# hanquansanren/DvD

Measured on AMD Instinct MI355X. Metric: documents/sec (50-step DDIM, 288x288 grid), higher is better.
Workload: dtype f16

## Files before the change

dvd_amd/csrc/attention.hip:

```cpp
#include "common.h"
#include "mfma.h"
#include <stdlib.h>

#ifndef DVD_ATTN64_OCC
#define DVD_ATTN64_OCC 2
#endif
#ifndef DVD_ATTN64_ROWSUM
#define DVD_ATTN64_ROWSUM 0
#endif
#ifndef DVD_ATTN_PF
#define DVD_ATTN_PF 4
#endif

namespace dvd {

struct AttnArgs {
  const _Float16* Q;
  const _Float16* K;
  const _Float16* Vt;
  _Float16* O;
  long sQ, sK, sVt, sO;
  int ldq, ldk, ldvt, ldo;
  int heads, batch, tq, tk;
  int kv_div;
  int nqb;
  float c;
  unsigned long long* stamps;
  int xcd_map;
};

__device__ __forceinline__ int kappa(int r) {
  return (r & ~12) | ((r & 4) << 1) | ((r & 8) >> 1);
}

__device__ __forceinline__ float half_swap_max(float x) {
  float a = x, b = x;
  asm volatile("s_nop 1\n\tv_permlane32_swap_b32 %0, %1\n\ts_nop 1" : "+v"(a), "+v"(b));
  return fmaxf(a, b);
}

template <int D>
__global__ void __launch_bounds__(256, (D == 256 ? 1 : 2)) flash_attn_kernel(AttnArgs p) {
  constexpr int KB = 64;
  constexpr int KP = 2 * D + 16;
  constexpr int VP = 2 * KB + 16;
  constexpr int KBYTES = KB * KP, VBYTES = D * VP;
  constexpr int KCH = D / 8;
  constexpr int NK = KB * KCH / 256;
  constexpr int NV = D * 8 / 256;
  constexpr int KS = D / 16;
  constexpr int DT = D / 32;
  constexpr float RESCALE_THR = 10.f;
  extern __shared__ __attribute__((aligned(16))) char smem[];

  const int nwg = gridDim.x;
  int id = blockIdx.x;
  {
    const int q = nwg / 8, rr = nwg % 8, xcd = id % 8, k = id / 8;
    id = (xcd < rr ? xcd * (q + 1) : rr * (q + 1) + (xcd - rr) * q) + k;
  }
  const int qb = id % p.nqb;
  const int bh = id / p.nqb;
  const int head = bh % p.heads, b = bh / p.heads;
  const int kvb = b / p.kv_div;

  const int tid = threadIdx.x, lane = tid & 63, wave = tid >> 6;
  const int r = lane & 31, h = lane >> 5;

  const _Float16* Qg = p.Q + b * p.sQ + (size_t)head * D;
  const _Float16* Kg = p.K + kvb * p.sK + (size_t)head * D;
  const _Float16* Vg = p.Vt + kvb * p.sVt + (size_t)head * D * p.ldvt;

  const int qrow = min(qb * 128 + wave * 32 + r, p.tq - 1);
  half8 qf[KS];
  {
    const _Float16* qp = Qg + (size_t)qrow * p.ldq + 8 * h;
#pragma unroll
    for (int ks = 0; ks < KS; ++ks) qf[ks] = *(const half8*)(qp + 16 * ks);
  }

  floatx16 o[DT];
#pragma unroll
  for (int dt = 0; dt < DT; ++dt)
#pragma unroll
    for (int i = 0; i < 16; ++i) o[dt][i] = 0.f;
  float m_run = -1e30f, l_run = 0.f;

  u32x4 kreg[NK], vreg[NV];
  int k_lofs[NK], v_lofs[NV];
  int k_row[NK], k_col[NK], v_row[NV], v_col[NV];
#pragma unroll
  for (int i = 0; i < NK; ++i) {
    const int cidx = tid + 256 * i;
    k_row[i] = cidx / KCH;
    k_col[i] = (cidx % KCH) * 8;
    k_lofs[i] = k_row[i] * KP + (cidx % KCH) * 16;
  }
#pragma unroll
  for (int i = 0; i < NV; ++i) {
    const int cidx = tid + 256 * i;
    v_row[i] = cidx / 8;
    v_col[i] = (cidx % 8) * 8;
    v_lofs[i] = KBYTES + v_row[i] * VP + (cidx % 8) * 16;
  }
  const int nt = (p.tk + KB - 1) / KB;

#define DVD_ATTN_GLOAD(t_)                                                                  \
  {                                                                                         \
    const int key0 = (t_) * KB;                                                             \
    _Pragma("unroll") for (int i = 0; i < NK; ++i) {                                        \
      const int kr = min(key0 + k_row[i], p.tk - 1);                                        \
// ... 1266 lines not shown
    if (j < 2) r64p::glds_piece(Vg + (size_t)min(j, nt - 1) * (KB * 2), voff, vdst + j * VBYTES);
  }
  asm volatile("s_waitcnt vmcnt(0)\n\ts_barrier" ::: "memory");

  float a0, a1;
  h64m_prologue_s0(kf, a0, a1);
  asm volatile("s_barrier" ::: "memory");
  {
    const float mloc[2] = {a0, a1};
#pragma unroll
    for (int rb = 0; rb < 2; ++rb) {
      const float m = half_swap_max(mloc[rb] * p.c);
      sm[rb].m = m;
      sm[rb].thr = m + RESCALE_THR;
    }
  }
  const char* kg = uniform_ptr(Kg + (size_t)min(3, nt - 1) * ktile);
  const char* vg = uniform_ptr(Vg + (size_t)min(2, nt - 1) * (KB * 2));
  const int klim = nt - 4, vlim = nt - 3;
  const unsigned kstep = (unsigned)ktile, vstep = KB * 2;
  float e0, e1;
  h64m_prologue_units(kf, p.c, sm[0].m, sm[1].m, e0, e1);
#define H64M_LOOP_ARGS sm[0].l, sm[1].l, sm[0].m, sm[1].m, sm[0].thr, sm[1].thr, e0, e1, kg, vg, nt, kf, vrel0, vrel1, koff, voff, p.c, \
                       kdst, vdst, kstep, vstep, klim, vlim
#ifdef DVD_LAB
  if constexpr (DBG == 1) h64m_loop_noeu(H64M_LOOP_ARGS);
  else if constexpr (DBG == 2) h64m_loop_m16(H64M_LOOP_ARGS);
  else if constexpr (DBG == 3) h64m_loop_mfmaonly(H64M_LOOP_ARGS);
  else
#endif
    h64m_loop(H64M_LOOP_ARGS);
#undef H64M_LOOP_ARGS

  const int lane_e = (int)__builtin_amdgcn_mbcnt_hi(~0u, __builtin_amdgcn_mbcnt_lo(~0u, 0u));
  const int re = lane_e & 31, he = lane_e >> 5;
#pragma unroll
  for (int rb = 0; rb < 2; ++rb) {
    const float l_tot = sm[rb].l + __shfl_xor(sm[rb].l, 32);
    const float inv = 1.f / l_tot;
    const int qglob = qb * 256 + wave * 64 + rb * 32 + re;
    if (qglob < p.tq) {
      _Float16* op = p.O + b * p.sO + (size_t)qglob * p.ldo + (size_t)head * D + 4 * he;
#pragma unroll
      for (int dt = 0; dt < 2; ++dt) {
        floatx16 x;
        if (rb == 0 && dt == 0) x = r64m_read_o<0>();
        else if (rb == 0) x = r64m_read_o<16>();
        else if (dt == 0) x = r64m_read_o<32>();
        else x = r64m_read_o<48>();
#pragma unroll
        for (int g4 = 0; g4 < 4; ++g4) {
          half4 v;
#pragma unroll
          for (int j = 0; j < 4; ++j) v[j] = (_Float16)(x[4 * g4 + j] * inv);
          *(half4*)(op + 32 * dt + 8 * g4) = v;
        }
      }
    }
  }
}


typedef unsigned uintx4 __attribute__((ext_vector_type(4)));
#include "attn_h64x_body.inc"
#include "attn_h64l_body.inc"
#ifdef DVD_LAB
#include "../../benchmarks/lab/csrc/attn_h64x_abl.inc"
#include "../../benchmarks/lab/csrc/attn_h64l_abl.inc"
#endif

template <int DBG, bool LM>
__global__ void __launch_bounds__(256, 2) __attribute__((amdgpu_num_vgpr(H64X_COMPILER_VGPRS))) flash_attn_h64x_kernel(AttnArgs p) {
  using namespace h64m;
  constexpr int D = 64, KB = 32;
  extern __shared__ __attribute__((aligned(16))) char smem[];
  typedef __attribute__((address_space(3))) void* lptr_t;

  const int nwg = gridDim.x;
  int id = blockIdx.x;
  {
    const int q = nwg / 8, rr = nwg % 8, xcd = id % 8, k = id / 8;
    id = (xcd < rr ? xcd * (q + 1) : rr * (q + 1) + (xcd - rr) * q) + k;
  }
  const int qb = id % p.nqb;
  const int bh = id / p.nqb;
  const int head = bh % p.heads, b = bh / p.heads;
  const int kvb = b / p.kv_div;
  const int tid = threadIdx.x, lane = tid & 63;
  const int wave = __builtin_amdgcn_readfirstlane(tid >> 6);
  const int c16 = lane & 15, g = lane >> 4;

  const _Float16* Qg = p.Q + b * p.sQ + (size_t)head * D;
  const char* Kg = (const char*)(p.K + kvb * p.sK + (size_t)head * D);
  const char* Vg = (const char*)(p.Vt + kvb * p.sVt + (size_t)head * D * p.ldvt);
  {
    const int qrow = qb * 256 + wave * 64 + c16;
    const unsigned rowb = (unsigned)(p.ldq * 2);
    const unsigned q0 = (unsigned)min(qrow, p.tq - 1) * rowb + 16 * g, q1 = (unsigned)min(qrow + 16, p.tq - 1) * rowb + 16 * g;
    const unsigned q2 = (unsigned)min(qrow + 32, p.tq - 1) * rowb + 16 * g, q3 = (unsigned)min(qrow + 48, p.tq - 1) * rowb + 16 * g;
    if constexpr (LM) h64l_load_q((const _Float16*)uniform_ptr((const char*)Qg), q0, q1, q2, q3, p.c);
    else h64x_load_q((const _Float16*)uniform_ptr((const char*)Qg), q0, q1, q2, q3, p.c);
  }
  unsigned koff, voff;
  {
    const int i = 8 * (wave & 1) + (lane >> 3), kb2 = wave >> 1;
    const int key = 8 * (i >> 2) + 4 * kb2 + (i & 3);
    koff = (unsigned)key * (unsigned)(p.ldk * 2) + (unsigned)(((lane & 7) ^ ((i >> 1) & 7)) * 16);
    voff = (unsigned)(16 * wave + (lane >> 2)) * (unsigned)(p.ldvt * 2) + (unsigned)(((lane & 3) ^ ((0u - (unsigned)(lane >> 4)) & 3)) * 16);
  }
  const unsigned lds0 = (unsigned)(uintptr_t)(lptr_t)smem;
  const unsigned kf0 = lds0 + c16 * 128 + (((0 + g) ^ ((c16 >> 1) & 7)) * 16);
  const unsigned kf1 = lds0 + c16 * 128 + (((4 + g) ^ ((c16 >> 1) & 7)) * 16);
  const unsigned vrel = lds0 + VBASE + c16 * 64 + ((g ^ ((0u - (unsigned)(c16 >> 2)) & 3)) * 16);

  if constexpr (LM) h64l_zero_o();
  else h64x_zero_o();
  const int nt = p.tk / KB;
  const size_t ktile = (size_t)KB * p.ldk * 2;
  const unsigned kdst = lds0 + wave * 1024, vdst = lds0 + VBASE + wave * 1024;
#pragma unroll
  for (int j = 0; j < 3; ++j) {
    r64p::glds_piece(Kg + (size_t)min(j, nt - 1) * ktile, koff, kdst + j * KBYTES);
    if (j < 2) r64p::glds_piece(Vg + (size_t)min(j, nt - 1) * (KB * 2), voff, vdst + j * VBYTES);
  }
  asm volatile("s_waitcnt vmcnt(0)\n\ts_barrier" ::: "memory");

  float a[4];
  if constexpr (LM) h64l_prologue_s0(kf0, kf1, a[0], a[1], a[2], a[3]);
  else h64x_prologue_s0(kf0, kf1, a[0], a[1], a[2], a[3]);
  asm volatile("s_barrier" ::: "memory");
  float m[4];
#pragma unroll
  for (int q = 0; q < 4; ++q) {
    float x = a[q];
    x = fmaxf(x, __shfl_xor(x, 16));
    x = fmaxf(x, __shfl_xor(x, 32));
    m[q] = x;
  }
  const char* kg = uniform_ptr(Kg + (size_t)min(3, nt - 1) * ktile);
  const char* vg = uniform_ptr(Vg + (size_t)min(2, nt - 1) * (KB * 2));
  const int klim = nt - 4, vlim = nt - 3;
  const unsigned kstep = (unsigned)ktile, vstep = KB * 2;
  if constexpr (LM) h64l_prologue_units(kf0, kf1, m[0], m[1], m[2], m[3]);
  else h64x_prologue_units(kf0, kf1, m[0], m[1], m[2], m[3]);
  float l[4] = {0.f, 0.f, 0.f, 0.f};
#define H64X_TAIL_ARGS kg, vg, nt, kf0, kf1, vrel, koff, voff, kdst, vdst, kstep, vstep, klim, vlim
  if constexpr (LM) {
    const uintx4 ones = {0x3c003c00u, 0x3c003c00u, 0x3c003c00u, 0x3c003c00u};
#ifdef DVD_LAB
    if constexpr (DBG == 1) h64l_loop_novalu(ones, H64X_TAIL_ARGS);
    else if constexpr (DBG == 2) h64l_loop_nobar(ones, H64X_TAIL_ARGS);
    else if constexpr (DBG == 3) h64l_loop_mfmaonly(ones, H64X_TAIL_ARGS);
    else
#endif
      h64l_loop(ones, H64X_TAIL_ARGS);
    l[0] = h64l_read_l<0>(); l[1] = h64l_read_l<1>(); l[2] = h64l_read_l<2>(); l[3] = h64l_read_l<3>();
  } else {
#ifdef DVD_LAB
    if constexpr (DBG == 1) h64x_loop_novalu(l[0], l[1], l[2], l[3], H64X_TAIL_ARGS);
    else if constexpr (DBG == 2) h64x_loop_nobar(l[0], l[1], l[2], l[3], H64X_TAIL_ARGS);
    else if constexpr (DBG == 3) h64x_loop_mfmaonly(l[0], l[1], l[2], l[3], H64X_TAIL_ARGS);
    else
#endif
      h64x_loop(l[0], l[1], l[2], l[3], H64X_TAIL_ARGS);
  }
#undef H64X_TAIL_ARGS

  const int lane_e = (int)__builtin_amdgcn_mbcnt_hi(~0u, __builtin_amdgcn_mbcnt_lo(~0u, 0u));
  const int c16e = lane_e & 15, ge = lane_e >> 4;
#pragma unroll
  for (int q = 0; q < 4; ++q) {
    float lt = l[q];
    if constexpr (!LM) {
      lt += __shfl_xor(lt, 16);
      lt += __shfl_xor(lt, 32);
    }
    const float inv = 1.f / lt;
    const int qglob = qb * 256 + wave * 64 + 16 * q + c16e;
    if (qglob < p.tq) {
      _Float16* op = p.O + b * p.sO + (size_t)qglob * p.ldo + (size_t)head * D + 4 * ge;
      floatx16 x;
      if (q == 0) x = r64m_read_o<0>();
      else if (q == 1) x = r64m_read_o<16>();
      else if (q == 2) x = r64m_read_o<32>();
      else x = r64m_read_o<48>();
#pragma unroll
      for (int db = 0; db < 4; ++db) {
        half4 v;
#pragma unroll
        for (int j = 0; j < 4; ++j) v[j] = (_Float16)(x[4 * db + j] * inv);
        *(half4*)(op + 16 * db) = v;
      }
    }
  }
}

#ifdef DVD_LAB
#include "../../benchmarks/lab/csrc/attention_lab.inc"
#endif

}

using namespace dvd;

#ifdef DVD_LAB
static unsigned long long* g_attn_stamps = nullptr;
extern "C" int dvd_attn_debug_stamps(void* dev_u64) { g_attn_stamps = (unsigned long long*)dev_u64; return DVD_OK; }
#endif

static constexpr int R64_MIN_TQ = 5376;

struct AttnKernel {
  const char* name;
  void (*fn)(AttnArgs);
  int rows, lds;
};
constexpr int GLDS256_LDS = 2 * (64 * 512 + 256 * 128), GLDS64_LDS = 2 * (64 * 128 + 64 * 128);

static AttnKernel attn_kernel(int head_dim, bool fast, bool r64) {
  const bool d256 = head_dim == 256;
  if (fast && d256 && !r64) return {"flash_attn_glds_kernel<256, 0>", flash_attn_glds_kernel<256, 0>, 128, GLDS256_LDS};
  if (fast && d256) return {"flash_attn_r64x_kernel<0>", flash_attn_r64x_kernel<0>, 256, r64p::LDS_BYTES};
  if (fast && r64) return {"flash_attn_h64x_kernel<0, true>", flash_attn_h64x_kernel<0, true>, 256, h64m::LDS_BYTES};
  if (d256) return {"flash_attn_kernel<256>", flash_attn_kernel<256>, 128, 2 * (64 * (2 * 256 + 16) + 256 * (2 * 64 + 16))};
  if (fast) return {"flash_attn_glds_kernel<64, 0>", flash_attn_glds_kernel<64, 0>, 128, GLDS64_LDS};
  return {"flash_attn_kernel<64>", flash_attn_kernel<64>, 128, 2 * (64 * (2 * 64 + 16) + 64 * (2 * 64 + 16))};
}
static bool attn_fast(int tk) { return tk % 64 == 0; }
static bool attn_r64(int tq) { return tq >= R64_MIN_TQ; }
static AttnKernel attn_select(int head_dim, int tq, int tk) { return attn_kernel(head_dim, attn_fast(tk), attn_r64(tq)); }

extern "C" const char* dvd_flash_attn_kernel_name(int head_dim, int tq, int tk) {
  if (head_dim == 32) return "flash_attn_f32_hd32_kernel";
  if (head_dim != 64 && head_dim != 256) return "";
  return attn_select(head_dim, tq, tk).name;
}

template <typename KernelT>
static void allow_lds(KernelT kernel, int bytes) {
  (void)hipFuncSetAttribute((const void*)kernel, hipFuncAttributeMaxDynamicSharedMemorySize, bytes);
}

extern "C" int dvd_flash_attn(const dvd_attn_desc* d, void* stream) {
  DVD_REQUIRE(d && d->Q && d->K && d->Vt && d->O, "flash_attn: null pointer");
  DVD_REQUIRE(d->head_dim == 64 || d->head_dim == 256, "flash_attn: head_dim %d not in {64,256}", d->head_dim);
  DVD_REQUIRE(d->heads > 0 && d->batch > 0 && d->tq > 0 && d->tk > 0 && d->kv_batch_div > 0, "flash_attn: bad shape");
  DVD_REQUIRE(d->tk % 8 == 0, "flash_attn: tk=%d must be a multiple of 8", d->tk);
  DVD_REQUIRE(d->ldq % 8 == 0 && d->ldk % 8 == 0 && d->ldvt % 8 == 0 && d->ldo % 4 == 0 &&
                  d->strideQ % 8 == 0 && d->strideK % 8 == 0 && d->strideVt % 8 == 0 && d->strideO % 4 == 0 &&
                  ((uintptr_t)d->Q % 16) == 0 && ((uintptr_t)d->K % 16) == 0 && ((uintptr_t)d->Vt % 16) == 0 &&
                  ((uintptr_t)d->O % 8) == 0,
              "flash_attn: operands must be 16-byte aligned");
  AttnArgs p;
  p.Q = (const _Float16*)d->Q; p.K = (const _Float16*)d->K; p.Vt = (const _Float16*)d->Vt; p.O = (_Float16*)d->O;
  p.sQ = d->strideQ; p.sK = d->strideK; p.sVt = d->strideVt; p.sO = d->strideO;
  p.ldq = d->ldq; p.ldk = d->ldk; p.ldvt = d->ldvt; p.ldo = d->ldo;
  p.heads = d->heads; p.batch = d->batch; p.tq = d->tq; p.tk = d->tk;
  p.kv_div = d->kv_batch_div;
  p.nqb = cdiv(d->tq, 128);
  p.c = d->scale * 1.4426950408889634f;
  p.stamps = nullptr;
  p.xcd_map = 0;
  const long nwg = (long)p.nqb * d->heads * d->batch;
  DVD_REQUIRE(nwg < (1l << 31), "flash_attn: grid too large");
  hipStream_t st = (hipStream_t)stream;
  bool fast = attn_fast(d->tk), r64 = attn_r64(d->tq);
  static DeviceOnce attr_done;
  const unsigned long long dev_bit = DeviceOnce::current_bit();
  const bool first_on_device = attr_done.need(dev_bit);
  if (first_on_device) {
    for (int hd : {256, 64})
      for (bool f : {false, true})
        for (bool r : {false, true}) {
          const AttnKernel k = attn_kernel(hd, f, r);
          allow_lds(k.fn, k.lds);
        }
    attr_done.done(dev_bit);
  }
#ifdef DVD_LAB
  p.stamps = g_attn_stamps;
  if (const char* xm = getenv("DVD_ATTN_XCDMAP")) p.xcd_map = atoi(xm);
  const bool dbg = getenv("DVD_ATTN_DEBUG"), bulk = getenv("DVD_ATTN_BULK");
  if (getenv("DVD_ATTN_V1")) fast = false;
  if (getenv("DVD_ATTN_R64") || getenv("DVD_ATTN_R64P") || getenv("DVD_ATTN_R64M") || getenv("DVD_ATTN_R64M_ABL") || getenv("DVD_ATTN_R64X_ABL") ||
      getenv("DVD_ATTN_R64OLD"))
    r64 = true;
  if (getenv("DVD_ATTN_R32") || getenv("DVD_ATTN_PIPE") || getenv("DVD_ATTN_GLDS64") || bulk) r64 = false;
  if (first_on_device) {
    constexpr int LDS = GLDS256_LDS;
    allow_lds(flash_attn_dsplit_kernel, LDS);
    allow_lds(flash_attn_glds_kernel<256, 1>, LDS);
    allow_lds(flash_attn_glds_kernel<256, 2>, LDS);
    allow_lds(flash_attn_glds_kernel<256, 3>, LDS);
    allow_lds(flash_attn_pipe_kernel<0>, LDS);
    allow_lds(flash_attn_pipe_kernel<1>, LDS);
    allow_lds(flash_attn_r64_kernel<0>, 2 * (32 * 512 + 256 * 64));
    allow_lds(flash_attn_r64_kernel<1>, 2 * (32 * 512 + 256 * 64));
    allow_lds(flash_attn_r64p_kernel<0>, r64p::LDS_BYTES);
    allow_lds(flash_attn_r64p_kernel<1>, r64p::LDS_BYTES);
    allow_lds(flash_attn_r64m_kernel<0>, r64p::LDS_BYTES);
    allow_lds(flash_attn_r64x_kernel<1>, r64p::LDS_BYTES);
    allow_lds(flash_attn_r64x_kernel<2>, r64p::LDS_BYTES);
    allow_lds(flash_attn_r64x_kernel<3>, r64p::LDS_BYTES);
    allow_lds(flash_attn_r64m_kernel<1>, r64p::LDS_BYTES);
    allow_lds(flash_attn_r64m_kernel<2>, r64p::LDS_BYTES);
    allow_lds(flash_attn_r64m_kernel<3>, r64p::LDS_BYTES);
    allow_lds(flash_attn_r64m_kernel<4>, r64p::LDS_BYTES);
    allow_lds(flash_attn_r64m_kernel<5>, r64p::LDS_BYTES);
    allow_lds(flash_attn_r64m_kernel<6>, r64p::LDS_BYTES);
    allow_lds(flash_attn_r64m_kernel<7>, r64p::LDS_BYTES);
  }
  if (fast && d->head_dim == 256) {
    constexpr int LDS = GLDS256_LDS;
    if (getenv("DVD_ATTN_DSPLIT")) {
      flash_attn_dsplit_kernel<<<(unsigned)nwg, 512, LDS, st>>>(p);
      return check_launch("flash_attn(lab dsplit)");
    }
    if (r64 && getenv("DVD_ATTN_R64X_ABL")) {
      p.nqb = cdiv(d->tq, 256);
      const unsigned g = (unsigned)((long)p.nqb * d->heads * d->batch);
      switch (atoi(getenv("DVD_ATTN_R64X_ABL"))) {
        case 1: flash_attn_r64x_kernel<1><<<g, 256, r64p::LDS_BYTES, st>>>(p); break;
        case 2: flash_attn_r64x_kernel<2><<<g, 256, r64p::LDS_BYTES, st>>>(p); break;
        case 3: flash_attn_r64x_kernel<3><<<g, 256, r64p::LDS_BYTES, st>>>(p); break;
        default: flash_attn_r64x_kernel<0><<<g, 256, r64p::LDS_BYTES, st>>>(p);
      }
      return check_launch("flash_attn(lab r64x ablation)");
    }
    if (r64 && (getenv("DVD_ATTN_R64M") || getenv("DVD_ATTN_R64M_ABL"))) {
      p.nqb = cdiv(d->tq, 256);
      const unsigned g = (unsigned)((long)p.nqb * d->heads * d->batch);
      switch (getenv("DVD_ATTN_R64M_ABL") ? atoi(getenv("DVD_ATTN_R64M_ABL")) : 0) {
        case 1: flash_attn_r64m_kernel<1><<<g, 256, r64p::LDS_BYTES, st>>>(p); break;
        case 2: flash_attn_r64m_kernel<2><<<g, 256, r64p::LDS_BYTES, st>>>(p); break;
        case 3: flash_attn_r64m_kernel<3><<<g, 256, r64p::LDS_BYTES, st>>>(p); break;
        case 4: flash_attn_r64m_kernel<4><<<g, 256, r64p::LDS_BYTES, st>>>(p); break;
        case 5: flash_attn_r64m_kernel<5><<<g, 256, r64p::LDS_BYTES, st>>>(p); break;
        case 6: flash_attn_r64m_kernel<6><<<g, 256, r64p::LDS_BYTES, st>>>(p); break;
        case 7: flash_attn_r64m_kernel<7><<<g, 256, r64p::LDS_BYTES, st>>>(p); break;
        default: flash_attn_r64m_kernel<0><<<g, 256, r64p::LDS_BYTES, st>>>(p);
      }
      return check_launch("flash_attn(lab r64m)");
    }
    if (r64 && getenv("DVD_ATTN_R64P")) {
      p.nqb = cdiv(d->tq, 256);
      const unsigned g = (unsigned)((long)p.nqb * d->heads * d->batch);
      if (dbg) flash_attn_r64p_kernel<1><<<g, 256, r64p::LDS_BYTES, st>>>(p);
      else flash_attn_r64p_kernel<0><<<g, 256, r64p::LDS_BYTES, st>>>(p);
      return check_launch("flash_attn(lab r64p)");
    }
    if (r64 && getenv("DVD_ATTN_R64OLD")) {
      p.nqb = cdiv(d->tq, 256);
      const unsigned g = (unsigned)((long)p.nqb * d->heads * d->batch);
      if (dbg) flash_attn_r64_kernel<1><<<g, 256, 2 * (32 * 512 + 256 * 64), st>>>(p);
      else flash_attn_r64_kernel<0><<<g, 256, 2 * (32 * 512 + 256 * 64), st>>>(p);
      return check_launch("flash_attn(lab r64 old)");
    }
    if (!r64 && getenv("DVD_ATTN_PIPE")) {
      if (dbg) flash_attn_pipe_kernel<1><<<(unsigned)nwg, 256, LDS, st>>>(p);
      else flash_attn_pipe_kernel<0><<<(unsigned)nwg, 256, LDS, st>>>(p);
      return check_launch("flash_attn(lab pipe)");
    }
    if (!r64 && (dbg || bulk)) {
      if (dbg && bulk) flash_attn_glds_kernel<256, 3><<<(unsigned)nwg, 256, LDS, st>>>(p);
      else if (bulk) flash_attn_glds_kernel<256, 2><<<(unsigned)nwg, 256, LDS, st>>>(p);
      else flash_attn_glds_kernel<256, 1><<<(unsigned)nwg, 256, LDS, st>>>(p);
      return check_launch("flash_attn(lab glds variant)");
    }
  } else if (fast) {
    constexpr int LDS = GLDS64_LDS;
    if (getenv("DVD_ATTN_H64X") || (r64 && (getenv("DVD_ATTN_H64X_ABL") || getenv("DVD_ATTN_H64X_NOLM")))) {
      p.nqb = cdiv(d->tq, 256);
      const unsigned g = (unsigned)((long)p.nqb * d->heads * d->batch);
      const int abl = getenv("DVD_ATTN_H64X_ABL") ? atoi(getenv("DVD_ATTN_H64X_ABL")) : 0;
      if (getenv("DVD_ATTN_H64X_NOLM")) {
        switch (abl) {
          case 1: flash_attn_h64x_kernel<1, false><<<g, 256, h64m::LDS_BYTES, st>>>(p); break;
          case 2: flash_attn_h64x_kernel<2, false><<<g, 256, h64m::LDS_BYTES, st>>>(p); break;
          case 3: flash_attn_h64x_kernel<3, false><<<g, 256, h64m::LDS_BYTES, st>>>(p); break;
          default: flash_attn_h64x_kernel<0, false><<<g, 256, h64m::LDS_BYTES, st>>>(p);
        }
        return check_launch("flash_attn(lab h64x, row sums on the VALU)");
      }
      switch (abl) {
        case 1: flash_attn_h64x_kernel<1, true><<<g, 256, h64m::LDS_BYTES, st>>>(p); break;
        case 2: flash_attn_h64x_kernel<2, true><<<g, 256, h64m::LDS_BYTES, st>>>(p); break;
        case 3: flash_attn_h64x_kernel<3, true><<<g, 256, h64m::LDS_BYTES, st>>>(p); break;
        default: flash_attn_h64x_kernel<0, true><<<g, 256, h64m::LDS_BYTES, st>>>(p);
      }
      return check_launch("flash_attn(lab h64x)");
    }
    if (getenv("DVD_ATTN_H64M")) {
      p.nqb = cdiv(d->tq, 256);
      const unsigned g = (unsigned)((long)p.nqb * d->heads * d->batch);
      switch (getenv("DVD_ATTN_H64M_ABL") ? atoi(getenv("DVD_ATTN_H64M_ABL")) : 0) {
        case 1: flash_attn_h64m_kernel<1><<<g, 256, h64m::LDS_BYTES, st>>>(p); break;
        case 2: flash_attn_h64m_kernel<2><<<g, 256, h64m::LDS_BYTES, st>>>(p); break;
        case 3: flash_attn_h64m_kernel<3><<<g, 256, h64m::LDS_BYTES, st>>>(p); break;
        default: flash_attn_h64m_kernel<0><<<g, 256, h64m::LDS_BYTES, st>>>(p);
      }
      return check_launch("flash_attn(lab h64m)");
    }
    if (getenv("DVD_ATTN_64X2")) {
      p.nqb = cdiv(d->tq, 256);
      flash_attn_glds64x2_kernel<<<(unsigned)((long)p.nqb * d->heads * d->batch), 256, LDS, st>>>(p);
      return check_launch("flash_attn(lab 64x2)");
    }
    if (dbg || bulk) {
      if (dbg) flash_attn_glds_kernel<64, 1><<<(unsigned)nwg, 256, LDS, st>>>(p);
      else flash_attn_glds_kernel<64, 2><<<(unsigned)nwg, 256, LDS, st>>>(p);
      return check_launch("flash_attn(lab glds64 variant)");
    }
  }
#endif
  const AttnKernel k = attn_kernel(d->head_dim, fast, r64);
  p.nqb = cdiv(d->tq, k.rows);
  k.fn<<<(unsigned)((long)p.nqb * d->heads * d->batch), 256, k.lds, st>>>(p);
  return check_launch("flash_attn");
}
```

dvd_amd/csrc/dither.hip:

```cpp
#include "common.h"

namespace dvd {

__device__ __forceinline__ unsigned dither_hash(unsigned g) {
  unsigned h = g * 0x9E3779B1u;
  h ^= h >> 15; h *= 0x85EBCA77u;
  h ^= h >> 13; h *= 0xC2B2AE3Du;
  h ^= h >> 16;
  return h;
}

__device__ __forceinline__ unsigned short dither_one(unsigned short hb, unsigned short lb, unsigned g, unsigned phase) {
  if ((lb & 0x7fffu) == 0) return hb;
  unsigned short nb;
  if ((hb & 0x7fffu) == 0) nb = (unsigned short)((lb & 0x8000u) | 1u);
  else nb = ((hb ^ lb) & 0x8000u) ? (unsigned short)(hb - 1) : (unsigned short)(hb + 1);
  if ((nb & 0x7c00u) == 0x7c00u) return hb;
  const float hf = __half2float(__ushort_as_half(hb)), lf = __half2float(__ushort_as_half(lb));
  const float nf = __half2float(__ushort_as_half(nb));
  float frac = __fdiv_rn(fabsf(lf), fabsf(__fsub_rn(nf, hf)));
  frac = fminf(frac, 0.99999994f);
  const unsigned thr = (unsigned)(frac * 4294967296.0f);
  const unsigned u = dither_hash(g) + phase;
  return u < thr ? nb : hb;
}

__global__ void __launch_bounds__(256) dither_f16_kernel(const uint4* __restrict__ hi, const uint4* __restrict__ lo,
                                                         uint4* __restrict__ out, long n8, unsigned elem0, unsigned phase) {
  const long i = (long)blockIdx.x * 256 + threadIdx.x;
  if (i >= n8) return;
  const uint4 h = hi[i], l = lo[i];
  const unsigned hw[4] = {h.x, h.y, h.z, h.w}, lw[4] = {l.x, l.y, l.z, l.w};
  unsigned ow[4];
  const unsigned g0 = elem0 + (unsigned)(i * 8);
#pragma unroll
  for (int k = 0; k < 4; ++k) {
    const unsigned short a = dither_one((unsigned short)(hw[k] & 0xffffu), (unsigned short)(lw[k] & 0xffffu), g0 + 2 * k, phase);
    const unsigned short b = dither_one((unsigned short)(hw[k] >> 16), (unsigned short)(lw[k] >> 16), g0 + 2 * k + 1, phase);
    ow[k] = (unsigned)a | ((unsigned)b << 16);
  }
  out[i] = make_uint4(ow[0], ow[1], ow[2], ow[3]);
}

}

using namespace dvd;

extern "C" int dvd_dither_f16(const void* hi, const void* lo, void* out, long nelem, unsigned elem0, unsigned step,
                              void* stream) {
  DVD_REQUIRE(hi && lo && out, "dither_f16: null pointer");
  DVD_REQUIRE(nelem > 0 && nelem % 8 == 0, "dither_f16: nelem=%ld must be a positive multiple of 8", nelem);
  DVD_REQUIRE(((uintptr_t)hi % 16) == 0 && ((uintptr_t)lo % 16) == 0 && ((uintptr_t)out % 16) == 0,
              "dither_f16: pointers must be 16-byte aligned");
  const long n8 = nelem / 8;
  const unsigned phase = step * 0x9E3779B9u;
  dither_f16_kernel<<<(unsigned)((n8 + 255) / 256), 256, 0, (hipStream_t)stream>>>((const uint4*)hi, (const uint4*)lo,
                                                                                   (uint4*)out, n8, elem0, phase);
  return check_launch("dither_f16");
}
```

dvd_amd/csrc/engine.hip:

```cpp
#include <string.h>
#include <algorithm>

#include <string>
#include <vector>

#include "common.h"
#include "gemm_common.h"
#include "mfma.h"

extern "C" {
int dvd_embed_obs_ln(const float*, const float*, const float*, const float*, float*, void*, int, int, void*);
int dvd_layernorm_rows(const float*, int, long, void*, int, long, int, long, int, const float*, const float*,
                       const float*, const float*, int, int, float, void*);
int dvd_build_r_rows(const float*, const float*, const float*, void*, int, int, int, int, int, void*);
int dvd_patch_rows(const float*, long, long, long, long, float*, int, int, int, int, void*);
int dvd_dwconv3x3(const void*, void*, const float*, const float*, int, int, int, void*);
int dvd_colmean(const float*, float*, float*, int, int, int, int, void*);
int dvd_posenc_add(float*, const float*, const float*, const float*, const float*, int, int, int, void*);
int dvd_small_linear(const float*, int, const float*, const float*, float*, int, int, int, int, int, int, int, void*);
int dvd_final_tokens(const float*, const float*, const float*, const float*, const float*, int, int, const float*,
                     const float*, const float*, float*, float*, int, int, void*);
int dvd_im2col3x3(const float*, long, long, long, float*, int, int, int, int, void*);
int dvd_conv3x3_nhwc(const float*, int, const float*, int, const float*, float*, int, int, int, int, void*);
int dvd_maxpool2_nhwc(const float*, float*, int, int, int, void*);
int dvd_resize_bilinear_nhwc(const float*, float*, int, int, int, int, int, void*);
int dvd_nhwc_to_nchw(const float*, float*, int, int, int, void*);
int dvd_dither_f16(const void*, const void*, void*, long, unsigned, unsigned, void*);
}

namespace dvd {

constexpr int HID = 384, DEC = 1536, FFN = 2048, RK = 1088 ;
constexpr int COLCHUNKS = 64;
constexpr int DEC_LAYERS = 6, PYR_LAYERS = 7;

struct TensorSpec {
  std::string name;
  int dtype;
  long nelem;
  bool wide;
};

static const int PYR_CIN[7] = {4, 64, 64, 128, 128, 256, 256};
static const int PYR_COUT[7] = {64, 64, 128, 128, 256, 256, 256};
static inline int pyr_kpad(int i) { return ((9 * PYR_CIN[i] + 63) / 64) * 64; }

#define DVD_W_HEAD(F, H)                                                                                           \
  F(obs_w, HID * 8) F(obs_b, HID) F(pos, T * HID)                                                                  \
  H(r_w16, (long)HID * RK, false) F(r_b, HID)                                                                      \
  F(c_w, (long)HID * 1024) F(c_b, HID) F(m_w, (long)HID * 1536) F(m_b, HID) F(l_w, (long)HID * 256) F(l_b, HID)    \
  F(t_w0, HID * 256) F(t_b0, HID) F(t_w2, HID * HID) F(t_b2, HID) F(ada_w, 6 * HID * HID) F(ada_b, 6 * HID)        \
  H(ca_wq16, HID * HID, false) F(ca_bq, HID) H(ca_wk16, HID * HID, false) F(ca_bk, HID)                            \
  H(ca_wv16, HID * HID, true) F(ca_bv, HID) F(ca_wk32, HID * HID) F(ca_wv32, HID * HID)                            \
  H(ca_wo16, HID * HID, false) F(ca_bo, HID)                                                                       \
  H(sa_wqk16, 2 * HID * HID, true) F(sa_bqk, 2 * HID) H(sa_wv16, HID * HID, true) F(sa_bv, HID)                    \
  H(sa_wp16, HID * HID, false) F(sa_bp, HID)                                                                       \
  H(fc1_w16, 4 * HID * HID, true) F(fc1_b, 4 * HID) H(fc2_w16, 4 * HID * HID, false) F(fc2_b, HID)                 \
  F(pe_h0_w, (long)DEC * DEC) F(pe_h0_b, DEC) F(pe_h2_w, (long)DEC * DEC) F(pe_h2_b, DEC)                          \
  F(pe_w0_w, (long)DEC * DEC) F(pe_w0_b, DEC) F(pe_w2_w, (long)DEC * DEC) F(pe_w2_b, DEC)                          \
  F(pe_htab, side * DEC) F(pe_wtab, side * DEC)
#define DVD_W_DEC(F, H)                                                                                            \
  F(n1w, DEC) F(n1b, DEC)                                                                                          \
  H(wqk16, 2L * DEC * DEC, true) H(wv16, (long)DEC * DEC, true) H(wfc16, (long)DEC * DEC, true)                    \
  F(n2w, DEC) F(n2b, DEC) H(c1w16, (long)FFN * DEC, true) F(c1b, FFN) F(dww, 9 * FFN) F(dwb, FFN)                  \
  H(c2w16, (long)DEC * FFN, true) F(c2b, DEC)
#define DVD_W_TAIL(F, H)                                                                                           \
  F(dec_nw, DEC) F(dec_nb, DEC) F(fin_ada_w, 2L * DEC * DEC) F(fin_ada_b, 2 * DEC) F(fin_w, 8 * DEC) F(fin_b, 8)
#define DVD_W_PYR(F, H) F(w, (long)PYR_COUT[i] * pyr_kpad(i)) F(b, PYR_COUT[i])

#define DVD_B_STEP(X)                                                                                              \
                                                                         \
  X(feat, docs * G * G * 256 * 4)                                                                                  \
  X(kc16, docs * T * HID * 2) X(km16, docs * T * HID * 2) X(kl16, docs * T * HID * 2)                              \
  X(vtc16, docs * T * HID * 2) X(vtm16, docs * T * HID * 2) X(vtl16, docs * T * HID * 2)                           \
                                                                                       \
  X(tbuf, 256) X(th, HID * 4) X(cvec, HID * 4) X(mod, 6 * HID * 4) X(finmod, 2 * DEC * 4)                          \
  X(pooled, N * DEC * 4) X(petmp, N * DEC * 4) X(hs, N * DEC * 4) X(wsc, N * DEC * 4)                              \
  X(part, N * COLCHUNKS * DEC * 4)                                                                                 \
      \
  X(w16dith, dith_bytes)                                                                                           \
                                                                                         \
  X(xtok32, NT * HID * 4) X(xq16, NT * HID * 2) X(arows16, NT * RK * 2) X(rtok16, NT * HID * 2)                    \
  X(q16, NT * HID * 2) X(kr16, NT * HID * 2) X(vtr16, NT * HID * 2)                                                \
  X(att16, NT * DEC * 2) X(z, NT * DEC * 4) X(h16, NT * DEC * 2) X(qk16, NT * 2 * DEC * 2)                         \
  X(vt16, NT * DEC * 2) X(mlp16, NT * 4 * DEC * 2)
#define DVD_B_PREP(X)                                                                                              \
  X(p_cat4, (size_t)4 * 512 * 512 * 4) X(p_col, (size_t)512 * 512 * 576 * 4) X(p_actA, (size_t)512 * 512 * 64 * 4) \
  X(p_actB, (size_t)512 * 512 * 64 * 4) X(p_rows, T * 1536 * 4) X(p_tok32, T * HID * 4)

#define F(n, e) PFX(n),
#define H(n, e, wide) PFX(n), PFX(n##_lo),
#define PFX(n) WD_##n
enum { DVD_W_DEC(F, H) WD_COUNT };
#undef PFX
#define PFX(n) WP_##n
enum { DVD_W_PYR(F, H) WP_COUNT };
#undef PFX
#define PFX(n) W_##n
enum {
  DVD_W_HEAD(F, H) W_DEC0, W_DEC_LAST = W_DEC0 + DEC_LAYERS * WD_COUNT - 1,
  DVD_W_TAIL(F, H) W_PYR0, W_COUNT = W_PYR0 + PYR_LAYERS * WP_COUNT
};
#undef PFX
#undef F
#undef H
constexpr int W_dec(int j, int k) { return W_DEC0 + j * WD_COUNT + k; }
constexpr int W_pyr(int i, int k) { return W_PYR0 + i * WP_COUNT + k; }
#define X(n, bytes) B_##n,
enum { DVD_B_STEP(X) DVD_B_PREP(X) B_COUNT };
#undef X

static std::vector<TensorSpec> tensor_specs(int G) {
  const long T = (long)(G / 2) * (G / 2), side = G / 2;
  std::vector<TensorSpec> v;
  std::string p;
#define F(n, e) v.push_back({p + #n, 0, (long)(e), false});
#define H(n, e, wide) v.push_back({p + #n, 1, (long)(e), wide}); v.push_back({p + #n "_lo", 1, (long)(e), false});
  DVD_W_HEAD(F, H)
  for (int j = 0; j < DEC_LAYERS; ++j) { p = "d" + std::to_string(j) + "_"; DVD_W_DEC(F, H) }
  p.clear();
  DVD_W_TAIL(F, H)
  for (int i = 0; i < PYR_LAYERS; ++i) { p = "pyr" + std::to_string(i) + "_"; DVD_W_PYR(F, H) }
#undef F
#undef H
  return v;
}

struct Buf {
  const char* name;
  size_t off, bytes;
};

struct GraphKey {
  int feat_mode;
  const void *x_t, *init_flow, *init_feat, *x0_out;
  bool operator==(const GraphKey& o) const {
    return feat_mode == o.feat_mode && x_t == o.x_t && init_flow == o.init_flow && init_feat == o.init_feat &&
           x0_out == o.x0_out;
  }
};
struct GraphEntry {
  GraphKey key;
  hipGraphExec_t exec;
  unsigned long last_use;
};

struct Engine {
  int G, side, docs, hyp, N;
  long T, NT;
  std::vector<TensorSpec> specs;
  std::vector<const void*> wptr;
  char* ws = nullptr;
  size_t ws_bytes = 0, need_bytes = 0;
  std::vector<Buf> bufs;
  bool prepared = false;
  bool split_weights = true;
  bool ffn_lo = true;
  bool small_tiles = false;
  bool dither = false;
  unsigned dither_step = 0;
  std::vector<long> dith_off;
  std::vector<int> dith_list;
  long dith_total = 0;
  bool use_graphs = false;
  bool prof_on = false;
  std::vector<hipEvent_t> prof_ev;
  size_t prof_head = 0, prof_inflight = 0;
  double prof_total_ms = 0.0;
  long prof_count = 0;
  int debug_stop = 0;
  std::vector<GraphEntry> graphs;
  hipStream_t cap_stream = nullptr;

  const float* F(int i) const { return (const float*)wptr[i]; }
  char* B(int i) const { return ws + bufs[i].off; }
  float* f32(int i) const { return (float*)B(i); }
  _Float16* f16(int i) const { return (_Float16*)B(i); }
  struct Pair { const void *hi, *lo; };
  Pair W16(int i, bool ffn = false) const {
    if (dither && !small_tiles && specs[i].wide) return {f16(B_w16dith) + dith_off[i], nullptr};
    return {wptr[i], split_weights && (ffn_lo || !ffn) ? wptr[i + 1] : nullptr};
  }
  int find_b(const char* name) const {
    for (size_t i = 0; i < bufs.size(); ++i)
      if (strcmp(bufs[i].name, name) == 0) return (int)i;
    return -1;
  }
  unsigned long graph_clock = 0;
  void drop_graphs() {
    bool any = false;
    for (auto& g : graphs) any = any || g.exec;
    if (any) (void)hipDeviceSynchronize();
    for (auto& g : graphs)
      if (g.exec) (void)hipGraphExecDestroy(g.exec);
    graphs.clear();
  }
  void evict_one(hipStream_t st) {
    size_t victim = 0;
    bool found_eager = false;
    for (size_t i = 0; i < graphs.size(); ++i) {
      if (!graphs[i].exec) {
        if (!found_eager || graphs[i].last_use < graphs[victim].last_use) victim = i;
        found_eager = true;
      } else if (!found_eager && graphs[i].last_use < graphs[victim].last_use) {
        victim = i;
      }
    }
    if (graphs[victim].exec) {
      (void)hipStreamSynchronize(st);
      (void)hipGraphExecDestroy(graphs[victim].exec);
    }
    graphs.erase(graphs.begin() + (long)victim);
  }
};

static const int PROF_PAIRS = 4096;

static int prof_drain_one(Engine* e) {
  float ms = 0.f;
  hipEvent_t a = e->prof_ev[2 * e->prof_head], b = e->prof_ev[2 * e->prof_head + 1];
  if (hipEventSynchronize(b) != hipSuccess || hipEventElapsedTime(&ms, a, b) != hipSuccess) {
    set_error("engine_profile: event query failed");
    return DVD_E_LAUNCH;
  }
  e->prof_total_ms += ms; e->prof_count += 1;
  e->prof_head = (e->prof_head + 1) % PROF_PAIRS; e->prof_inflight -= 1;
  return DVD_OK;
}

static void plan(Engine* e) {
  size_t off = 0;
  auto add = [&](const char* n, size_t bytes) {
    bytes = (bytes + 255) & ~(size_t)255;
    e->bufs.push_back({n, off, bytes});
    off += bytes;
  };
  const size_t T = e->T, NT = e->NT, docs = e->docs, N = e->N, G = e->G;
  e->dith_off.assign(e->specs.size(), -1);
  e->dith_list.clear();
  e->dith_total = 0;
  for (size_t i = 0; i + 1 < e->specs.size(); ++i) {
    if (!e->specs[i].wide) continue;
    e->dith_off[i] = e->dith_total;
    e->dith_list.push_back((int)i);
    e->dith_total += (e->specs[i].nelem + 127) / 128 * 128;
  }
  const size_t dith_bytes = (size_t)e->dith_total * 2;
#define X(n, bytes) add(#n, bytes);
  DVD_B_STEP(X)
  const size_t step_end = off;
  off = e->bufs[B_xtok32].off;
  DVD_B_PREP(X)
#undef X
  e->need_bytes = off > step_end ? off : step_end;
}

constexpr int GELU = 1, RELU = 2;
struct Gemm : dvd_gemm_desc {
  Gemm(int dtype_, int M_, int N_, int K_, int batch_ = 1) {
    memset(static_cast<dvd_gemm_desc*>(this), 0, sizeof(dvd_gemm_desc));
    dtype = dtype_ == 1 ? 1 : 0; small_tiles = dtype_ == 2 ? 1 : dtype_ == 3 ? 2 : 0;
    M = M_; N = N_; K = K_; batch = batch_;
    lo_scale = 1.f; ldpos = N_; ldgate = N_;
  }
  Gemm& a(const void* p, int ld, long stride = 0) { A = p; lda = ld; strideA = stride; return *this; }
  Gemm& b(const void* p, int ld, long stride = 0) { B = p; ldb = ld; strideB = stride; return *this; }
  Gemm& a(Engine::Pair w, int ld) { A_lo = w.lo; return a(w.hi, ld); }
  Gemm& b(Engine::Pair w, int ld) { B_lo = w.lo; return b(w.hi, ld); }
  Gemm& out32(float* p, int ld, long stride = 0) { C32 = p; ldc = ld; strideC32 = stride; return *this; }
  Gemm& out16(void* p, int ld, long stride = 0) { C16 = p; ldc16 = ld; strideC16 = stride; return *this; }
  Gemm& bias_col(const float* p) { bias = p; bias_row = 0; return *this; }
  Gemm& bias_rows(const float* p) { bias = p; bias_row = 1; return *this; }
  Gemm& act_fn(int f) { act = f; return *this; }
  Gemm& add_pos(const float* p, int rows) { pos = p; pos_rows = rows; return *this; }
  Gemm& mul_gate(const float* p, int rows) { gate = p; gate_rows = rows; return *this; }
  Gemm& add_res(const float* p, int ld, long stride = 0) { res = p; ldres = ld; strideRes = stride; return *this; }
};

static int gemm(const Gemm& d, void* stream) {
  auto a16 = [](const void* q) { return ((uintptr_t)q % 16) == 0; };
  DVD_REQUIRE(a16(d.C32) && a16(d.C16) && a16(d.bias) && a16(d.pos) && a16(d.gate) && a16(d.res),
              "engine gemm: output / epilogue pointers must be 16-byte aligned");
  return dvd_gemm_nt(&d, stream);
}

struct Attn : dvd_attn_desc {
  Attn(int hd, int heads_, int batch_, int tq_, int tk_, int kv_div, float scale_) {
    memset(static_cast<dvd_attn_desc*>(this), 0, sizeof(dvd_attn_desc));
    head_dim = hd; heads = heads_; batch = batch_; tq = tq_; tk = tk_; kv_batch_div = kv_div; scale = scale_;
  }
  Attn& q(const void* p, int ld, long stride) { Q = p; ldq = ld; strideQ = stride; return *this; }
  Attn& k(const void* p, int ld, long stride) { K = p; ldk = ld; strideK = stride; return *this; }
  Attn& vt(const void* p, int ld, long stride) { Vt = p; ldvt = ld; strideVt = stride; return *this; }
  Attn& out(void* p, int ld, long stride) { O = p; ldo = ld; strideO = stride; return *this; }
};

static int attn(const Attn& d, void* stream) { return dvd_flash_attn(&d, stream); }

__global__ void set_scalar_kernel(float* p, float v) { *p = v; }

#define TRY(x)            \
  do {                    \
    int _e = (x);         \
    if (_e) return _e;    \
  } while (0)

}

using namespace dvd;

extern "C" int dvd_engine_create(int grid, int docs, int n_hyp, void** handle) {
  DVD_REQUIRE(handle, "engine_create: null handle");
  DVD_REQUIRE(grid >= 4 && grid % 2 == 0 && ((grid / 2) * (grid / 2)) % 8 == 0,
              "engine_create: grid=%d must be even with (grid/2)^2 a multiple of 8", grid);
  DVD_REQUIRE(docs > 0 && n_hyp > 0, "engine_create: docs/n_hyp must be positive");
  Engine* e = new Engine();
  e->G = grid; e->side = grid / 2; e->docs = docs; e->hyp = n_hyp; e->N = docs * n_hyp;
  e->T = (long)e->side * e->side; e->NT = e->T * e->N;
  e->specs = tensor_specs(grid);
  e->wptr.assign(e->specs.size(), nullptr);
  plan(e);
  e->small_tiles = e->T <= 1024;
  e->dither = !e->small_tiles;
  if (e->specs.size() != (size_t)W_COUNT || e->bufs.size() != (size_t)B_COUNT) {
    delete e;
    set_error("engine_create: the index enumerators and the expanded tables differ in length");
    return DVD_E_STATE;
  }
  *handle = e;
  return DVD_OK;
}

extern "C" int dvd_engine_destroy(void* handle) {
  Engine* e = (Engine*)handle;
  if (!e) return DVD_OK;
  e->drop_graphs();
  if (e->cap_stream) (void)hipStreamDestroy(e->cap_stream);
  for (auto& ev : e->prof_ev) (void)hipEventDestroy(ev);
  delete e;
  return DVD_OK;
}

extern "C" long dvd_engine_workspace_bytes(void* handle) { return handle ? (long)((Engine*)handle)->need_bytes : -1; }

extern "C" int dvd_engine_bind_workspace(void* handle, void* ws, long bytes) {
  DVD_REQUIRE(handle && ws, "engine_bind_workspace: null pointer");
  Engine* e = (Engine*)handle;
  DVD_REQUIRE((size_t)bytes >= e->need_bytes && ((uintptr_t)ws % 256) == 0,
              "engine_bind_workspace: need %zu bytes, 256-byte aligned (got %ld)", e->need_bytes, bytes);
  e->ws = (char*)ws; e->ws_bytes = bytes; e->prepared = false;
  e->drop_graphs();
  return DVD_OK;
}

extern "C" int dvd_engine_tensor_count(void* handle) { return handle ? (int)((Engine*)handle)->specs.size() : -1; }

extern "C" int dvd_engine_tensor_info(void* handle, int index, const char** name, int* dtype, long* nelem) {
  DVD_REQUIRE(handle && name && dtype && nelem, "engine_tensor_info: null pointer");
  Engine* e = (Engine*)handle;
  DVD_REQUIRE(index >= 0 && index < (int)e->specs.size(), "engine_tensor_info: index out of range");
  *name = e->specs[index].name.c_str(); *dtype = e->specs[index].dtype; *nelem = e->specs[index].nelem;
  return DVD_OK;
}

extern "C" int dvd_engine_set_tensor(void* handle, const char* name, const void* dev_ptr, long nelem) {
  DVD_REQUIRE(handle && name && dev_ptr, "engine_set_tensor: null pointer");
  Engine* e = (Engine*)handle;
  for (size_t i = 0; i < e->specs.size(); ++i)
    if (e->specs[i].name == name) {
      DVD_REQUIRE(e->specs[i].nelem == nelem, "engine_set_tensor: %s expects %ld elements, got %ld", name,
                  e->specs[i].nelem, nelem);
      DVD_REQUIRE(((uintptr_t)dev_ptr % 16) == 0, "engine_set_tensor: %s must be 16-byte aligned", name);
      if (e->wptr[i] != dev_ptr) e->drop_graphs();
      e->wptr[i] = dev_ptr;
      return DVD_OK;
    }
  set_error("engine_set_tensor: unknown tensor '%s'", name);
  return DVD_E_ARG;
}

extern "C" int dvd_engine_profile(void* handle, int enable) {
  DVD_REQUIRE(handle, "engine_profile: null handle");
  Engine* e = (Engine*)handle;
  if (enable && e->prof_ev.empty()) {
    e->prof_ev.resize(2 * PROF_PAIRS);
    for (auto& ev : e->prof_ev)
      if (hipEventCreate(&ev) != hipSuccess) { set_error("engine_profile: hipEventCreate failed"); return DVD_E_LAUNCH; }
  }
  e->prof_on = enable != 0;
  e->prof_head = 0; e->prof_inflight = 0; e->prof_total_ms = 0.0; e->prof_count = 0;
  return DVD_OK;
}

extern "C" int dvd_engine_profile_read(void* handle, int* launches, double* total_ms) {
  DVD_REQUIRE(handle && launches && total_ms, "engine_profile_read: null pointer");
  Engine* e = (Engine*)handle;
  while (e->prof_inflight) TRY(prof_drain_one(e));
  *launches = (int)e->prof_count; *total_ms = e->prof_total_ms;
  e->prof_total_ms = 0.0; e->prof_count = 0;
  return DVD_OK;
}

extern "C" int dvd_engine_set_option(void* handle, const char* name, int value) {
  DVD_REQUIRE(handle && name, "engine_set_option: null pointer");
  Engine* e = (Engine*)handle;
  if (strcmp(name, "split_weights") == 0) { e->split_weights = value != 0; e->drop_graphs(); return DVD_OK; }
  if (strcmp(name, "small_tiles") == 0) { e->small_tiles = value != 0; e->drop_graphs(); return DVD_OK; }
  if (strcmp(name, "ffn_lo") == 0) { e->ffn_lo = value != 0; e->drop_graphs(); return DVD_OK; }
  if (strcmp(name, "dither") == 0) { e->dither = value != 0; e->drop_graphs(); return DVD_OK; }
  if (strcmp(name, "dither_step") == 0) { e->dither_step = (unsigned)value; return DVD_OK; }
  if (strcmp(name, "graphs") == 0) {
    e->use_graphs = value != 0;
    if (!e->use_graphs) e->drop_graphs();
    return DVD_OK;
  }
  set_error("engine_set_option: unknown option '%s'", name);
  return DVD_E_ARG;
}

extern "C" int dvd_engine_debug_stop(void* handle, int stage) {
  DVD_REQUIRE(handle && stage >= 0, "engine_debug_stop: bad arguments");
  ((Engine*)handle)->debug_stop = stage;
  return DVD_OK;
}

extern "C" int dvd_engine_debug_buffer(void* handle, const char* name, void** ptr, long* bytes) {
  DVD_REQUIRE(handle && name && ptr && bytes, "engine_debug_buffer: null pointer");
  Engine* e = (Engine*)handle;
  DVD_REQUIRE(e->ws, "engine_debug_buffer: no workspace bound");
  const int i = e->find_b(name);
  DVD_REQUIRE(i >= 0, "engine_debug_buffer: unknown buffer '%s'", name);
  *ptr = e->B(i); *bytes = (long)e->bufs[i].bytes;
  return DVD_OK;
}

static int require_ready(Engine* e, bool need_prepared) {
  if (!e->ws) { set_error("engine: no workspace bound"); return DVD_E_STATE; }
  for (size_t i = 0; i < e->specs.size(); ++i)
    if (!e->wptr[i]) { set_error("engine: weight tensor '%s' not set", e->specs[i].name.c_str()); return DVD_E_STATE; }
  if (need_prepared && !e->prepared) { set_error("engine: dvd_engine_prepare_docs has not run"); return DVD_E_STATE; }
  return DVD_OK;
}

extern "C" int dvd_engine_prepare_docs(void* handle, const float* y512, const float* mask_cat,
                                       const float* mask_y512, const float* line_msk, void* stream) {
  DVD_REQUIRE(handle && y512 && mask_cat && mask_y512 && line_msk, "engine_prepare_docs: null pointer");
  Engine* e = (Engine*)handle;
  TRY(require_ready(e, false));
  hipStream_t st = (hipStream_t)stream;
  const int G = e->G;
  const long T = e->T;
  float *cat4 = e->f32(B_p_cat4), *col = e->f32(B_p_col);
  const float* pos = e->F(W_pos);
  for (int d = 0; d < e->docs; ++d) {
    if (hipMemcpyAsync(cat4, y512 + (size_t)d * 3 * 512 * 512, (size_t)3 * 512 * 512 * 4, hipMemcpyDeviceToDevice, st) != hipSuccess ||
        hipMemcpyAsync(cat4 + 3 * 512 * 512, mask_cat + (size_t)d * 512 * 512, (size_t)512 * 512 * 4, hipMemcpyDeviceToDevice, st) != hipSuccess) {
      set_error("engine_prepare_docs: device copy failed");
      return DVD_E_LAUNCH;
    }
    struct L { int idx, hw; bool pool; };
    const L layers[7] = {{0, 512, false}, {1, 512, true}, {2, 256, false}, {3, 256, true},
                         {4, 128, false}, {5, 128, false}, {6, 128, true}};
    const float* cur = cat4;
    long sc = 512L * 512, sy = 512, sx = 1;
    float* act[2] = {e->f32(B_p_actA), e->f32(B_p_actB)};
    int wi = 0;
    for (const L& l : layers) {
      const int cin = PYR_CIN[l.idx], cout = PYR_COUT[l.idx], kp = pyr_kpad(l.idx);
      const float *w = e->F(W_pyr(l.idx, WP_w)), *b = e->F(W_pyr(l.idx, WP_b));
      float* outp = act[wi];
      wi ^= 1;
      if (sc == 1 && cin % 16 == 0 && kp == 9 * cin) {
        TRY(dvd_conv3x3_nhwc(cur, cin, w, kp, b, outp, cout, l.hw, l.hw, 1, stream));
      } else {
        TRY(dvd_im2col3x3(cur, sc, sy, sx, col, kp, cin, l.hw, l.hw, stream));
        TRY(gemm(Gemm(1, l.hw * l.hw, cout, kp).a(col, kp).b(w, kp).out32(outp, cout).bias_col(b).act_fn(RELU), stream));
      }
      int hw = l.hw;
      if (l.pool) {
        TRY(dvd_maxpool2_nhwc(outp, act[wi], cout, hw, hw, stream));
        outp = act[wi];
        wi ^= 1;
        hw /= 2;
      }
      cur = outp;
      sc = 1; sy = (long)hw * cout; sx = cout;
    }
    float* feat = e->f32(B_feat) + (size_t)d * G * G * 256;
    if (G == 64) {
      if (hipMemcpyAsync(feat, cur, (size_t)64 * 64 * 256 * 4, hipMemcpyDeviceToDevice, st) != hipSuccess) {
        set_error("engine_prepare_docs: device copy failed");
        return DVD_E_LAUNCH;
      }
    } else {
      TRY(dvd_resize_bilinear_nhwc(cur, feat, 256, 64, 64, G, G, stream));
    }
  }
  {
    const size_t per_doc = (size_t)T * (1536 + HID) * 4;
    {
      const int chain[5] = {B_p_col, B_p_actA, B_p_actB, B_p_rows, B_p_tok32};
      for (int i = 0; i + 1 < 5; ++i)
        DVD_REQUIRE(e->bufs[chain[i]].off < e->bufs[chain[i + 1]].off &&
                        e->bufs[chain[i]].off + e->bufs[chain[i]].bytes <= e->bufs[chain[i + 1]].off &&
                        e->bufs[chain[i + 1]].off - (e->bufs[chain[i]].off + e->bufs[chain[i]].bytes) < 4096,
                    "engine_prepare_docs: the prepare-time scratch regions are not laid out back to back (plan() changed?)");
    }
    const size_t avail = e->bufs[B_p_tok32].off + e->bufs[B_p_tok32].bytes - e->bufs[B_p_col].off;
    DVD_REQUIRE(avail >= per_doc, "engine_prepare_docs: prepare scratch smaller than one document's rows");
    const int gmax = (int)std::max<size_t>(1, std::min<size_t>((size_t)e->docs, avail / per_doc));
    for (int d0 = 0; d0 < e->docs; d0 += gmax) {
      const int gd = std::min(gmax, e->docs - d0);
      float* rows_g = col;
      float* tok_g = col + (size_t)gd * T * 1536;
      struct S { const float* src; long sn, sc, sy, sx; int c; int w, b, k16, vt16; };
      const S streams[3] = {
          {e->f32(B_feat) + (size_t)d0 * G * G * 256, (long)G * G * 256, 1, (long)G * 256, 256, 256, W_c_w, W_c_b, B_kc16,
           B_vtc16},
          {mask_y512 + (size_t)d0 * 384 * G * G, 384L * G * G, (long)G * G, G, 1, 384, W_m_w, W_m_b, B_km16, B_vtm16},
          {line_msk + (size_t)d0 * 64 * G * G, 64L * G * G, (long)G * G, G, 1, 64, W_l_w, W_l_b, B_kl16, B_vtl16}};
      for (const S& s : streams) {
        const int K4 = 4 * s.c;
        DVD_REQUIRE((long)gd * T < (1l << 31), "engine_prepare_docs: group too large");
        TRY(dvd_patch_rows(s.src, s.sn, s.sc, s.sy, s.sx, rows_g, K4, gd, s.c, G, stream));
        TRY(gemm(Gemm(1, (int)(gd * T), HID, K4).a(rows_g, K4).b(e->F(s.w), K4).out32(tok_g, HID).bias_col(e->F(s.b))
                     .add_pos(pos, (int)T), stream));
        _Float16* k16 = e->f16(s.k16) + (size_t)d0 * T * HID;
        _Float16* vt16 = e->f16(s.vt16) + (size_t)d0 * T * HID;
        TRY(gemm(Gemm(1, (int)(gd * T), HID, HID).a(tok_g, HID).b(e->F(W_ca_wk32), HID).out16(k16, HID)
                     .bias_col(e->F(W_ca_bk)), stream));
        TRY(gemm(Gemm(1, HID, (int)T, HID, gd).a(e->F(W_ca_wv32), HID).b(tok_g, HID, (long)T * HID)
                     .out16(vt16, (int)T, (long)T * HID).bias_rows(e->F(W_ca_bv)), stream));
      }
    }
  }
  e->prepared = true;
  return DVD_OK;
}

extern "C" int dvd_engine_feat_nchw(void* handle, float* out, void* stream) {
  DVD_REQUIRE(handle && out, "engine_feat_nchw: null pointer");
  Engine* e = (Engine*)handle;
  TRY(require_ready(e, true));
  for (int d = 0; d < e->docs; ++d)
    TRY(dvd_nhwc_to_nchw(e->f32(B_feat) + (size_t)d * e->G * e->G * 256,
                         out + (size_t)d * 256 * e->G * e->G, 256, e->G, e->G, stream));
  return DVD_OK;
}

static int enqueue_step(Engine* e, const float* x_t, int feat_mode, const float* init_flow,
                        const float* init_feat_nchw, float* x0_out, void* stream) {
  hipStream_t st = (hipStream_t)stream;
  const int G = e->G, N = e->N, side = e->side, hyp = e->hyp;
  const int T = (int)e->T;
  const long NT = e->NT;
  const int F16 = e->small_tiles ? (e->NT >= 16384 ? 3 : 2) : 0;
  constexpr int F16S = 2;

  auto f32 = [e](int i) { return e->f32(i); };
  auto f16 = [e](int i) { return e->f16(i); };
  const long TH = (long)T * HID, TD = (long)T * DEC;

  TRY(dvd_small_linear(f32(B_tbuf), 1, e->F(W_t_w0), e->F(W_t_b0), f32(B_th), HID, 1, 256, HID, 256, 2, 1, stream));
  TRY(dvd_small_linear(f32(B_th), HID, e->F(W_t_w2), e->F(W_t_b2), f32(B_cvec), HID, 1, HID, HID, HID, 0, 0, stream));
  TRY(dvd_small_linear(f32(B_cvec), HID, e->F(W_ada_w), e->F(W_ada_b), f32(B_mod), 6 * HID, 1, HID, 6 * HID, HID, 1, 0,
                       stream));
  TRY(dvd_small_linear(f32(B_cvec), HID, e->F(W_fin_ada_w), e->F(W_fin_ada_b), f32(B_finmod), 2 * DEC, 1, DEC, 2 * DEC, HID,
                       1, 0, stream));
  const float* mod = f32(B_mod);
  const float *sh_a = mod, *sc_a = mod + HID, *g_a = mod + 2 * HID, *sh_m = mod + 3 * HID, *sc_m = mod + 4 * HID,
              *g_m = mod + 5 * HID;

  TRY(dvd_embed_obs_ln(x_t, e->F(W_obs_w), e->F(W_obs_b), e->F(W_pos), f32(B_xtok32), f16(B_xq16), N, G, stream));
  TRY(dvd_build_r_rows(f32(B_feat), init_feat_nchw, init_flow, f16(B_arows16), RK, N, G, hyp, feat_mode, stream));
  TRY(gemm(Gemm(F16, (int)NT, HID, RK).a(f16(B_arows16), RK).b(e->W16(W_r_w16), RK).out16(f16(B_rtok16), HID)
               .bias_col(e->F(W_r_b)).add_pos(e->F(W_pos), T), stream));

  TRY(gemm(Gemm(F16, (int)NT, HID, HID).a(f16(B_xq16), HID).b(e->W16(W_ca_wq16), HID).out16(f16(B_q16), HID)
               .bias_col(e->F(W_ca_bq)), stream));
  TRY(gemm(Gemm(F16, (int)NT, HID, HID).a(f16(B_rtok16), HID).b(e->W16(W_ca_wk16), HID).out16(f16(B_kr16), HID)
               .bias_col(e->F(W_ca_bk)), stream));
  TRY(gemm(Gemm(F16S, HID, T, HID, N).a(e->W16(W_ca_wv16), HID).b(f16(B_rtok16), HID, TH).out16(f16(B_vtr16), T, TH)
               .bias_rows(e->F(W_ca_bv)), stream));
  {
    const int kn[3] = {B_kc16, B_km16, B_kl16}, vn[3] = {B_vtc16, B_vtm16, B_vtl16};
    for (int s = 0; s < 3; ++s)
      TRY(attn(Attn(64, 6, N, T, T, hyp, 0.125f).q(f16(B_q16), HID, TH).k(f16(kn[s]), HID, TH).vt(f16(vn[s]), T, TH)
                   .out(f16(B_att16) + (size_t)s * NT * HID, HID, TH), stream));
    TRY(attn(Attn(64, 6, N, T, T, 1, 0.125f).q(f16(B_q16), HID, TH).k(f16(B_kr16), HID, TH).vt(f16(B_vtr16), T, TH)
                 .out(f16(B_att16) + (size_t)3 * NT * HID, HID, TH), stream));
  }
  TRY(gemm(Gemm(F16, (int)NT, HID, HID, 4).a(f16(B_att16), HID, NT * HID).b(e->W16(W_ca_wo16), HID).out32(f32(B_z), DEC, HID)
               .bias_col(e->F(W_ca_bo)).add_res(f32(B_xtok32), HID), stream));

  if (e->debug_stop == 1) return check_launch("engine_denoise_step(stop 1)");
  TRY(dvd_layernorm_rows(f32(B_z), DEC, HID, f16(B_h16), HID, NT * HID, 4, NT, HID, nullptr, nullptr, sh_a, sc_a, 0, (int)NT,
                         1e-6f, stream));
  TRY(gemm(Gemm(F16, (int)(4 * NT), 2 * HID, HID).a(f16(B_h16), HID).b(e->W16(W_sa_wqk16), HID).out16(f16(B_qk16), 2 * HID)
               .bias_col(e->F(W_sa_bqk)), stream));
  TRY(gemm(Gemm(F16S, HID, T, HID, 4 * N).a(e->W16(W_sa_wv16), HID).b(f16(B_h16), HID, TH).out16(f16(B_vt16), T, TH)
               .bias_rows(e->F(W_sa_bv)), stream));
  TRY(attn(Attn(64, 6, 4 * N, T, T, 1, 0.125f).q(f16(B_qk16), 2 * HID, 2 * TH).k(f16(B_qk16) + HID, 2 * HID, 2 * TH)
               .vt(f16(B_vt16), T, TH).out(f16(B_att16), HID, TH), stream));
  TRY(gemm(Gemm(F16, (int)NT, HID, HID, 4).a(f16(B_att16), HID, NT * HID).b(e->W16(W_sa_wp16), HID).out32(f32(B_z), DEC, HID)
               .bias_col(e->F(W_sa_bp)).mul_gate(g_a, (int)NT).add_res(f32(B_z), DEC, HID), stream));
  TRY(dvd_layernorm_rows(f32(B_z), DEC, HID, f16(B_h16), HID, NT * HID, 4, NT, HID, nullptr, nullptr, sh_m, sc_m, 0, (int)NT,
                         1e-6f, stream));
  TRY(gemm(Gemm(F16, (int)(4 * NT), 4 * HID, HID).a(f16(B_h16), HID).b(e->W16(W_fc1_w16), HID).out16(f16(B_mlp16), 4 * HID)
               .bias_col(e->F(W_fc1_b)).act_fn(GELU), stream));
  TRY(gemm(Gemm(F16, (int)NT, HID, 4 * HID, 4).a(f16(B_mlp16), 4 * HID, NT * 4 * HID).b(e->W16(W_fc2_w16), 4 * HID)
               .out32(f32(B_z), DEC, HID).bias_col(e->F(W_fc2_b)).mul_gate(g_m, (int)NT).add_res(f32(B_z), DEC, HID), stream));

  if (e->debug_stop == 2) return check_launch("engine_denoise_step(stop 2)");
  TRY(dvd_colmean(f32(B_z), f32(B_part), f32(B_pooled), N, T, DEC, COLCHUNKS, stream));
  TRY(dvd_small_linear(f32(B_pooled), DEC, e->F(W_pe_h0_w), e->F(W_pe_h0_b), f32(B_petmp), DEC, N, DEC, DEC, DEC, 0, 2, stream));
  TRY(dvd_small_linear(f32(B_petmp), DEC, e->F(W_pe_h2_w), e->F(W_pe_h2_b), f32(B_hs), DEC, N, DEC, DEC, DEC, 0, 3, stream));
  TRY(dvd_small_linear(f32(B_pooled), DEC, e->F(W_pe_w0_w), e->F(W_pe_w0_b), f32(B_petmp), DEC, N, DEC, DEC, DEC, 0, 2, stream));
  TRY(dvd_small_linear(f32(B_petmp), DEC, e->F(W_pe_w2_w), e->F(W_pe_w2_b), f32(B_wsc), DEC, N, DEC, DEC, DEC, 0, 3, stream));
  TRY(dvd_posenc_add(f32(B_z), f32(B_hs), f32(B_wsc), e->F(W_pe_htab), e->F(W_pe_wtab), N, side, DEC, stream));

  if (e->debug_stop == 3) return check_launch("engine_denoise_step(stop 3)");
  _Float16* f1 = f16(B_mlp16);
  _Float16* f2 = f1 + (size_t)NT * FFN;
  for (int j = 0; j < DEC_LAYERS; ++j) {
    auto w = [j](int k) { return W_dec(j, k); };
    TRY(dvd_layernorm_rows(f32(B_z), DEC, 0, f16(B_h16), DEC, 0, 1, NT, DEC, e->F(w(WD_n1w)), e->F(w(WD_n1b)), nullptr, nullptr,
                           0, 1, 1e-5f, stream));
    TRY(gemm(Gemm(F16, (int)NT, 2 * DEC, DEC).a(f16(B_h16), DEC).b(e->W16(w(WD_wqk16)), DEC).out16(f16(B_qk16), 2 * DEC),
             stream));
    TRY(gemm(Gemm(F16, DEC, T, DEC, N).a(e->W16(w(WD_wv16)), DEC).b(f16(B_h16), DEC, TD).out16(f16(B_vt16), T, TD), stream));
    const bool timed = e->prof_on;
    size_t slot = 0;
    if (timed) {
      if (e->prof_inflight == (size_t)PROF_PAIRS) TRY(prof_drain_one(e));
      slot = (e->prof_head + e->prof_inflight) % PROF_PAIRS;
      (void)hipEventRecord(e->prof_ev[2 * slot], st);
    }
    TRY(attn(Attn(256, 6, N, T, T, 1, 0.0625f).q(f16(B_qk16), 2 * DEC, 2 * TD).k(f16(B_qk16) + DEC, 2 * DEC, 2 * TD)
                 .vt(f16(B_vt16), T, TD).out(f16(B_att16), DEC, TD), stream));
    if (timed) { (void)hipEventRecord(e->prof_ev[2 * slot + 1], st); e->prof_inflight += 1; }
    TRY(gemm(Gemm(F16, (int)NT, DEC, DEC).a(f16(B_att16), DEC).b(e->W16(w(WD_wfc16)), DEC).out32(f32(B_z), DEC)
                 .add_res(f32(B_z), DEC), stream));
    TRY(dvd_layernorm_rows(f32(B_z), DEC, 0, f16(B_h16), DEC, 0, 1, NT, DEC, e->F(w(WD_n2w)), e->F(w(WD_n2b)), nullptr, nullptr,
                           0, 1, 1e-5f, stream));
    TRY(gemm(Gemm(F16, (int)NT, FFN, DEC).a(f16(B_h16), DEC).b(e->W16(w(WD_c1w16),  true), DEC).out16(f1, FFN)
                 .bias_col(e->F(w(WD_c1b))).act_fn(RELU), stream));
    TRY(dvd_dwconv3x3(f1, f2, e->F(w(WD_dww)), e->F(w(WD_dwb)), N, side, FFN, stream));
    TRY(gemm(Gemm(F16, (int)NT, DEC, FFN).a(f2, FFN).b(e->W16(w(WD_c2w16),  true), FFN).out32(f32(B_z), DEC)
                 .bias_col(e->F(w(WD_c2b))).act_fn(RELU).add_res(f32(B_z), DEC), stream));
    if (e->debug_stop == 4 + j) return check_launch("engine_denoise_step(stop 4+j)");
  }

  const float* finmod = f32(B_finmod);
  TRY(dvd_final_tokens(f32(B_z), e->F(W_dec_nw), e->F(W_dec_nb), finmod, finmod + DEC, 0, (int)NT, e->F(W_fin_w),
                       e->F(W_fin_b), init_flow, x0_out, nullptr, N, G, stream));
  return check_launch("engine_denoise_step");
}

extern "C" int dvd_engine_denoise_step(void* handle, const float* x_t, float t_embed, int feat_mode,
                                       const float* init_flow, const float* init_feat_nchw, float* x0_out,
                                       void* stream) {
  DVD_REQUIRE(handle && x_t && init_flow && x0_out, "engine_denoise_step: null pointer");
  DVD_REQUIRE(feat_mode >= 0 && feat_mode <= 3 && (feat_mode != 3 || init_feat_nchw),
              "engine_denoise_step: feat_mode %d (3 needs init_feat)", feat_mode);
  Engine* e = (Engine*)handle;
  TRY(require_ready(e, true));
  DVD_REQUIRE(4 * e->NT < (1L << 31), "engine_denoise_step: batch too large for 32-bit row indices (NT=%ld)", e->NT);
  hipStream_t st = (hipStream_t)stream;
  set_scalar_kernel<<<1, 1, 0, st>>>(e->f32(B_tbuf), t_embed);
  if (e->dither && !e->small_tiles) {
    _Float16* dst = e->f16(B_w16dith);
    for (int i : e->dith_list)
      TRY(dvd_dither_f16(e->wptr[i], e->wptr[i + 1], dst + e->dith_off[i], e->specs[i].nelem, (unsigned)e->dith_off[i],
                         e->dither_step, stream));
  }
  if (!e->use_graphs || e->prof_on || e->debug_stop)
    return enqueue_step(e, x_t, feat_mode, init_flow, init_feat_nchw, x0_out, stream);

  const GraphKey key{feat_mode, x_t, init_flow, feat_mode == 3 ? init_feat_nchw : nullptr, x0_out};
  GraphEntry* ge = nullptr;
  for (auto& g : e->graphs)
    if (g.key == key) { ge = &g; break; }
  e->graph_clock += 1;
  if (!ge) {
    if (e->graphs.size() >= 32) e->evict_one(st);
    e->graphs.push_back({key, nullptr, e->graph_clock});
    return enqueue_step(e, x_t, feat_mode, init_flow, init_feat_nchw, x0_out, stream);
  }
  ge->last_use = e->graph_clock;
  if (!ge->exec) {
    if (!e->cap_stream && hipStreamCreateWithFlags(&e->cap_stream, hipStreamNonBlocking) != hipSuccess) {
      set_error("engine_denoise_step: cannot create the capture stream");
      return DVD_E_LAUNCH;
    }
    hipGraph_t graph = nullptr;
    if (hipStreamBeginCapture(e->cap_stream, hipStreamCaptureModeRelaxed) != hipSuccess) {
      set_error("engine_denoise_step: hipStreamBeginCapture failed");
      return DVD_E_LAUNCH;
    }
    const int rc = enqueue_step(e, x_t, feat_mode, init_flow, init_feat_nchw, x0_out, e->cap_stream);
    const hipError_t ec = hipStreamEndCapture(e->cap_stream, &graph);
    if (rc != DVD_OK) { if (graph) (void)hipGraphDestroy(graph); return rc; }
    if (ec != hipSuccess || !graph || hipGraphInstantiate(&ge->exec, graph, nullptr, nullptr, 0) != hipSuccess) {
      if (graph) (void)hipGraphDestroy(graph);
      ge->exec = nullptr;
      set_error("engine_denoise_step: graph capture/instantiate failed (%s)", hipGetErrorString(ec));
      return DVD_E_LAUNCH;
    }
    (void)hipGraphDestroy(graph);
  }
  if (hipGraphLaunch(ge->exec, st) != hipSuccess) {
    set_error("engine_denoise_step: hipGraphLaunch failed");
    return DVD_E_LAUNCH;
  }
  return check_launch("engine_denoise_step(graph)");
}
```

dvd_amd/csrc/tokens.hip:

```cpp
#include "common.h"
#include "mfma.h"

namespace dvd {

__device__ __forceinline__ float wave_sum(float v) {
#pragma unroll
  for (int o = 32; o > 0; o >>= 1) v += __shfl_xor(v, o);
  return v;
}

__global__ void __launch_bounds__(256) embed_obs_ln_kernel(const float* __restrict__ x, const float* __restrict__ w,
                                                           const float* __restrict__ bias,
                                                           const float* __restrict__ pos, float* __restrict__ tok32,
                                                           _Float16* __restrict__ ln16, int g, long rows) {
  const long row = (long)blockIdx.x * 4 + (threadIdx.x >> 6);
  if (row >= rows) return;
  const int lane = threadIdx.x & 63;
  const int side = g >> 1, T = side * side;
  const int n = (int)(row / T), t = (int)(row % T);
  const int ty = t / side, tx = t % side;
  float pv[8];
#pragma unroll
  for (int c = 0; c < 2; ++c)
#pragma unroll
    for (int p = 0; p < 2; ++p)
#pragma unroll
      for (int q = 0; q < 2; ++q)
        pv[c * 4 + p * 2 + q] = x[(((size_t)n * 2 + c) * g + (2 * ty + p)) * g + 2 * tx + q];
  float v[6];
  float s = 0.f;
#pragma unroll
  for (int j = 0; j < 6; ++j) {
    const int o = lane + 64 * j;
    float acc = bias[o];
#pragma unroll
    for (int k = 0; k < 8; ++k) acc += w[o * 8 + k] * pv[k];
    acc += pos[(size_t)t * 384 + o];
    v[j] = acc;
    s += acc;
  }
  const float mean = wave_sum(s) * (1.f / 384.f);
  float q2 = 0.f;
#pragma unroll
  for (int j = 0; j < 6; ++j) {
    const float d = v[j] - mean;
    q2 += d * d;
  }
  const float rstd = rsqrtf(wave_sum(q2) * (1.f / 384.f) + 1e-6f);
#pragma unroll
  for (int j = 0; j < 6; ++j) {
    const int o = lane + 64 * j;
    tok32[row * 384 + o] = v[j];
    ln16[row * 384 + o] = (_Float16)((v[j] - mean) * rstd);
  }
}

template <int C>
__global__ void __launch_bounds__(256) layernorm_rows_kernel(const float* __restrict__ in, int ldin, long sIn,
                                                             _Float16* __restrict__ out, int ldout, long sOut,
                                                             const float* __restrict__ gamma,
                                                             const float* __restrict__ beta,
                                                             const float* __restrict__ shift,
                                                             const float* __restrict__ scale, int ldmod,
                                                             int mod_rows, float eps, long rows) {
  constexpr int PER = C / 64;
  constexpr int V = (C == 384) ? 2 : 4;
  constexpr int NV = PER / V;
  const long row = (long)blockIdx.x * 4 + (threadIdx.x >> 6);
  if (row >= rows) return;
  const int lane = threadIdx.x & 63;
  const float* ip = in + blockIdx.y * sIn + row * ldin;
  float v[PER];
  float s = 0.f;
  typedef float fvec __attribute__((ext_vector_type(V)));
  typedef _Float16 hvec __attribute__((ext_vector_type(V)));
#pragma unroll
  for (int k = 0; k < NV; ++k) {
    const int c0 = (k * 64 + lane) * V;
    const fvec x = *(const fvec*)(ip + c0);
#pragma unroll
    for (int e = 0; e < V; ++e) {
      v[k * V + e] = x[e];
      s += x[e];
    }
  }
  const float mean = wave_sum(s) * (1.f / C);
  float q2 = 0.f;
#pragma unroll
  for (int k = 0; k < PER; ++k) {
    const float d = v[k] - mean;
    q2 += d * d;
  }
  const float rstd = rsqrtf(wave_sum(q2) * (1.f / C) + eps);
  _Float16* op = out + blockIdx.y * sOut + row * ldout;
  const float* sh = shift ? shift + (row / mod_rows) * ldmod : nullptr;
  const float* sc = scale ? scale + (row / mod_rows) * ldmod : nullptr;
#pragma unroll
  for (int k = 0; k < NV; ++k) {
    const int c0 = (k * 64 + lane) * V;
    fvec g = {}, bt = {}, scv = {}, shv = {};
    if (gamma) { g = *(const fvec*)(gamma + c0); bt = *(const fvec*)(beta + c0); }
    if (sc) { scv = *(const fvec*)(sc + c0); shv = *(const fvec*)(sh + c0); }
    hvec o;
#pragma unroll
    for (int e = 0; e < V; ++e) {
      float y = (v[k * V + e] - mean) * rstd;
      if (gamma) y = y * g[e] + bt[e];
      if (sc) y = y * (1.f + scv[e]) + shv[e];
      o[e] = (_Float16)y;
    }
    *(hvec*)(op + c0) = o;
  }
}

__global__ void __launch_bounds__(256) build_r_rows_kernel(const float* __restrict__ feat,
                                                           const float* __restrict__ init_feat_nchw,
                                                           const float* __restrict__ flow,
                                                           _Float16* __restrict__ out, int ldo, int g, int n_hyp,
                                                           int mode, long items) {
  const long item = (long)blockIdx.x * 4 + (threadIdx.x >> 6);
  if (item >= items) return;
  const int lane = threadIdx.x & 63;
  const int side = g >> 1, T = side * side;
  const int pq = (int)(item & 3);
  const long tokrow = item >> 2;
  const int n = (int)(tokrow / T), t = (int)(tokrow % T);
  const int y = 2 * (t / side) + (pq >> 1), x = 2 * (t % side) + (pq & 1);
  const size_t gg = (size_t)g * g;
  const float fx = flow[((size_t)n * 2 + 0) * gg + (size_t)y * g + x];
  const float fy = flow[((size_t)n * 2 + 1) * gg + (size_t)y * g + x];
  _Float16* orow = out + tokrow * ldo + pq * 258;
  const float* fd = feat + (size_t)(n / n_hyp) * gg * 256;
  float v[4] = {0.f, 0.f, 0.f, 0.f};
  if (mode == 1) {
    const floatx4 f = *(const floatx4*)(fd + ((size_t)y * g + x) * 256 + 4 * lane);
    v[0] = f[0]; v[1] = f[1]; v[2] = f[2]; v[3] = f[3];
  } else if (mode == 3) {
#pragma unroll
    for (int e = 0; e < 4; ++e) v[e] = init_feat_nchw[((size_t)n * 256 + 4 * lane + e) * gg + (size_t)y * g + x];
  } else if (mode == 2) {
    const float inv = 1.f / (float)(g - 1);
    const float gx = sub_rn(mul_rn(add_rn(fx, (float)x * inv), 2.f), 1.f);
    const float gy = sub_rn(mul_rn(add_rn(fy, (float)y * inv), 2.f), 1.f);
    const float ix = ((gx + 1.f) * 0.5f) * (float)(g - 1), iy = ((gy + 1.f) * 0.5f) * (float)(g - 1);
    float x0f = floorf(ix), y0f = floorf(iy);
    const float wx1 = ix - x0f, wy1 = iy - y0f, wx0 = (x0f + 1.f) - ix, wy0 = (y0f + 1.f) - iy;
    x0f = fminf(fmaxf(x0f, -2.f), (float)g);
    y0f = fminf(fmaxf(y0f, -2.f), (float)g);
    if (!(ix == ix)) x0f = -2.f;
    if (!(iy == iy)) y0f = -2.f;
    const int x0 = (int)x0f, y0 = (int)y0f;
    const float wts[4] = {wx0 * wy0, wx1 * wy0, wx0 * wy1, wx1 * wy1};
#pragma unroll
    for (int k = 0; k < 4; ++k) {
      const int xx = x0 + (k & 1), yy = y0 + (k >> 1);
      if (xx >= 0 && xx < g && yy >= 0 && yy < g) {
        const floatx4 f = *(const floatx4*)(fd + ((size_t)yy * g + xx) * 256 + 4 * lane);
#pragma unroll
        for (int e = 0; e < 4; ++e) v[e] += f[e] * wts[k];
      }
    }
  }
#pragma unroll
  for (int e = 0; e < 4; ++e) orow[2 + 4 * lane + e] = (_Float16)v[e];
  if (lane == 0) {
    orow[0] = (_Float16)fx;
    orow[1] = (_Float16)fy;
  }
  if (pq == 3) {
    for (int c = 1032 + lane; c < ldo; c += 64) out[tokrow * ldo + c] = (_Float16)0.f;
  }
}

__global__ void __launch_bounds__(256) patch_rows_kernel(const float* __restrict__ in, long sn, long sc, long sy,
                                                         long sx, float* __restrict__ out, int ldo, int c, int g,
                                                         long total) {
  const long idx = (long)blockIdx.x * blockDim.x + threadIdx.x;
  if (idx >= total) return;
  const int k4 = 4 * c;
  const long row = idx / k4;
  const int col = (int)(idx % k4);
  const int pq = col / c, ch = col % c;
  const int side = g >> 1, T = side * side;
  const int n = (int)(row / T), t = (int)(row % T);
  const int y = 2 * (t / side) + (pq >> 1), x = 2 * (t % side) + (pq & 1);
  out[row * ldo + col] = in[n * sn + ch * sc + y * sy + x * sx];
}

__global__ void __launch_bounds__(256) dwconv3x3_kernel(const _Float16* __restrict__ in,
                                                        _Float16* __restrict__ out, const float* __restrict__ w,
                                                        const float* __restrict__ b, int side, int c, long total) {
  const long idx = (long)blockIdx.x * blockDim.x + threadIdx.x;
  if (idx >= total) return;
  const int c8 = c >> 3;
// ... 179 lines not shown
          const half8 (&row)[TX + 2] = R[(u + 1 + dy) & 3];
#pragma unroll
          for (int dx = -1; dx <= 1; ++dx) {
            const int t = (dy + 1) * 3 + (dx + 1);
#pragma unroll
            for (int k = 0; k < TX; ++k) {
              if (LEFT && k + dx < 0) continue;
              if (RIGHT && k + dx >= ncol) continue;
#pragma unroll
              for (int e = 0; e < 8; ++e) acc[k][e] = __builtin_fmaf((float)row[k + 1 + dx][e], wt[t][e], acc[k][e]);
            }
          }
        }
        _Float16* op = oimg + ((size_t)y * side + x0) * c;
#pragma unroll
        for (int k = 0; k < TX; ++k) {
          if (RIGHT && k >= ncol) continue;
          half8 o;
#pragma unroll
          for (int e = 0; e < 8; ++e) o[e] = (_Float16)fmaxf(acc[k][e], 0.f);
          if (NT) __builtin_nontemporal_store(o, (half8*)(op + (size_t)k * c));
          else *(half8*)(op + (size_t)k * c) = o;
        }
      }
    }
  }
}

template <int TX, bool NT>
__global__ void __launch_bounds__(256) dwconv3x3_strip_kernel(const _Float16* __restrict__ in, _Float16* __restrict__ out,
                                                              const float* __restrict__ w, const float* __restrict__ b, int side,
                                                              int c, int sy, int xstrips, int ybands, int nwaves) {
  int id = blockIdx.x;
  {
    const int nwg = gridDim.x, q = nwg / 8, rr = nwg % 8, xcd = id % 8, k = id / 8;
    id = (xcd < rr ? xcd * (q + 1) : rr * (q + 1) + (xcd - rr) * q) + k;
  }
  const int lane = threadIdx.x & 63;
  const int wid = __builtin_amdgcn_readfirstlane(id * 4 + (int)(threadIdx.x >> 6));
  if (wid >= nwaves) return;
  const int chunks = c >> 9;
  const int chunk = wid % chunks;
  int unit = wid / chunks;
  const int xs = unit % xstrips;
  unit /= xstrips;
  const int yb = unit % ybands;
  const int n = unit / ybands;
  const int x0 = xs * TX, y0 = yb * sy, y1 = min(y0 + sy, side);
  const int ch = chunk * 512 + lane * 8;
  const _Float16* img = in + (size_t)n * side * side * c + ch;
  _Float16* oimg = out + (size_t)n * side * side * c + ch;
  float wt[9][8], bs[8];
#pragma unroll
  for (int t = 0; t < 9; ++t) {
    const floatx4 w0 = *(const floatx4*)(w + t * c + ch), w1 = *(const floatx4*)(w + t * c + ch + 4);
#pragma unroll
    for (int e = 0; e < 4; ++e) { wt[t][e] = w0[e]; wt[t][4 + e] = w1[e]; }
  }
  {
    const floatx4 b0 = *(const floatx4*)(b + ch), b1 = *(const floatx4*)(b + ch + 4);
#pragma unroll
    for (int e = 0; e < 4; ++e) { bs[e] = b0[e]; bs[4 + e] = b1[e]; }
  }
  const bool left = x0 == 0, right = x0 + TX >= side;
  if (!left && !right) dwconv_strip<TX, NT, false, false>(img, oimg, wt, bs, side, c, x0, y0, y1);
  else if (left && !right) dwconv_strip<TX, NT, true, false>(img, oimg, wt, bs, side, c, x0, y0, y1);
  else if (!left) dwconv_strip<TX, NT, false, true>(img, oimg, wt, bs, side, c, x0, y0, y1);
  else dwconv_strip<TX, NT, true, true>(img, oimg, wt, bs, side, c, x0, y0, y1);
}

__global__ void __launch_bounds__(256) colsum_partial_kernel(const float* __restrict__ z, float* __restrict__ part,
                                                             int T, int c, int chunks) {
  const int n = blockIdx.z, chunk = blockIdx.y;
  const int col = blockIdx.x * 256 + threadIdx.x;
  if (col >= c) return;
  const int per = (T + chunks - 1) / chunks;
  const int t0 = chunk * per, t1 = min(T, t0 + per);
  const float* p = z + ((size_t)n * T + t0) * c + col;
  float s = 0.f;
  for (int t = t0; t < t1; ++t, p += c) s += *p;
  part[((size_t)n * chunks + chunk) * c + col] = s;
}

__global__ void __launch_bounds__(256) colmean_final_kernel(const float* __restrict__ part,
                                                            float* __restrict__ pooled, int T, int c, int chunks,
                                                            int total) {
  const int idx = blockIdx.x * 256 + threadIdx.x;
  if (idx >= total) return;
  const int n = idx / c, col = idx % c;
  float s = 0.f;
  for (int k = 0; k < chunks; ++k) s += part[((size_t)n * chunks + k) * c + col];
  pooled[idx] = s / (float)T;
}

__global__ void __launch_bounds__(256) posenc_add_kernel(float* __restrict__ z, const float* __restrict__ hs,
                                                         const float* __restrict__ ws,
                                                         const float* __restrict__ htab,
                                                         const float* __restrict__ wtab, int side, int c,
                                                         long total4) {
  const long idx = (long)blockIdx.x * blockDim.x + threadIdx.x;
  if (idx >= total4) return;
  const int c4 = c >> 2;
  const long tok = idx / c4;
  const int ch = (int)(idx % c4) * 4;
  const int T = side * side;
  const int n = (int)(tok / T), t = (int)(tok % T);
  const int ty = t / side, tx = t % side;
  floatx4 v = *(floatx4*)(z + tok * c + ch);
  const floatx4 a = *(const floatx4*)(hs + (size_t)n * c + ch), hb = *(const floatx4*)(htab + (size_t)ty * c + ch);
  const floatx4 b = *(const floatx4*)(ws + (size_t)n * c + ch), wb = *(const floatx4*)(wtab + (size_t)tx * c + ch);
#pragma unroll
  for (int e = 0; e < 4; ++e) v[e] = (v[e] + a[e] * hb[e]) + b[e] * wb[e];
  *(floatx4*)(z + tok * c + ch) = v;
}

__global__ void __launch_bounds__(256) small_linear_kernel(const float* __restrict__ x, int ldx,
                                                           const float* __restrict__ w,
                                                           const float* __restrict__ b, float* __restrict__ y,
                                                           int ldy, int M, int K, int N, int kmod, int act_in,
                                                           int act_out) {
  const int o = blockIdx.x * 4 + (threadIdx.x >> 6);
  if (o >= N) return;
  const int lane = threadIdx.x & 63;
  const float* wr = w + (size_t)o * K;
  for (int m0 = 8 * blockIdx.y; m0 < M; m0 += 8 * gridDim.y) {
    float acc[8];
#pragma unroll
    for (int j = 0; j < 8; ++j) acc[j] = 0.f;
    for (int k = lane; k < K; k += 64) {
      const float wv = wr[k];
      const int kk = k % kmod;
#pragma unroll
      for (int j = 0; j < 8; ++j) {
        if (m0 + j < M) {
          float xv;
          if (act_in == 2) {
            const int half = kmod >> 1;
            const float t = x[(m0 + j) * ldx];
            const int kf = kk < half ? kk : kk - half;
            const float fr = expf(-9.210340371976184f * (float)kf / (float)half);
            xv = kk < half ? cosf(t * fr) : sinf(t * fr);
          } else {
            xv = x[(size_t)(m0 + j) * ldx + kk];
            if (act_in == 1) xv = xv / (1.f + expf(-xv));
          }
          acc[j] += wv * xv;
        }
      }
    }
#pragma unroll
    for (int j = 0; j < 8; ++j) {
      const float s = wave_sum(acc[j]);
      if (lane == 0 && m0 + j < M) {
        float v = s + (b ? b[o] : 0.f);
        if (act_out == 1) v = v / (1.f + expf(-v));
        else if (act_out == 2) v = fmaxf(v, 0.f);
        else if (act_out == 3) v = 1.f / (1.f + expf(-v));
        y[(size_t)(m0 + j) * ldy + o] = v;
      }
    }
  }
}

__global__ void __launch_bounds__(256) final_tokens_kernel(const float* __restrict__ z,
                                                           const float* __restrict__ gamma,
                                                           const float* __restrict__ beta,
                                                           const float* __restrict__ shift,
                                                           const float* __restrict__ scale, int ldmod,
                                                           int mod_rows, const float* __restrict__ w,
                                                           const float* __restrict__ b,
                                                           const float* __restrict__ init_flow,
                                                           float* __restrict__ x0, float* __restrict__ tok8, int g,
                                                           long rows) {
  constexpr int C = 1536, PER = 24;
  const long row = (long)blockIdx.x * 4 + (threadIdx.x >> 6);
  if (row >= rows) return;
  const int lane = threadIdx.x & 63;
  const float* ip = z + row * C;
  float v[PER];
  float s = 0.f;
#pragma unroll
  for (int k = 0; k < 6; ++k) {
    const floatx4 f = *(const floatx4*)(ip + (k * 64 + lane) * 4);
#pragma unroll
    for (int e = 0; e < 4; ++e) {
      v[k * 4 + e] = f[e];
      s += f[e];
    }
  }
  float mean = wave_sum(s) * (1.f / C);
  float q2 = 0.f;
#pragma unroll
  for (int k = 0; k < PER; ++k) {
    const float d = v[k] - mean;
    q2 += d * d;
  }
  float rstd = rsqrtf(wave_sum(q2) * (1.f / C) + 1e-5f);
  s = 0.f;
#pragma unroll
  for (int k = 0; k < 6; ++k)
#pragma unroll
    for (int e = 0; e < 4; ++e) {
      const int c = (k * 64 + lane) * 4 + e;
      v[k * 4 + e] = (v[k * 4 + e] - mean) * rstd * gamma[c] + beta[c];
      s += v[k * 4 + e];
    }
  mean = wave_sum(s) * (1.f / C);
  q2 = 0.f;
#pragma unroll
  for (int k = 0; k < PER; ++k) {
    const float d = v[k] - mean;
    q2 += d * d;
  }
  rstd = rsqrtf(wave_sum(q2) * (1.f / C) + 1e-6f);
  const float* sh = shift + (row / mod_rows) * ldmod;
  const float* sc = scale + (row / mod_rows) * ldmod;
  float dot[8];
#pragma unroll
  for (int j = 0; j < 8; ++j) dot[j] = 0.f;
#pragma unroll
  for (int k = 0; k < 6; ++k)
#pragma unroll
    for (int e = 0; e < 4; ++e) {
      const int c = (k * 64 + lane) * 4 + e;
      const float y = ((v[k * 4 + e] - mean) * rstd) * (1.f + sc[c]) + sh[c];
#pragma unroll
      for (int j = 0; j < 8; ++j) dot[j] += y * w[j * C + c];
    }
#pragma unroll
  for (int j = 0; j < 8; ++j) dot[j] = wave_sum(dot[j]);
  if (lane < 8) {
    float o = 0.f;
#pragma unroll
    for (int j = 0; j < 8; ++j)
      if (lane == j) o = dot[j];
    o += b[lane];
    if (tok8) tok8[row * 8 + lane] = o;
    const int side = g >> 1, T = side * side;
    const int n = (int)(row / T), t = (int)(row % T);
    const int p = lane >> 2, q = (lane >> 1) & 1, c = lane & 1;
    const size_t at = (((size_t)n * 2 + c) * g + 2 * (t / side) + p) * g + 2 * (t % side) + q;
    x0[at] = o + (init_flow ? init_flow[at] : 0.f);
  }
}

}

using namespace dvd;

#define LAUNCH_ROWS(rows) cdiv((rows), 4), 256, 0, (hipStream_t)stream

extern "C" int dvd_embed_obs_ln(const float* x, const float* w, const float* bias, const float* pos, float* tok32,
                                void* ln16, int n, int g, void* stream) {
  DVD_REQUIRE(x && w && bias && pos && tok32 && ln16, "embed_obs_ln: null pointer");
  DVD_REQUIRE(n > 0 && g >= 2 && g % 2 == 0, "embed_obs_ln: bad shape");
  const long rows = (long)n * (g / 2) * (g / 2);
  embed_obs_ln_kernel<<<LAUNCH_ROWS(rows)>>>(x, w, bias, pos, tok32, (_Float16*)ln16, g, rows);
  return check_launch("embed_obs_ln");
}

extern "C" int dvd_layernorm_rows(const float* in, int ldin, long stride_in, void* out16, int ldout, long stride_out,
                                  int batch, long rows, int c, const float* gamma, const float* beta,
                                  const float* shift, const float* scale, int ldmod, int mod_rows, float eps,
                                  void* stream) {
  DVD_REQUIRE(in && out16, "layernorm_rows: null pointer");
  DVD_REQUIRE(c == 384 || c == 1536, "layernorm_rows: C=%d not in {384,1536}", c);
  DVD_REQUIRE((gamma == nullptr) == (beta == nullptr) && (shift == nullptr) == (scale == nullptr),
              "layernorm_rows: affine / modulate pointers must come in pairs");
  DVD_REQUIRE(!shift || mod_rows > 0, "layernorm_rows: mod_rows");
  DVD_REQUIRE(rows > 0 && batch > 0 && batch < 65536, "layernorm_rows: bad rows/batch");
  DVD_REQUIRE(ldin % 4 == 0 && stride_in % 2 == 0 && ldout % 4 == 0 && stride_out % 2 == 0 && ldmod % 4 == 0 &&
                  ((uintptr_t)in % 16) == 0 && ((uintptr_t)out16 % 8) == 0 && ((uintptr_t)gamma % 16) == 0 &&
                  ((uintptr_t)beta % 16) == 0 && ((uintptr_t)shift % 16) == 0 && ((uintptr_t)scale % 16) == 0,
              "layernorm_rows: rows must be 16-byte aligned (vector loads)");
  dim3 grid(cdiv(rows, 4), batch);
  if (c == 384)
    layernorm_rows_kernel<384><<<grid, 256, 0, (hipStream_t)stream>>>(in, ldin, stride_in, (_Float16*)out16, ldout,
                                                                       stride_out, gamma, beta, shift, scale, ldmod,
                                                                       mod_rows > 0 ? mod_rows : 1, eps, rows);
  else
    layernorm_rows_kernel<1536><<<grid, 256, 0, (hipStream_t)stream>>>(in, ldin, stride_in, (_Float16*)out16, ldout,
                                                                        stride_out, gamma, beta, shift, scale, ldmod,
                                                                        mod_rows > 0 ? mod_rows : 1, eps, rows);
  return check_launch("layernorm_rows");
}

extern "C" int dvd_build_r_rows(const float* feat_nhwc, const float* init_feat_nchw, const float* flow, void* out16,
                                int ldo, int n, int g, int n_hyp, int mode, void* stream) {
  DVD_REQUIRE(feat_nhwc && flow && out16, "build_r_rows: null pointer");
  DVD_REQUIRE(ldo >= 1032 && n > 0 && g >= 2 && g % 2 == 0 && n_hyp > 0 && mode >= 0 && mode <= 3,
              "build_r_rows: bad arguments");
  DVD_REQUIRE(mode != 3 || init_feat_nchw, "build_r_rows: mode 3 needs init_feat");
  const long items = (long)n * (g / 2) * (g / 2) * 4;
  build_r_rows_kernel<<<LAUNCH_ROWS(items)>>>(feat_nhwc, init_feat_nchw, flow, (_Float16*)out16, ldo, g, n_hyp, mode,
                                              items);
  return check_launch("build_r_rows");
}

extern "C" int dvd_patch_rows(const float* in, long sn, long sc, long sy, long sx, float* out, int ldo, int n, int c,
                              int g, void* stream) {
  DVD_REQUIRE(in && out, "patch_rows: null pointer");
  DVD_REQUIRE(n > 0 && c > 0 && g >= 2 && g % 2 == 0 && ldo >= 4 * c, "patch_rows: bad shape");
  const long total = (long)n * (g / 2) * (g / 2) * 4 * c;
  patch_rows_kernel<<<cdiv(total, 256), 256, 0, (hipStream_t)stream>>>(in, sn, sc, sy, sx, out, ldo, c, g, total);
  return check_launch("patch_rows");
}

extern "C" int dvd_dwconv3x3(const void* in16, void* out16, const float* w9c, const float* b, int n, int side, int c,
                             void* stream) {
  DVD_REQUIRE(in16 && out16 && w9c && b, "dwconv3x3: null pointer");
  DVD_REQUIRE(n > 0 && side > 0 && c % 8 == 0, "dwconv3x3: bad shape");
#ifdef DVD_LAB
  if (getenv("DVD_DWCONV_V1")) {
    const long total1 = (long)n * side * side * (c / 8);
    dwconv3x3_kernel<<<cdiv(total1, 256), 256, 0, (hipStream_t)stream>>>((const _Float16*)in16, (_Float16*)out16, w9c, b,
                                                                         side, c, total1);
    return check_launch("dwconv3x3(lab v1)");
  }
#endif
  int stx = (c % 512 == 0 && (long)n * side * side >= 16384) ? 3 : 0, ssy = 24;
  bool snt = true;
  (void)snt;
#ifdef DVD_LAB
  if (getenv("DVD_DWCONV_TY") || getenv("DVD_DWCONV_TX")) stx = 0;
  if (const char* e = getenv("DVD_DWCONV_STRIP")) stx = (c % 512 == 0) ? atoi(e) : 0;
  if (const char* e = getenv("DVD_DWCONV_SY")) ssy = atoi(e);
  if (const char* e = getenv("DVD_DWCONV_NT")) snt = atoi(e) != 0;
#endif
  if (stx >= 2 && stx <= 4 && ssy >= 1) {
    const int xstrips = cdiv(side, stx), ybands = cdiv(side, ssy);
    const int nwaves = n * ybands * xstrips * (c / 512);
    const dim3 g(cdiv(nwaves, 4));
#define DW_STRIP(TX_, NT_) dwconv3x3_strip_kernel<TX_, NT_><<<g, 256, 0, (hipStream_t)stream>>>((const _Float16*)in16, (_Float16*)out16, w9c, b, side, c, ssy, xstrips, ybands, nwaves)
#ifdef DVD_LAB
    if (stx == 2) { if (snt) DW_STRIP(2, true); else DW_STRIP(2, false); }
    else if (stx == 4) { if (snt) DW_STRIP(4, true); else DW_STRIP(4, false); }
    else if (!snt) DW_STRIP(3, false);
    else
#endif
    DW_STRIP(3, true);
#undef DW_STRIP
    return check_launch("dwconv3x3(strip)");
  }
  int ty = DW_TY_P, tx = DW_TX_P;
#ifdef DVD_LAB
  if (const char* e = getenv("DVD_DWCONV_TY")) ty = atoi(e);
  if (const char* e = getenv("DVD_DWCONV_TX")) tx = atoi(e);
#endif
  const long total = (long)n * cdiv(side, ty) * cdiv(side, tx) * (c / 8);
  const dim3 grd(cdiv(total, 256));
#define DW_LAUNCH(TX_, TY_) dwconv3x3_tile_kernel<TX_, TY_><<<grd, 256, 0, (hipStream_t)stream>>>((const _Float16*)in16, (_Float16*)out16, w9c, b, side, c, total)
#ifdef DVD_LAB
  if (tx == 2 && ty == 2) DW_LAUNCH(2, 2);
  else if (tx == 2 && ty == 4) DW_LAUNCH(2, 4);
  else if (tx == 2 && ty == 8) DW_LAUNCH(2, 8);
  else if (tx == 1 && ty == 4) DW_LAUNCH(1, 4);
  else if (tx == 1 && ty == 8) DW_LAUNCH(1, 8);
  else if (tx == 2) DW_LAUNCH(2, 1);
  else if (ty == 1) DW_LAUNCH(4, 1);
  else if (ty == 4) DW_LAUNCH(4, 4);
  else
#endif
  DW_LAUNCH(DW_TX_P, DW_TY_P);
#undef DW_LAUNCH
  return check_launch("dwconv3x3");
}

extern "C" int dvd_colmean(const float* z, float* partial, float* pooled, int n, int t, int c, int chunks,
                           void* stream) {
  DVD_REQUIRE(z && partial && pooled, "colmean: null pointer");
  DVD_REQUIRE(n > 0 && n < 65536 && t > 0 && c > 0 && chunks > 0 && chunks < 65536, "colmean: bad shape");
  dim3 grid(cdiv(c, 256), chunks, n);
  colsum_partial_kernel<<<grid, 256, 0, (hipStream_t)stream>>>(z, partial, t, c, chunks);
  colmean_final_kernel<<<cdiv((long)n * c, 256), 256, 0, (hipStream_t)stream>>>(partial, pooled, t, c, chunks, n * c);
  return check_launch("colmean");
}

extern "C" int dvd_posenc_add(float* z, const float* hs, const float* ws, const float* htab, const float* wtab,
                              int n, int side, int c, void* stream) {
  DVD_REQUIRE(z && hs && ws && htab && wtab, "posenc_add: null pointer");
  DVD_REQUIRE(n > 0 && side > 0 && c % 4 == 0, "posenc_add: bad shape");
  const long total4 = (long)n * side * side * (c / 4);
  posenc_add_kernel<<<cdiv(total4, 256), 256, 0, (hipStream_t)stream>>>(z, hs, ws, htab, wtab, side, c, total4);
  return check_launch("posenc_add");
}

extern "C" int dvd_small_linear(const float* x, int ldx, const float* w, const float* b, float* y, int ldy, int m,
                                int k, int n, int kmod, int act_in, int act_out, void* stream) {
  DVD_REQUIRE(x && w && y, "small_linear: null pointer");
  DVD_REQUIRE(m > 0 && k > 0 && n > 0 && kmod > 0 && act_in >= 0 && act_in <= 2 && act_out >= 0 && act_out <= 3,
              "small_linear: bad arguments");
  small_linear_kernel<<<dim3(cdiv(n, 4), cdiv(m, 8)), 256, 0, (hipStream_t)stream>>>(x, ldx, w, b, y, ldy, m, k, n, kmod, act_in,
                                                                                       act_out);
  return check_launch("small_linear");
}

extern "C" int dvd_final_tokens(const float* z, const float* gamma, const float* beta, const float* shift,
                                const float* scale, int ldmod, int mod_rows, const float* w8, const float* b8,
                                const float* init_flow, float* x0, float* tok8, int n, int g, void* stream) {
  DVD_REQUIRE(z && gamma && beta && shift && scale && w8 && b8 && x0, "final_tokens: null pointer");
  DVD_REQUIRE(n > 0 && g >= 2 && g % 2 == 0 && mod_rows > 0, "final_tokens: bad shape");
  const long rows = (long)n * (g / 2) * (g / 2);
  final_tokens_kernel<<<LAUNCH_ROWS(rows)>>>(z, gamma, beta, shift, scale, ldmod, mod_rows, w8, b8, init_flow, x0,
                                             tok8, g, rows);
  return check_launch("final_tokens");
}
```

dvd_amd/lib.py:

```python
from __future__ import annotations

import ctypes as C
import os

import torch

_HERE = os.path.dirname(os.path.abspath(__file__))
LIB_PATH = os.path.join(_HERE, "libdvd_hip.so")


class DvdError(RuntimeError):
    pass


def _load():
    if not os.path.exists(LIB_PATH):
        raise DvdError(
            f"{LIB_PATH} is missing: build it with `python -c 'import __graft_entry__ as g; g.build()'` "
            "or `make -C dvd_amd/csrc`.  The DvD engine has no non-HIP fallback.")
    return C.CDLL(LIB_PATH)


_lib = _load()

c_f32p = C.POINTER(C.c_float)
c_void = C.c_void_p


class SchedCoef(C.Structure):
    _fields_ = [("kind", C.c_int), ("c_recip", C.c_float), ("c_recipm1", C.c_float),
                ("sqrt_abar_prev", C.c_float), ("dir_coef", C.c_float), ("coef1", C.c_float),
                ("coef2", C.c_float), ("sigma", C.c_float)]


class GemmDesc(C.Structure):
    _fields_ = [("dtype", C.c_int), ("M", C.c_int), ("N", C.c_int), ("K", C.c_int), ("batch", C.c_int),
                ("A", C.c_void_p), ("lda", C.c_int), ("strideA", C.c_long),
                ("B", C.c_void_p), ("ldb", C.c_int), ("strideB", C.c_long),
                ("B_lo", C.c_void_p), ("A_lo", C.c_void_p), ("lo_scale", C.c_float),
                ("C32", C.c_void_p), ("ldc", C.c_int), ("strideC32", C.c_long),
                ("C16", C.c_void_p), ("ldc16", C.c_int), ("strideC16", C.c_long),
                ("bias", C.c_void_p), ("bias_row", C.c_int), ("strideBias", C.c_long),
                ("act", C.c_int),
                ("pos", C.c_void_p), ("ldpos", C.c_int), ("pos_rows", C.c_int),
                ("gate", C.c_void_p), ("ldgate", C.c_int), ("gate_rows", C.c_int), ("strideGate", C.c_long),
                ("res", C.c_void_p), ("ldres", C.c_int), ("strideRes", C.c_long), ("small_tiles", C.c_int)]


class AttnDesc(C.Structure):
    _fields_ = [("head_dim", C.c_int), ("heads", C.c_int), ("batch", C.c_int), ("tq", C.c_int), ("tk", C.c_int),
                ("kv_batch_div", C.c_int),
                ("Q", C.c_void_p), ("ldq", C.c_int), ("strideQ", C.c_long),
                ("K", C.c_void_p), ("ldk", C.c_int), ("strideK", C.c_long),
                ("Vt", C.c_void_p), ("ldvt", C.c_int), ("strideVt", C.c_long),
                ("O", C.c_void_p), ("ldo", C.c_int), ("strideO", C.c_long),
                ("scale", C.c_float)]


class CnOp(C.Structure):
    _fields_ = [("op", C.c_int), ("a", C.c_int), ("b", C.c_int), ("dst", C.c_int), ("ks", C.c_int), ("dil", C.c_int),
                ("cout", C.c_int), ("act", C.c_int), ("w_off", C.c_long), ("h", C.c_int), ("w", C.c_int),
                ("flag", C.c_int)]


class RaggedImage(C.Structure):
    _fields_ = [("src", C.c_void_p), ("out", C.c_void_p), ("h", C.c_int), ("w", C.c_int)]


SSIM_REPLICATE, SSIM_VALID = 0, 1
MSSSIM_DOCUNET, MSSSIM_WANG = 0, 1

PNG_SEGMENT = 32768
PNG_HUFFMAN_FIXED, PNG_HUFFMAN_DYNAMIC = 0, 1

JPEG_420, JPEG_444 = 0, 1


class JpegDecInfo(C.Structure):
    _fields_ = [("h", C.c_int), ("w", C.c_int), ("out_h", C.c_int), ("out_w", C.c_int), ("components", C.c_int),
                ("hs", C.c_int), ("vs", C.c_int), ("orientation", C.c_int), ("restart_interval", C.c_int),
                ("scan_offset", C.c_long), ("scan_bytes", C.c_long), ("blocks", C.c_long), ("scratch_bytes", C.c_long)]


JPEG_DECODE_CODES = {-20: "HEADER", -21: "PROGRESSIVE", -22: "EXTENDED", -23: "LOSSLESS", -24: "ARITHMETIC", -25: "PRECISION",
                     -26: "COMPONENTS", -27: "ADOBE", -28: "SAMPLING", -29: "SCANS", -30: "QUANT16", -31: "TABLE", -32: "SIZE",
                     -33: "ORIENTATION", -34: "NOSYNC", -35: "DATA"}
JPEGDEC_SUBSEQ = 128

class SflowParams(C.Structure):
    _fields_ = [(name, C.c_int) for name in ("levels", "w_top", "w", "iters_top", "iters", "alpha", "d", "gamma", "T", "eps")]


SFLOW_DEFAULTS = dict(levels=4, w_top=10, w=2, iters_top=60, iters=30, alpha=510, d=10200, gamma=1, T=8160, eps=1 << 17)
SFLOW_MIN_TOP = 12

RAGGED_CAP = 64

NON_STATUS = {"dvd_last_error", "dvd_version", "dvd_engine_workspace_bytes", "dvd_engine_tensor_count",
              "dvd_flash_attn_kernel_name", "dvd_gemm_kernel_name", "dvd_convnet_workspace_bytes", "dvd_convnet_weight_floats",
              "dvd_ingest_scratch_bytes", "dvd_ingest_ragged_scratch_bytes", "dvd_resize_gray_scratch_bytes",
              "dvd_msssim_workspace_bytes", "dvd_png_bound", "dvd_png_scratch_bytes", "dvd_png_scratch_bytes_huff", "dvd_jpeg_bound",
              "dvd_jpeg_scratch_bytes", "dvd_sflow_level_workspace_bytes", "dvd_sflow_workspace_bytes"}

SIGNATURES = {
    "dvd_grid_sample_bilinear_zeros_ac": [c_void, c_void, c_void, C.c_int, C.c_int, C.c_int, C.c_int, C.c_int,
                                          C.c_int, C.c_int, c_void],
    "dvd_unwarp_f32": [c_void, C.c_int, c_void, c_void, C.c_int, C.c_int, C.c_float, c_void],
    "dvd_unwarp_u8": [c_void, C.c_int, c_void, c_void, C.c_int, C.c_int, C.c_float, c_void],
    "dvd_unwarp_f32_batch": [c_void, C.c_int, c_void, c_void, C.c_int, C.c_int, C.c_int, C.c_float, c_void],
    "dvd_unwarp_u8_batch": [c_void, C.c_int, c_void, c_void, C.c_int, C.c_int, C.c_int, C.c_float, c_void],
    "dvd_unwarp_grid": [c_void, C.c_int, c_void, C.c_int, C.c_int, C.c_float, c_void],
    "dvd_unwarp_u8_ragged": [c_void, C.c_int, C.POINTER(RaggedImage), C.c_int, C.c_float, c_void],
    "dvd_grid_sample_bicubic_zeros_ac": [c_void, c_void, c_void, C.c_int, C.c_int, C.c_int, C.c_int, C.c_int,
                                         C.c_int, C.c_int, c_void],
    "dvd_unwarp_u8_bicubic_batch": [c_void, C.c_int, c_void, c_void, C.c_int, C.c_int, C.c_int, C.c_float, c_void],
    "dvd_unwarp_u8_bicubic_ragged": [c_void, C.c_int, C.POINTER(RaggedImage), C.c_int, C.c_float, c_void],
    "dvd_sched_step": [C.POINTER(SchedCoef), c_void, c_void, c_void, c_void, c_void, C.c_int, C.c_int, c_void],
    "dvd_sched_step_clip": [C.POINTER(SchedCoef), c_void, c_void, c_void, c_void, c_void, C.c_int, C.c_int, c_void],
    "dvd_hyp_mean_clamp": [c_void, c_void, C.c_int, C.c_int, C.c_int, c_void],
    "dvd_selftest_mfma": [c_void, c_void, c_void, c_void, c_void],
    "dvd_gemm_nt": [C.POINTER(GemmDesc), c_void],
    "dvd_gemm_kernel_name": [C.POINTER(GemmDesc)],
    "dvd_flash_attn": [C.POINTER(AttnDesc), c_void],
    "dvd_embed_obs_ln": [c_void, c_void, c_void, c_void, c_void, c_void, C.c_int, C.c_int, c_void],
    "dvd_layernorm_rows": [c_void, C.c_int, C.c_long, c_void, C.c_int, C.c_long, C.c_int, C.c_long, C.c_int, c_void,
                           c_void, c_void, c_void, C.c_int, C.c_int, C.c_float, c_void],
    "dvd_build_r_rows": [c_void, c_void, c_void, c_void, C.c_int, C.c_int, C.c_int, C.c_int, C.c_int, c_void],
    "dvd_patch_rows": [c_void, C.c_long, C.c_long, C.c_long, C.c_long, c_void, C.c_int, C.c_int, C.c_int, C.c_int,
                       c_void],
    "dvd_dwconv3x3": [c_void, c_void, c_void, c_void, C.c_int, C.c_int, C.c_int, c_void],
    "dvd_colmean": [c_void, c_void, c_void, C.c_int, C.c_int, C.c_int, C.c_int, c_void],
    "dvd_posenc_add": [c_void, c_void, c_void, c_void, c_void, C.c_int, C.c_int, C.c_int, c_void],
    "dvd_small_linear": [c_void, C.c_int, c_void, c_void, c_void, C.c_int, C.c_int, C.c_int, C.c_int, C.c_int, C.c_int,
                         C.c_int, c_void],
    "dvd_final_tokens": [c_void, c_void, c_void, c_void, c_void, C.c_int, C.c_int, c_void, c_void, c_void, c_void,
                         c_void, C.c_int, C.c_int, c_void],
    "dvd_im2col3x3": [c_void, C.c_long, C.c_long, C.c_long, c_void, C.c_int, C.c_int, C.c_int, C.c_int, c_void],
    "dvd_conv3x3_nhwc": [c_void, C.c_int, c_void, C.c_int, c_void, c_void, C.c_int, C.c_int, C.c_int, C.c_int, c_void],
    "dvd_maxpool2_nhwc": [c_void, c_void, C.c_int, C.c_int, C.c_int, c_void],
    "dvd_resize_bilinear_nhwc": [c_void, c_void, C.c_int, C.c_int, C.c_int, C.c_int, C.c_int, c_void],
    "dvd_nhwc_to_nchw": [c_void, c_void, C.c_int, C.c_int, C.c_int, c_void],
    "dvd_convnet_create": [C.POINTER(CnOp), C.c_int, C.c_int, C.c_int, C.c_int, C.c_int, C.POINTER(c_void)],
    "dvd_convnet_create_batched": [C.POINTER(CnOp), C.c_int, C.c_int, C.c_int, C.c_int, C.c_int, C.c_int, C.POINTER(c_void)],
    "dvd_convnet_destroy": [c_void],
    "dvd_convnet_slot_shape": [c_void, C.c_int, C.POINTER(C.c_int), C.POINTER(C.c_int), C.POINTER(C.c_int)],
    "dvd_convnet_run": [c_void, c_void, c_void, c_void, C.c_long, C.c_int, C.POINTER(C.c_int), C.POINTER(c_void), c_void],
    "dvd_resize_bilinear_nchw": [c_void, c_void, C.c_long, C.c_int, C.c_int, C.c_int, C.c_int, C.c_int, c_void],
    "dvd_threshold_mask_mul": [c_void, c_void, c_void, c_void, C.c_int, C.c_long, C.c_float, c_void],
    "dvd_threshold_mask_mul_batch": [c_void, c_void, c_void, c_void, C.c_int, C.c_int, C.c_long, C.c_float, c_void],
    "dvd_flash_attn_f32": [C.POINTER(AttnDesc), c_void],
    "dvd_layernorm256_f32": [c_void, c_void, C.c_long, c_void, c_void, C.c_float, c_void],
    "dvd_add_rows_f32": [c_void, c_void, c_void, C.c_long, C.c_int, C.c_int, c_void],
    "dvd_transpose_f32": [c_void, c_void, C.c_int, C.c_int, C.c_int, c_void],
    "dvd_soft_mask_mul_batch": [c_void, c_void, c_void, C.c_int, C.c_int, C.c_long, c_void],
    "dvd_convex_upsample": [c_void, c_void, C.c_int, C.c_int, C.c_int, c_void, c_void, C.c_int, C.c_float, c_void],
    "dvd_ingest_u8": [c_void, C.c_int, C.c_int, C.c_int, c_void, C.c_int, c_void, c_void, c_void],
    "dvd_ingest_ragged_scratch_bytes": [C.c_int, C.c_int],
    "dvd_ingest_u8_ragged": [C.POINTER(RaggedImage), C.c_int, C.c_int, c_void, C.c_int, c_void, c_void],
    "dvd_resize_gray_scratch_bytes": [C.c_int, C.c_int, C.c_int, C.c_int],
    "dvd_resize_gray_u8": [c_void, C.c_int, C.c_int, C.c_int, c_void, C.c_int, C.c_int, c_void, c_void],
    "dvd_ssim_scale": [c_void, c_void, C.c_int, C.c_int, C.c_int, C.c_int, c_void, c_void],
    "dvd_ssim_finalize": [c_void, C.c_int, C.c_int, C.c_long, c_void, C.c_int, c_void],
    "dvd_reduce2_pair": [c_void, c_void, c_void, c_void, C.c_int, C.c_int, C.c_int, C.c_int, c_void],
    "dvd_msssim_workspace_bytes": [C.c_int, C.c_int, C.c_int],
    "dvd_msssim_scales": [c_void, c_void, C.c_int, C.c_int, C.c_int, C.c_int, c_void, c_void, c_void],
    "dvd_dsift_u8": [c_void, C.c_int, C.c_int, C.c_int, C.c_int, c_void, c_void],
    "dvd_sflow_cost": [c_void, c_void, c_void, C.c_int, C.c_int, C.c_int, C.POINTER(SflowParams), c_void, c_void],
    "dvd_sflow_level_workspace_bytes": [C.c_int, C.c_int, C.c_int],
    "dvd_sflow_level": [c_void, c_void, c_void, C.c_int, C.c_int, C.c_int, C.c_int, C.POINTER(SflowParams), c_void, c_void, c_void,
                        c_void],
    "dvd_sflow_workspace_bytes": [C.c_int, C.c_int, C.POINTER(SflowParams)],
    "dvd_sflow": [c_void, c_void, C.c_int, C.c_int, C.c_int, C.POINTER(SflowParams), c_void, c_void, c_void, c_void],
    "dvd_png_bound": [C.c_int, C.c_int],
    "dvd_png_scratch_bytes": [C.c_int, C.c_int],
    "dvd_png_encode_rgb8": [c_void, C.c_int, C.c_int, c_void, C.c_long, c_void, c_void, c_void],
    "dvd_png_scratch_bytes_huff": [C.c_int, C.c_int, C.c_int],
    "dvd_png_encode_rgb8_huff": [c_void, C.c_int, C.c_int, c_void, C.c_long, c_void, c_void, C.c_int, c_void],
    "dvd_jpeg_bound": [C.c_int, C.c_int, C.c_int],
    "dvd_jpeg_scratch_bytes": [C.c_int, C.c_int, C.c_int],
    "dvd_jpeg_encode_rgb8": [c_void, C.c_int, C.c_int, C.c_int, C.c_int, c_void, C.c_long, c_void, c_void, c_void],
    "dvd_jpegdec_probe": [c_void, C.c_long, C.POINTER(JpegDecInfo)],
    "dvd_jpeg_decode_rgb8": [c_void, c_void, C.c_long, c_void, C.c_long, C.c_int, C.POINTER(C.c_int), c_void, c_void],
    "dvd_dither_f16": [c_void, c_void, c_void, C.c_long, C.c_uint, C.c_uint, c_void],
    "dvd_engine_create": [C.c_int, C.c_int, C.c_int, C.POINTER(c_void)],
    "dvd_engine_destroy": [c_void],
    "dvd_engine_bind_workspace": [c_void, c_void, C.c_long],
    "dvd_engine_tensor_count": [c_void],
    "dvd_engine_tensor_info": [c_void, C.c_int, C.POINTER(C.c_char_p), C.POINTER(C.c_int), C.POINTER(C.c_long)],
    "dvd_engine_set_tensor": [c_void, C.c_char_p, c_void, C.c_long],
    "dvd_engine_prepare_docs": [c_void, c_void, c_void, c_void, c_void, c_void],
    "dvd_engine_feat_nchw": [c_void, c_void, c_void],
    "dvd_engine_denoise_step": [c_void, c_void, C.c_float, C.c_int, c_void, c_void, c_void, c_void],
    "dvd_engine_debug_buffer": [c_void, C.c_char_p, C.POINTER(c_void), C.POINTER(C.c_long)],
    "dvd_engine_debug_stop": [c_void, C.c_int],
    "dvd_engine_set_option": [c_void, C.c_char_p, C.c_int],
    "dvd_engine_profile": [c_void, C.c_int],
    "dvd_engine_profile_read": [c_void, C.POINTER(C.c_int), C.POINTER(C.c_double)],
}


RESTYPES = {"dvd_gemm_kernel_name": C.c_char_p, "dvd_ingest_ragged_scratch_bytes": C.c_long,
            "dvd_resize_gray_scratch_bytes": C.c_long, "dvd_msssim_workspace_bytes": C.c_long,
            "dvd_sflow_level_workspace_bytes": C.c_long, "dvd_sflow_workspace_bytes": C.c_long,
            "dvd_png_bound": C.c_long, "dvd_png_scratch_bytes": C.c_long, "dvd_png_scratch_bytes_huff": C.c_long,
            "dvd_jpeg_bound": C.c_long, "dvd_jpeg_scratch_bytes": C.c_long}

LAB_SIGNATURES = {"dvd_gemm_debug_stamps": [c_void], "dvd_attn_debug_stamps": [c_void]}


def bind(cdll):
    cdll.dvd_last_error.restype = C.c_char_p
    cdll.dvd_version.restype = C.c_int
    cdll.dvd_engine_workspace_bytes.restype = C.c_long
    cdll.dvd_engine_workspace_bytes.argtypes = [C.c_void_p]
    for fn in (cdll.dvd_convnet_workspace_bytes, cdll.dvd_convnet_weight_floats):
        fn.restype, fn.argtypes = C.c_long, [C.c_void_p]
    cdll.dvd_ingest_scratch_bytes.restype, cdll.dvd_ingest_scratch_bytes.argtypes = C.c_long, [C.c_int]
    cdll.dvd_flash_attn_kernel_name.restype = C.c_char_p
    cdll.dvd_flash_attn_kernel_name.argtypes = [C.c_int, C.c_int, C.c_int]
    for name, args in SIGNATURES.items():
        fn = getattr(cdll, name)
        fn.argtypes, fn.restype = args, RESTYPES.get(name, C.c_int)
    for name, args in LAB_SIGNATURES.items():
        if hasattr(cdll, name):
            fn = getattr(cdll, name)
            fn.argtypes, fn.restype = args, C.c_int
    return cdll


bind(_lib)


def use_library(path: str):
    global _lib
    _lib = bind(C.CDLL(os.path.abspath(path)))
    return _lib


def call(name: str, *args):
    rc = getattr(_lib, name)(*args)
    if rc != 0:
        raise DvdError(f"{name} failed ({rc}): {_lib.dvd_last_error().decode()}")


def flash_attn_kernel_name(head_dim: int, tq: int, tk: int) -> str:
    return _lib.dvd_flash_attn_kernel_name(head_dim, tq, tk).decode()


def gemm_kernel_name(desc: GemmDesc) -> str:
    return _lib.dvd_gemm_kernel_name(C.byref(desc)).decode()


def version() -> int:
    return int(_lib.dvd_version())


def raw():
    return _lib


def ptr(t):
    return None if t is None else C.c_void_p(t.data_ptr())


def stream_ptr():
    import torch
    return C.c_void_p(torch.cuda.current_stream().cuda_stream)
```

dvd_amd/ops.py:

```python
from __future__ import annotations

import ctypes as C
import os

import numpy as np
import torch

from . import lib
from .lib import ptr, stream_ptr


def _chk(t: torch.Tensor, dtype, name):
    if not t.is_cuda:
        raise lib.DvdError(f"{name}: expected a device tensor (the DvD engine has no CPU path)")
    if t.dtype != dtype or not t.is_contiguous():
        raise lib.DvdError(f"{name}: expected contiguous {dtype}, got {t.dtype} contiguous={t.is_contiguous()}")


_WARP_MODES = ("bilinear", "bicubic")


def _warp_mode(mode, name):
    if mode not in _WARP_MODES:
        raise ValueError(f"{name}: mode must be 'bilinear' or 'bicubic', got {mode!r}")
# ... 144 lines not shown
    if clip and x0.data_ptr() in (x_t.data_ptr(), out.data_ptr(), None if noise is None else noise.data_ptr()):
        raise lib.DvdError("sched_step(clip=True) updates x0 in place: it must not share memory with x_t, noise or out")
    lib.call("dvd_sched_step_clip" if clip else "dvd_sched_step", C.byref(coef), ptr(x_t), ptr(x0), ptr(noise), ptr(out),
             ptr(ngrid), n, g, stream_ptr())
    return (out, ngrid) if want_grid else out


def hyp_mean_clamp(x0: torch.Tensor, n_hyp: int) -> torch.Tensor:
    _chk(x0, torch.float32, "x0")
    n, _, g, _ = x0.shape
    docs = n // n_hyp
    out = torch.empty((docs, 2, g, g), dtype=torch.float32, device=x0.device)
    lib.call("dvd_hyp_mean_clamp", ptr(x0), ptr(out), docs, n_hyp, g, stream_ptr())
    return out


def dither_f16(hi: torch.Tensor, lo: torch.Tensor, step: int, elem0: int = 0, out=None) -> torch.Tensor:
    _chk(hi, torch.float16, "hi")
    _chk(lo, torch.float16, "lo")
    if out is None:
        out = torch.empty_like(hi)
    lib.call("dvd_dither_f16", ptr(hi), ptr(lo), ptr(out), hi.numel(), C.c_uint(elem0 & 0xFFFFFFFF),
             C.c_uint(step & 0xFFFFFFFF), stream_ptr())
    return out


def selftest_mfma(a16, b16, vt16):
    out = torch.empty(3072, dtype=torch.float32, device=a16.device)
    lib.call("dvd_selftest_mfma", ptr(a16), ptr(b16), ptr(vt16), ptr(out), stream_ptr())
    return out


def _addr(t):
    return None if t is None else t.data_ptr()


def gemm_nt(a, b, *, out32=None, out16=None, bias=None, bias_row=False, act=0, pos=None, gate=None,
            gate_rows=0, res=None, batch=1, strides=None, M=None, N=None, K=None, lda=None, ldb=None, b_lo=None,
            a_lo=None, lo_scale=2.0 ** -11, small_tiles=False):
    assert a.dtype == b.dtype and a.dtype in (torch.float16, torch.float32)
    d = lib.GemmDesc()
    d.dtype = 1 if a.dtype == torch.float32 else 0
    d.M = M if M is not None else a.shape[-2]
    d.N = N if N is not None else b.shape[-2]
    d.K = K if K is not None else a.shape[-1]
    d.batch = batch
    st = strides or {}
    d.A, d.lda, d.strideA = _addr(a), (lda if lda is not None else a.stride(-2)), st.get("A", 0)
    d.B, d.ldb, d.strideB = _addr(b), (ldb if ldb is not None else b.stride(-2)), st.get("B", 0)
    if b_lo is not None:
        d.B_lo, d.lo_scale = _addr(b_lo), lo_scale
    if a_lo is not None:
        d.A_lo, d.lo_scale = _addr(a_lo), lo_scale
    if out32 is not None:
        d.C32, d.ldc, d.strideC32 = _addr(out32), out32.stride(-2), st.get("C32", 0)
    if out16 is not None:
        d.C16, d.ldc16, d.strideC16 = _addr(out16), out16.stride(-2), st.get("C16", 0)
    if bias is not None:
        d.bias, d.bias_row, d.strideBias = _addr(bias), int(bias_row), st.get("bias", 0)
    d.act = act
    if pos is not None:
        d.pos, d.ldpos, d.pos_rows = _addr(pos), pos.stride(-2), pos.shape[-2]
    if gate is not None:
        d.gate, d.ldgate, d.gate_rows, d.strideGate = _addr(gate), gate.stride(-2), gate_rows, st.get("gate", 0)
    if res is not None:
        d.res, d.ldres, d.strideRes = _addr(res), res.stride(-2), st.get("res", 0)
    d.small_tiles = int(small_tiles)
    lib.call("dvd_gemm_nt", C.byref(d), stream_ptr())


def flash_attn(q, k, vt, out, heads, head_dim, scale, kv_batch_div=1):
    d = lib.AttnDesc()
    d.head_dim, d.heads, d.batch, d.tq, d.tk = head_dim, heads, q.shape[0], q.shape[1], k.shape[1]
    d.kv_batch_div = kv_batch_div
    d.Q, d.ldq, d.strideQ = q.data_ptr(), q.stride(1), q.stride(0)
    d.K, d.ldk, d.strideK = k.data_ptr(), k.stride(1), k.stride(0)
    d.Vt, d.ldvt, d.strideVt = vt.data_ptr(), vt.stride(1), vt.stride(0)
    d.O, d.ldo, d.strideO = out.data_ptr(), out.stride(1), out.stride(0)
    d.scale = scale
    lib.call("dvd_flash_attn", C.byref(d), stream_ptr())
    return out


def layernorm_rows(x, c, gamma=None, beta=None, shift=None, scale=None, mod_rows=1, eps=1e-6):
    rows = x.shape[0]
    out = torch.empty(rows, c, dtype=torch.float16, device=x.device)
    lib.call("dvd_layernorm_rows", ptr(x), x.stride(0), 0, ptr(out), c, 0, 1, rows, c, ptr(gamma), ptr(beta), ptr(shift),
             ptr(scale), (shift.stride(0) if shift is not None and shift.dim() > 1 else 0), mod_rows, C.c_float(eps),
             stream_ptr())
    return out


def dwconv3x3(x16, w9c, b, n, side):
    out = torch.empty_like(x16)
    lib.call("dvd_dwconv3x3", ptr(x16), ptr(out), ptr(w9c), ptr(b), n, side, x16.shape[-1], stream_ptr())
    return out


def embed_obs_ln(x, w, b, pos):
    n, _, g, _ = x.shape
    T = (g // 2) ** 2
    tok = torch.empty(n * T, 384, dtype=torch.float32, device=x.device)
    ln = torch.empty(n * T, 384, dtype=torch.float16, device=x.device)
    lib.call("dvd_embed_obs_ln", ptr(x), ptr(w), ptr(b), ptr(pos), ptr(tok), ptr(ln), n, g, stream_ptr())
    return tok, ln


def small_linear(x, w, b, act_in=0, act_out=0, kmod=None):
    m = x.shape[0]
    n, k = w.shape
    y = torch.empty(m, n, dtype=torch.float32, device=x.device)
    lib.call("dvd_small_linear", ptr(x), x.stride(0), ptr(w), ptr(b), ptr(y), n, m, k, n, kmod or k, act_in, act_out,
             stream_ptr())
    return y


def final_tokens(z, gamma, beta, shift, scale, w8, b8, init_flow, n, g):
    x0 = torch.empty(n, 2, g, g, dtype=torch.float32, device=z.device)
    tok8 = torch.empty(z.shape[0], 8, dtype=torch.float32, device=z.device)
    lib.call("dvd_final_tokens", ptr(z), ptr(gamma), ptr(beta), ptr(shift), ptr(scale), 0, z.shape[0], ptr(w8), ptr(b8),
             ptr(init_flow), ptr(x0), ptr(tok8), n, g, stream_ptr())
    return x0, tok8


def posenc(z, hs, ws, htab, wtab, n, side):
    c = z.shape[-1]
    chunks = 8
    part = torch.empty(n * chunks * c, dtype=torch.float32, device=z.device)
    pooled = torch.empty(n, c, dtype=torch.float32, device=z.device)
    lib.call("dvd_colmean", ptr(z), ptr(part), ptr(pooled), n, side * side, c, chunks, stream_ptr())
    lib.call("dvd_posenc_add", ptr(z), ptr(hs), ptr(ws), ptr(htab), ptr(wtab), n, side, c, stream_ptr())
    return pooled


def build_r_rows(feat_nhwc, flow, n_hyp, mode, init_feat=None):
    n, _, g, _ = flow.shape
    T = (g // 2) ** 2
    out = torch.empty(n * T, 1088, dtype=torch.float16, device=flow.device)
    lib.call("dvd_build_r_rows", ptr(feat_nhwc), ptr(init_feat), ptr(flow), ptr(out), 1088, n, g, n_hyp, mode, stream_ptr())
    return out


def conv3x3_relu_nhwc(x_nhwc, w_packed, bias, cin, cout, h, w):
    kp = w_packed.shape[1]
    col = torch.empty(h * w, kp, dtype=torch.float32, device=x_nhwc.device)
    lib.call("dvd_im2col3x3", ptr(x_nhwc), 1, w * cin, cin, ptr(col), kp, cin, h, w, stream_ptr())
    out = torch.empty(h * w, cout, dtype=torch.float32, device=x_nhwc.device)
    gemm_nt(col, w_packed, out32=out, bias=bias, act=2)
    return out


def conv3x3_relu_nhwc_implicit(x_nhwc, w_packed, bias, cin, cout, h, w):
    out = torch.empty(h * w, cout, dtype=torch.float32, device=x_nhwc.device)
    lib.call("dvd_conv3x3_nhwc", ptr(x_nhwc), cin, ptr(w_packed), w_packed.shape[1], ptr(bias), ptr(out), cout, h, w, 1,
             stream_ptr())
    return out


def maxpool2_nhwc(x, c, h, w):
    out = torch.empty((h // 2) * (w // 2), c, dtype=torch.float32, device=x.device)
    lib.call("dvd_maxpool2_nhwc", ptr(x), ptr(out), c, h, w, stream_ptr())
    return out


def resize_bilinear_nhwc(x, c, hin, win, hout, wout):
    out = torch.empty(hout * wout, c, dtype=torch.float32, device=x.device)
# ... 443 lines not shown
```

include/dvd_hip.h:

```cpp
#ifndef DVD_HIP_H
#define DVD_HIP_H

#include <stddef.h>
#include <stdint.h>

#ifdef __cplusplus
extern "C" {
#endif

#define DVD_OK 0
#define DVD_E_ARG (-1)
#define DVD_E_LAUNCH (-2)
#define DVD_E_STATE (-3)

const char* dvd_last_error(void);
int dvd_version(void);


int dvd_grid_sample_bilinear_zeros_ac(const float* src, const float* grid, float* out,
                                      int n, int c, int hin, int win, int h, int w,
                                      int src_batch_div, void* stream);

int dvd_unwarp_f32(const float* flow, int g, const float* src_chw, float* out_hwc,
                   int h, int w, float scale, void* stream);
int dvd_unwarp_u8(const float* flow, int g, const uint8_t* src_hwc, uint8_t* out_hwc,
                  int h, int w, float scale, void* stream);
int dvd_unwarp_f32_batch(const float* flow, int g, const float* src_chw, float* out_hwc,
                         int n, int h, int w, float scale, void* stream);
int dvd_unwarp_u8_batch(const float* flow, int g, const uint8_t* src_hwc, uint8_t* out_hwc,
                        int n, int h, int w, float scale, void* stream);
#define DVD_RAGGED_CAP 64
typedef struct {
  const uint8_t* src;
  uint8_t* out;
  int h, w;
} dvd_ragged_image;
int dvd_unwarp_u8_ragged(const float* flow, int g, const dvd_ragged_image* docs, int n, float scale, void* stream);
int dvd_unwarp_grid(const float* flow, int g, float* grid_out, int h, int w, float scale, void* stream);

int dvd_grid_sample_bicubic_zeros_ac(const float* src, const float* grid, float* out,
                                     int n, int c, int hin, int win, int h, int w,
                                     int src_batch_div, void* stream);
int dvd_unwarp_u8_bicubic_batch(const float* flow, int g, const uint8_t* src_hwc, uint8_t* out_hwc,
                                int n, int h, int w, float scale, void* stream);
int dvd_unwarp_u8_bicubic_ragged(const float* flow, int g, const dvd_ragged_image* docs, int n, float scale, void* stream);

typedef struct {
  int kind;
  float c_recip;
  float c_recipm1;
  float sqrt_abar_prev;
  float dir_coef;
  float coef1;
  float coef2;
  float sigma;
} dvd_sched_coef;

int dvd_sched_step(const dvd_sched_coef* coef, const float* x_t, const float* x0, const float* noise,
                   float* x_prev, float* next_grid, int n, int g, void* stream);

int dvd_sched_step_clip(const dvd_sched_coef* coef, const float* x_t, float* x0, const float* noise,
                        float* x_prev, float* next_grid, int n, int g, void* stream);

int dvd_hyp_mean_clamp(const float* x0, float* out, int docs, int n_hyp, int g, void* stream);

typedef struct {
  int dtype;
  int M, N, K, batch;
  const void* A; int lda; long strideA;
  const void* B; int ldb; long strideB;
  const void* B_lo; const void* A_lo; float lo_scale;
  float* C32; int ldc; long strideC32;
  void* C16; int ldc16; long strideC16;
  const float* bias; int bias_row; long strideBias;
  int act;
  const float* pos; int ldpos; int pos_rows;
  const float* gate; int ldgate; int gate_rows; long strideGate;
  const float* res; int ldres; long strideRes;
  int small_tiles;
} dvd_gemm_desc;

int dvd_gemm_nt(const dvd_gemm_desc* desc, void* stream);
const char* dvd_gemm_kernel_name(const dvd_gemm_desc* desc);

typedef struct {
  int head_dim, heads, batch, tq, tk, kv_batch_div;
  const void* Q; int ldq; long strideQ;
  const void* K; int ldk; long strideK;
  const void* Vt; int ldvt; long strideVt;
  void* O; int ldo; long strideO;
  float scale;
} dvd_attn_desc;

int dvd_flash_attn(const dvd_attn_desc* desc, void* stream);
const char* dvd_flash_attn_kernel_name(int head_dim, int tq, int tk);


int dvd_embed_obs_ln(const float* x, const float* w, const float* bias, const float* pos, float* tok32,
                     void* ln16, int n, int g, void* stream);

int dvd_layernorm_rows(const float* in, int ldin, long stride_in, void* out16, int ldout, long stride_out,
                       int batch, long rows, int c, const float* gamma, const float* beta, const float* shift,
                       const float* scale, int ldmod, int mod_rows, float eps, void* stream);

int dvd_build_r_rows(const float* feat_nhwc, const float* init_feat_nchw, const float* flow, void* out16, int ldo,
                     int n, int g, int n_hyp, int mode, void* stream);

int dvd_patch_rows(const float* in, long sn, long sc, long sy, long sx, float* out, int ldo, int n, int c, int g,
                   void* stream);

int dvd_dwconv3x3(const void* in16, void* out16, const float* w9c, const float* b, int n, int side, int c,
                  void* stream);

int dvd_colmean(const float* z, float* partial, float* pooled, int n, int t, int c, int chunks, void* stream);
int dvd_posenc_add(float* z, const float* hs, const float* ws, const float* htab, const float* wtab, int n, int side,
                   int c, void* stream);

int dvd_small_linear(const float* x, int ldx, const float* w, const float* b, float* y, int ldy, int m, int k, int n,
                     int kmod, int act_in, int act_out, void* stream);

int dvd_final_tokens(const float* z, const float* gamma, const float* beta, const float* shift, const float* scale,
                     int ldmod, int mod_rows, const float* w8, const float* b8, const float* init_flow, float* x0,
                     float* tok8, int n, int g, void* stream);

int dvd_im2col3x3(const float* in, long sc, long sy, long sx, float* out, int ldo, int c, int h, int w, void* stream);
int dvd_conv3x3_nhwc(const float* in, int c, const float* wgt, int kp, const float* bias, float* out, int cout, int h, int w,
                     int relu, void* stream);
int dvd_maxpool2_nhwc(const float* in, float* out, int c, int h, int w, void* stream);
int dvd_resize_bilinear_nhwc(const float* in, float* out, int c, int hin, int win, int hout, int wout, void* stream);
int dvd_nhwc_to_nchw(const float* in, float* out, int c, int h, int w, void* stream);

enum { DVD_CN_CONV = 0, DVD_CN_POOL = 1, DVD_CN_RESIZE = 2, DVD_CN_ADD = 3, DVD_CN_SIGMOID = 4, DVD_CN_INSTNORM = 5 };
typedef struct {
  int op;
  int a, b;
  int dst;
  int ks, dil;
  int cout, act;
  long w_off;
  int h, w;
  int flag;
} dvd_cn_op;

int dvd_convnet_create(const dvd_cn_op* ops, int n_ops, int n_slots, int in_c, int in_h, int in_w, void** handle);
int dvd_convnet_create_batched(const dvd_cn_op* ops, int n_ops, int n_slots, int in_c, int in_h, int in_w, int batch,
                               void** handle);
int dvd_convnet_destroy(void* handle);
long dvd_convnet_workspace_bytes(void* handle);
long dvd_convnet_weight_floats(void* handle);
int dvd_convnet_slot_shape(void* handle, int slot, int* h, int* w, int* c);
int dvd_convnet_run(void* handle, const float* in_nchw, const float* weights, void* workspace, long workspace_bytes,
                    int n_out, const int* out_slots, float* const* out_nchw, void* stream);
int dvd_resize_bilinear_nchw(const float* in, float* out, long planes, int hin, int win, int hout, int wout,
                             int align_corners, void* stream);
int dvd_threshold_mask_mul(const float* d0, const float* x_nchw, float* out_nchw, float* mask_out, int c, long hw,
                           float thr, void* stream);
int dvd_threshold_mask_mul_batch(const float* d0, const float* x_nchw, float* out_nchw, float* mask_out, int n, int c,
                                 long hw, float thr, void* stream);

int dvd_flash_attn_f32(const dvd_attn_desc* desc, void* stream);
int dvd_layernorm256_f32(const float* in, float* out, long rows, const float* gamma, const float* beta, float eps,
                         void* stream);
int dvd_add_rows_f32(const float* a, const float* pos, float* out, long rows, int pos_rows, int c, void* stream);
int dvd_transpose_f32(const float* in, float* out, int n, int rows, int cols, void* stream);
int dvd_soft_mask_mul_batch(const float* msk, const float* x_nchw, float* out_nchw, int n, int c, long hw, void* stream);
int dvd_convex_upsample(const float* mask, const float* dflow, int n, int h, int w, float* bm, float* init_flow, int g,
                        float norm, void* stream);

long dvd_ingest_scratch_bytes(int out_size);
int dvd_ingest_u8(const uint8_t* src_hwc, int h, int w, int swap_rb, float* y_chw, int out_size,
                  uint8_t* rgb_hwc_out, void* scratch, void* stream);

long dvd_ingest_ragged_scratch_bytes(int out_size, int n);
int dvd_ingest_u8_ragged(const dvd_ragged_image* docs, int n, int swap_rb, float* y_nchw, int out_size, void* scratch,
                         void* stream);

int dvd_dither_f16(const void* hi, const void* lo, void* out, long nelem, unsigned elem0, unsigned step, void* stream);

int dvd_engine_create(int grid, int docs, int n_hyp, void** handle);
int dvd_engine_destroy(void* handle);
long dvd_engine_workspace_bytes(void* handle);
int dvd_engine_bind_workspace(void* handle, void* workspace, long bytes);
int dvd_engine_tensor_count(void* handle);
int dvd_engine_tensor_info(void* handle, int index, const char** name, int* dtype , long* nelem);
int dvd_engine_set_tensor(void* handle, const char* name, const void* dev_ptr, long nelem);
int dvd_engine_set_option(void* handle, const char* name, int value);
int dvd_engine_prepare_docs(void* handle, const float* y512, const float* mask_cat, const float* mask_y512,
                            const float* line_msk, void* stream);
int dvd_engine_feat_nchw(void* handle, float* out, void* stream);
int dvd_engine_denoise_step(void* handle, const float* x_t, float t_embed, int feat_mode, const float* init_flow,
                            const float* init_feat_nchw , float* x0_out, void* stream);
int dvd_engine_profile(void* handle, int enable);
int dvd_engine_profile_read(void* handle, int* launches, double* total_ms);
int dvd_engine_debug_buffer(void* handle, const char* name, void** ptr, long* bytes);
int dvd_engine_debug_stop(void* handle, int stage);

int dvd_selftest_mfma(const void* a16, const void* b16, const void* vt16, float* out3072, void* stream);

#define DVD_SSIM_REPLICATE 0
#define DVD_SSIM_VALID 1
#define DVD_MSSSIM_DOCUNET 0
#define DVD_MSSSIM_WANG 1
long dvd_resize_gray_scratch_bytes(int h, int w, int out_h, int out_w);
int dvd_resize_gray_u8(const uint8_t* src_nhwc, int n, int h, int w, float* out, int out_h, int out_w,
                       void* scratch, void* stream);
int dvd_ssim_scale(const float* x, const float* y, int n, int h, int w, int border, double* partials, void* stream);
int dvd_ssim_finalize(const double* partials, int n, int tiles, long count, float* out_n52, int scale, void* stream);
int dvd_reduce2_pair(const float* x, const float* y, float* x_out, float* y_out, int n, int h, int w, int taps,
                     void* stream);
long dvd_msssim_workspace_bytes(int h, int w, int n);
int dvd_msssim_scales(const float* x, const float* y, int n, int h, int w, int preset, void* workspace,
                      float* out_n52, void* stream);

#define DVD_PNG_SEGMENT 32768
#define DVD_PNG_HUFFMAN_FIXED 0
#define DVD_PNG_HUFFMAN_DYNAMIC 1
long dvd_png_bound(int h, int w);
long dvd_png_scratch_bytes(int h, int w);
int dvd_png_encode_rgb8(const uint8_t* img_hwc, int h, int w, uint8_t* out, long cap, unsigned long long* out_len,
                        void* scratch, void* stream);
long dvd_png_scratch_bytes_huff(int h, int w, int huffman);
int dvd_png_encode_rgb8_huff(const uint8_t* img_hwc, int h, int w, uint8_t* out, long cap, unsigned long long* out_len,
                             void* scratch, int huffman, void* stream);

#define DVD_JPEG_420 0
#define DVD_JPEG_444 1
long dvd_jpeg_bound(int h, int w, int subsampling);
long dvd_jpeg_scratch_bytes(int h, int w, int subsampling);
int dvd_jpeg_encode_rgb8(const uint8_t* img_hwc, int h, int w, int quality, int subsampling, uint8_t* out, long cap,
                         unsigned long long* out_len, void* scratch, void* stream);

#define DVD_E_JPEG_HEADER (-20)
#define DVD_E_JPEG_PROGRESSIVE (-21)
#define DVD_E_JPEG_EXTENDED (-22)
#define DVD_E_JPEG_LOSSLESS (-23)
#define DVD_E_JPEG_ARITHMETIC (-24)
#define DVD_E_JPEG_PRECISION (-25)
#define DVD_E_JPEG_COMPONENTS (-26)
#define DVD_E_JPEG_ADOBE (-27)
#define DVD_E_JPEG_SAMPLING (-28)
#define DVD_E_JPEG_SCANS (-29)
#define DVD_E_JPEG_QUANT16 (-30)
#define DVD_E_JPEG_TABLE (-31)
#define DVD_E_JPEG_SIZE (-32)
#define DVD_E_JPEG_ORIENTATION (-33)
#define DVD_E_JPEG_NOSYNC (-34)
#define DVD_E_JPEG_DATA (-35)
#define DVD_JPEGDEC_SUBSEQ 128
typedef struct dvd_jpegdec_info {
  int h, w;
  int out_h, out_w;
  int components;
  int hs, vs;
  int orientation;
  int restart_interval;
  long scan_offset;
  long scan_bytes;
  long blocks;
  long scratch_bytes;
} dvd_jpegdec_info;
// ... 32 lines not shown
```

Before: 0.4870.

## Fuse multi-group attention, dither segments, and glue kernels into fewer launches

```diff
diff --git a/dvd_amd/csrc/attention.hip b/dvd_amd/csrc/attention.hip
--- a/dvd_amd/csrc/attention.hip
+++ b/dvd_amd/csrc/attention.hip
@@ -1,6 +1,7 @@
 #include "common.h"
 #include "mfma.h"
 #include <stdlib.h>
+#include <string.h>
 
 #ifndef DVD_ATTN64_OCC
 #define DVD_ATTN64_OCC 2
@@ -13,6 +14,15 @@
 #endif
 
 namespace dvd {
+
+struct AttnGroup {
+  const _Float16* K;
+  const _Float16* Vt;
+  _Float16* O;
+  long sK, sVt, sO;
+  int kv_div, pad;
+};
+constexpr int ATTN_MAX_GROUPS = 4;
 
 struct AttnArgs {
   const _Float16* Q;
@@ -27,6 +37,8 @@
   float c;
   unsigned long long* stamps;
   int xcd_map;
+  int ngroups, gwg;
+  AttnGroup grp[ATTN_MAX_GROUPS];
 };
 
 __device__ __forceinline__ int kappa(int r) {
@@ -1459,17 +1471,28 @@
     const int q = nwg / 8, rr = nwg % 8, xcd = id % 8, k = id / 8;
     id = (xcd < rr ? xcd * (q + 1) : rr * (q + 1) + (xcd - rr) * q) + k;
   }
+  const _Float16 *Kp = p.K, *Vtp = p.Vt;
+  _Float16* Op = p.O;
+  long sK = p.sK, sVt = p.sVt, sO = p.sO;
+  int kv_div = p.kv_div;
+  if (p.ngroups > 1) {
+    int gi = 0;
+    while (gi < p.ngroups - 1 && id >= p.gwg) { id -= p.gwg; ++gi; }
+    Kp = p.grp[gi].K; Vtp = p.grp[gi].Vt; Op = p.grp[gi].O;
+    sK = p.grp[gi].sK; sVt = p.grp[gi].sVt; sO = p.grp[gi].sO;
+    kv_div = p.grp[gi].kv_div;
+  }
   const int qb = id % p.nqb;
   const int bh = id / p.nqb;
   const int head = bh % p.heads, b = bh / p.heads;
-  const int kvb = b / p.kv_div;
+  const int kvb = b / kv_div;
   const int tid = threadIdx.x, lane = tid & 63;
   const int wave = __builtin_amdgcn_readfirstlane(tid >> 6);
   const int c16 = lane & 15, g = lane >> 4;
 
   const _Float16* Qg = p.Q + b * p.sQ + (size_t)head * D;
-  const char* Kg = (const char*)(p.K + kvb * p.sK + (size_t)head * D);
-  const char* Vg = (const char*)(p.Vt + kvb * p.sVt + (size_t)head * D * p.ldvt);
+  const char* Kg = (const char*)(Kp + kvb * sK + (size_t)head * D);
+  const char* Vg = (const char*)(Vtp + kvb * sVt + (size_t)head * D * p.ldvt);
   {
     const int qrow = qb * 256 + wave * 64 + c16;
     const unsigned rowb = (unsigned)(p.ldq * 2);
@@ -1555,7 +1578,7 @@
     const float inv = 1.f / lt;
     const int qglob = qb * 256 + wave * 64 + 16 * q + c16e;
     if (qglob < p.tq) {
-      _Float16* op = p.O + b * p.sO + (size_t)qglob * p.ldo + (size_t)head * D + 4 * ge;
+      _Float16* op = Op + b * sO + (size_t)qglob * p.ldo + (size_t)head * D + 4 * ge;
       floatx16 x;
       if (q == 0) x = r64m_read_o<0>();
       else if (q == 1) x = r64m_read_o<16>();
@@ -1616,6 +1639,22 @@
 template <typename KernelT>
 static void allow_lds(KernelT kernel, int bytes) {
   (void)hipFuncSetAttribute((const void*)kernel, hipFuncAttributeMaxDynamicSharedMemorySize, bytes);
+}
+
+static bool attn_setup_device() {
+  static DeviceOnce attr_done;
+  const unsigned long long dev_bit = DeviceOnce::current_bit();
+  const bool first_on_device = attr_done.need(dev_bit);
+  if (first_on_device) {
+    for (int hd : {256, 64})
+      for (bool f : {false, true})
+        for (bool r : {false, true}) {
+          const AttnKernel k = attn_kernel(hd, f, r);
+          allow_lds(k.fn, k.lds);
+        }
+    attr_done.done(dev_bit);
+  }
+  return first_on_device;
 }
 
 extern "C" int dvd_flash_attn(const dvd_attn_desc* d, void* stream) {
@@ -1629,6 +1668,7 @@
                   ((uintptr_t)d->O % 8) == 0,
               "flash_attn: operands must be 16-byte aligned");
   AttnArgs p;
+  memset(&p, 0, sizeof(p));
   p.Q = (const _Float16*)d->Q; p.K = (const _Float16*)d->K; p.Vt = (const _Float16*)d->Vt; p.O = (_Float16*)d->O;
   p.sQ = d->strideQ; p.sK = d->strideK; p.sVt = d->strideVt; p.sO = d->strideO;
   p.ldq = d->ldq; p.ldk = d->ldk; p.ldvt = d->ldvt; p.ldo = d->ldo;
@@ -1642,18 +1682,8 @@
   DVD_REQUIRE(nwg < (1l << 31), "flash_attn: grid too large");
   hipStream_t st = (hipStream_t)stream;
   bool fast = attn_fast(d->tk), r64 = attn_r64(d->tq);
-  static DeviceOnce attr_done;
-  const unsigned long long dev_bit = DeviceOnce::current_bit();
-  const bool first_on_device = attr_done.need(dev_bit);
-  if (first_on_device) {
-    for (int hd : {256, 64})
-      for (bool f : {false, true})
-        for (bool r : {false, true}) {
-          const AttnKernel k = attn_kernel(hd, f, r);
-          allow_lds(k.fn, k.lds);
-        }
-    attr_done.done(dev_bit);
-  }
+  const bool first_on_device = attn_setup_device();
+  (void)first_on_device;
 #ifdef DVD_LAB
   p.stamps = g_attn_stamps;
   if (const char* xm = getenv("DVD_ATTN_XCDMAP")) p.xcd_map = atoi(xm);
@@ -1795,3 +1825,50 @@
   k.fn<<<(unsigned)((long)p.nqb * d->heads * d->batch), 256, k.lds, st>>>(p);
   return check_launch("flash_attn");
 }
+
+extern "C" int dvd_flash_attn_multi(const dvd_attn_desc* d, const dvd_attn_group* groups, int ngroups, void* stream) {
+  DVD_REQUIRE(d && groups && d->Q, "flash_attn_multi: null pointer");
+  DVD_REQUIRE(ngroups >= 1 && ngroups <= ATTN_MAX_GROUPS, "flash_attn_multi: ngroups=%d not in 1..%d", ngroups, ATTN_MAX_GROUPS);
+  DVD_REQUIRE(d->head_dim == 64 || d->head_dim == 256, "flash_attn_multi: head_dim %d not in {64,256}", d->head_dim);
+  DVD_REQUIRE(d->heads > 0 && d->batch > 0 && d->tq > 0 && d->tk > 0, "flash_attn_multi: bad shape");
+  const bool one_grid = ngroups > 1 && d->head_dim == 64 && attn_fast(d->tk) && attn_r64(d->tq);
+  if (!one_grid) {
+    for (int g = 0; g < ngroups; ++g) {
+      dvd_attn_desc one = *d;
+      one.K = groups[g].K; one.strideK = groups[g].strideK;
+      one.Vt = groups[g].Vt; one.strideVt = groups[g].strideVt;
+      one.O = groups[g].O; one.strideO = groups[g].strideO;
+      one.kv_batch_div = groups[g].kv_batch_div;
+      const int rc = dvd_flash_attn(&one, stream);
+      if (rc) return rc;
+    }
+    return DVD_OK;
+  }
+  DVD_REQUIRE(d->tk % 8 == 0 && d->ldq % 8 == 0 && d->ldk % 8 == 0 && d->ldvt % 8 == 0 && d->ldo % 4 == 0 && d->strideQ % 8 == 0 &&
+                  ((uintptr_t)d->Q % 16) == 0,
+              "flash_attn_multi: operands must be 16-byte aligned");
+  AttnArgs p;
+  memset(&p, 0, sizeof(p));
+  for (int g = 0; g < ngroups; ++g) {
+    const dvd_attn_group& s = groups[g];
+    DVD_REQUIRE(s.K && s.Vt && s.O && s.kv_batch_div > 0, "flash_attn_multi: group %d: null pointer or kv_batch_div", g);
+    DVD_REQUIRE(s.strideK % 8 == 0 && s.strideVt % 8 == 0 && s.strideO % 4 == 0 && ((uintptr_t)s.K % 16) == 0 &&
+                    ((uintptr_t)s.Vt % 16) == 0 && ((uintptr_t)s.O % 8) == 0,
+                "flash_attn_multi: group %d: operands must be 16-byte aligned", g);
+    p.grp[g] = {(const _Float16*)s.K, (const _Float16*)s.Vt, (_Float16*)s.O, s.strideK, s.strideVt, s.strideO, s.kv_batch_div, 0};
+  }
+  p.Q = (const _Float16*)d->Q; p.K = p.grp[0].K; p.Vt = p.grp[0].Vt; p.O = p.grp[0].O;
+  p.sQ = d->strideQ; p.sK = p.grp[0].sK; p.sVt = p.grp[0].sVt; p.sO = p.grp[0].sO;
+  p.ldq = d->ldq; p.ldk = d->ldk; p.ldvt = d->ldvt; p.ldo = d->ldo;
+  p.heads = d->heads; p.batch = d->batch; p.tq = d->tq; p.tk = d->tk;
+  p.kv_div = p.grp[0].kv_div;
+  p.c = d->scale * 1.4426950408889634f;
+  const AttnKernel k = attn_select(d->head_dim, d->tq, d->tk);
+  p.nqb = cdiv(d->tq, k.rows);
+  const long gwg = (long)p.nqb * d->heads * d->batch;
+  DVD_REQUIRE(gwg * ngroups < (1l << 31), "flash_attn_multi: grid too large");
+  p.ngroups = ngroups; p.gwg = (int)gwg;
+  (void)attn_setup_device();
+  k.fn<<<(unsigned)(gwg * ngroups), 256, k.lds, (hipStream_t)stream>>>(p);
+  return check_launch("flash_attn_multi");
+}
diff --git a/dvd_amd/csrc/dither.hip b/dvd_amd/csrc/dither.hip
--- a/dvd_amd/csrc/dither.hip
+++ b/dvd_amd/csrc/dither.hip
@@ -42,6 +42,28 @@
   out[i] = make_uint4(ow[0], ow[1], ow[2], ow[3]);
 }
 
+constexpr int DITHER_MAX_SEGS = 64;
+__global__ void __launch_bounds__(256) dither_f16_table_kernel(const dvd_dither_seg* __restrict__ segs, int nseg, unsigned phase) {
+  const int lane = threadIdx.x & 63;
+  const unsigned b0 = lane < nseg ? segs[lane].block0 : 0xffffffffu;
+  const int s = __builtin_amdgcn_readfirstlane(__popcll(__ballot(blockIdx.x >= b0)) - 1);
+  const dvd_dither_seg sg = segs[s];
+  const long n8 = sg.nelem / 8;
+  const long i = (long)(blockIdx.x - sg.block0) * 256 + threadIdx.x;
+  if (i >= n8) return;
+  const uint4 h = ((const uint4*)sg.hi)[i], l = ((const uint4*)sg.lo)[i];
+  const unsigned hw[4] = {h.x, h.y, h.z, h.w}, lw[4] = {l.x, l.y, l.z, l.w};
+  unsigned ow[4];
+  const unsigned g0 = sg.elem0 + (unsigned)(i * 8);
+#pragma unroll
+  for (int k = 0; k < 4; ++k) {
+    const unsigned short a = dither_one((unsigned short)(hw[k] & 0xffffu), (unsigned short)(lw[k] & 0xffffu), g0 + 2 * k, phase);
+    const unsigned short b = dither_one((unsigned short)(hw[k] >> 16), (unsigned short)(lw[k] >> 16), g0 + 2 * k + 1, phase);
+    ow[k] = (unsigned)a | ((unsigned)b << 16);
+  }
+  ((uint4*)sg.out)[i] = make_uint4(ow[0], ow[1], ow[2], ow[3]);
+}
+
 }
 
 using namespace dvd;
@@ -58,3 +80,23 @@
                                                                                    (uint4*)out, n8, elem0, phase);
   return check_launch("dither_f16");
 }
+
+extern "C" long dvd_dither_table_fill(dvd_dither_seg* segs, int nseg) {
+  if (!segs || nseg <= 0 || nseg > DITHER_MAX_SEGS) return -1;
+  long blocks = 0;
+  for (int i = 0; i < nseg; ++i) {
+    if (segs[i].nelem <= 0 || segs[i].nelem % 8 != 0 || blocks >= (1l << 31)) return -1;
+    segs[i].block0 = (unsigned)blocks;
+    blocks += (segs[i].nelem / 8 + 255) / 256;
+  }
+  return blocks < (1l << 31) ? blocks : -1;
+}
+
+extern "C" int dvd_dither_f16_table(const dvd_dither_seg* segs_dev, int nseg, long blocks, unsigned step, void* stream) {
+  DVD_REQUIRE(segs_dev, "dither_f16_table: null pointer");
+  DVD_REQUIRE(nseg > 0 && nseg <= DITHER_MAX_SEGS && blocks > 0 && blocks < (1l << 31),
+              "dither_f16_table: nseg=%d (1..%d) / blocks=%ld", nseg, DITHER_MAX_SEGS, blocks);
+  const unsigned phase = step * 0x9E3779B9u;
+  dither_f16_table_kernel<<<(unsigned)blocks, 256, 0, (hipStream_t)stream>>>(segs_dev, nseg, phase);
+  return check_launch("dither_f16_table");
+}
diff --git a/dvd_amd/csrc/engine.hip b/dvd_amd/csrc/engine.hip
--- a/dvd_amd/csrc/engine.hip
+++ b/dvd_amd/csrc/engine.hip
@@ -26,6 +26,15 @@
 int dvd_resize_bilinear_nhwc(const float*, float*, int, int, int, int, int, void*);
 int dvd_nhwc_to_nchw(const float*, float*, int, int, int, void*);
 int dvd_dither_f16(const void*, const void*, void*, long, unsigned, unsigned, void*);
+long dvd_dither_table_fill(dvd_dither_seg*, int);
+int dvd_dither_f16_table(const dvd_dither_seg*, int, long, unsigned, void*);
+int dvd_layernorm_rows_form(const float*, int, long, void*, int, long, int, long, int, const float*, const float*,
+                            const float*, const float*, int, int, float, int, void*);
+int dvd_colmean_form(const float*, float*, float*, int, int, int, int, int, void*);
+int dvd_posenc_add_ln(float*, const float*, const float*, const float*, const float*, void*, const float*, const float*,
+                      float, int, int, int, void*);
+int dvd_final_tokens_form(const float*, const float*, const float*, const float*, const float*, int, int, const float*,
+                          const float*, const float*, float*, float*, int, int, int, void*);
 }
 
 namespace dvd {
@@ -77,6 +86,8 @@
   X(tbuf, 256) X(th, HID * 4) X(cvec, HID * 4) X(mod, 6 * HID * 4) X(finmod, 2 * DEC * 4)                          \
   X(pooled, N * DEC * 4) X(petmp, N * DEC * 4) X(hs, N * DEC * 4) X(wsc, N * DEC * 4)                              \
   X(part, N * COLCHUNKS * DEC * 4)                                                                                 \
+   \
+  X(dithtab, 64 * sizeof(dvd_dither_seg))                                                                          \
       \
   X(w16dith, dith_bytes)                                                                                           \
                                                                                          \
@@ -156,12 +167,16 @@
   bool prepared = false;
   bool split_weights = true;
   bool ffn_lo = true;
+  bool fused_glue = true;
   bool small_tiles = false;
   bool dither = false;
   unsigned dither_step = 0;
   std::vector<long> dith_off;
   std::vector<int> dith_list;
   long dith_total = 0;
+  std::vector<dvd_dither_seg> dith_segs;
+  long dith_blocks = 0;
+  bool dith_dirty = true;
   bool use_graphs = false;
   bool prof_on = false;
   std::vector<hipEvent_t> prof_ev;
@@ -296,6 +311,28 @@
 };
 
 static int attn(const Attn& d, void* stream) { return dvd_flash_attn(&d, stream); }
+
+static int attn_multi(const Attn& d, const dvd_attn_group* g, int n, void* stream) { return dvd_flash_attn_multi(&d, g, n, stream); }
+
+static int layernorm_rows_form0(const float* in, int ldin, long sin, void* out, int ldout, long sout, int batch, long rows, int c,
+                                const float* shift, const float* scale, int ldmod, int mod_rows, float eps, void* stream) {
+  return dvd_layernorm_rows_form(in, ldin, sin, out, ldout, sout, batch, rows, c, nullptr, nullptr, shift, scale, ldmod, mod_rows, eps, 0,
+                                 stream);
+}
+static int colmean_form0(const float* z, float* part, float* pooled, int n, int t, int c, int chunks, void* stream) {
+  return dvd_colmean_form(z, part, pooled, n, t, c, chunks, 0, stream);
+}
+static int posenc_add_ln(float* z, const float* hs, const float* ws, const float* htab, const float* wtab, void* out16,
+                         const float* gamma, const float* beta, float eps, int n, int side, int c, void* stream) {
+  return dvd_posenc_add_ln(z, hs, ws, htab, wtab, out16, gamma, beta, eps, n, side, c, stream);
+}
+static int final_tokens_form0(const float* z, const float* g, const float* b, const float* sh, const float* sc, int ldmod, int mod_rows,
+                              const float* w8, const float* b8, const float* flow, float* x0, int n, int grid, void* stream) {
+  return dvd_final_tokens_form(z, g, b, sh, sc, ldmod, mod_rows, w8, b8, flow, x0, nullptr, n, grid, 0, stream);
+}
+static int dither_table(const void* segs, int nseg, long blocks, unsigned step, void* stream) {
+  return dvd_dither_f16_table((const dvd_dither_seg*)segs, nseg, blocks, step, stream);
+}
 
 __global__ void set_scalar_kernel(float* p, float v) { *p = v; }
 
@@ -348,7 +385,7 @@
   Engine* e = (Engine*)handle;
   DVD_REQUIRE((size_t)bytes >= e->need_bytes && ((uintptr_t)ws % 256) == 0,
               "engine_bind_workspace: need %zu bytes, 256-byte aligned (got %ld)", e->need_bytes, bytes);
-  e->ws = (char*)ws; e->ws_bytes = bytes; e->prepared = false;
+  e->ws = (char*)ws; e->ws_bytes = bytes; e->prepared = false; e->dith_dirty = true;
   e->drop_graphs();
   return DVD_OK;
 }
@@ -371,7 +408,7 @@
       DVD_REQUIRE(e->specs[i].nelem == nelem, "engine_set_tensor: %s expects %ld elements, got %ld", name,
                   e->specs[i].nelem, nelem);
       DVD_REQUIRE(((uintptr_t)dev_ptr % 16) == 0, "engine_set_tensor: %s must be 16-byte aligned", name);
-      if (e->wptr[i] != dev_ptr) e->drop_graphs();
+      if (e->wptr[i] != dev_ptr) { e->drop_graphs(); e->dith_dirty = true; }
       e->wptr[i] = dev_ptr;
       return DVD_OK;
     }
@@ -407,6 +444,7 @@
   if (strcmp(name, "split_weights") == 0) { e->split_weights = value != 0; e->drop_graphs(); return DVD_OK; }
   if (strcmp(name, "small_tiles") == 0) { e->small_tiles = value != 0; e->drop_graphs(); return DVD_OK; }
   if (strcmp(name, "ffn_lo") == 0) { e->ffn_lo = value != 0; e->drop_graphs(); return DVD_OK; }
+  if (strcmp(name, "fused_glue") == 0) { e->fused_glue = value != 0; e->drop_graphs(); return DVD_OK; }
   if (strcmp(name, "dither") == 0) { e->dither = value != 0; e->drop_graphs(); return DVD_OK; }
   if (strcmp(name, "dither_step") == 0) { e->dither_step = (unsigned)value; return DVD_OK; }
   if (strcmp(name, "graphs") == 0) {
@@ -560,6 +598,7 @@
   auto f32 = [e](int i) { return e->f32(i); };
   auto f16 = [e](int i) { return e->f16(i); };
   const long TH = (long)T * HID, TD = (long)T * DEC;
+  const bool glue = e->fused_glue;
 
   TRY(dvd_small_linear(f32(B_tbuf), 1, e->F(W_t_w0), e->F(W_t_b0), f32(B_th), HID, 1, 256, HID, 256, 2, 1, stream));
   TRY(dvd_small_linear(f32(B_th), HID, e->F(W_t_w2), e->F(W_t_b2), f32(B_cvec), HID, 1, HID, HID, HID, 0, 0, stream));
@@ -584,18 +623,31 @@
                .bias_rows(e->F(W_ca_bv)), stream));
   {
     const int kn[3] = {B_kc16, B_km16, B_kl16}, vn[3] = {B_vtc16, B_vtm16, B_vtl16};
-    for (int s = 0; s < 3; ++s)
-      TRY(attn(Attn(64, 6, N, T, T, hyp, 0.125f).q(f16(B_q16), HID, TH).k(f16(kn[s]), HID, TH).vt(f16(vn[s]), T, TH)
-                   .out(f16(B_att16) + (size_t)s * NT * HID, HID, TH), stream));
-    TRY(attn(Attn(64, 6, N, T, T, 1, 0.125f).q(f16(B_q16), HID, TH).k(f16(B_kr16), HID, TH).vt(f16(B_vtr16), T, TH)
-                 .out(f16(B_att16) + (size_t)3 * NT * HID, HID, TH), stream));
+    if (glue) {
+      dvd_attn_group grp[4];
+      for (int s = 0; s < 4; ++s)
+        grp[s] = {s < 3 ? f16(kn[s]) : f16(B_kr16), TH, s < 3 ? f16(vn[s]) : f16(B_vtr16), TH,
+                  f16(B_att16) + (size_t)s * NT * HID, TH, s < 3 ? hyp : 1};
+      const Attn shared = Attn(64, 6, N, T, T, 1, 0.125f).q(f16(B_q16), HID, TH).k(nullptr, HID, 0).vt(nullptr, T, 0)
+                              .out(nullptr, HID, 0);
+      TRY(attn_multi(shared, grp, 4, stream));
+    } else {
+      for (int s = 0; s < 3; ++s)
+        TRY(attn(Attn(64, 6, N, T, T, hyp, 0.125f).q(f16(B_q16), HID, TH).k(f16(kn[s]), HID, TH).vt(f16(vn[s]), T, TH)
+                     .out(f16(B_att16) + (size_t)s * NT * HID, HID, TH), stream));
+      TRY(attn(Attn(64, 6, N, T, T, 1, 0.125f).q(f16(B_q16), HID, TH).k(f16(B_kr16), HID, TH).vt(f16(B_vtr16), T, TH)
+                   .out(f16(B_att16) + (size_t)3 * NT * HID, HID, TH), stream));
+    }
   }
   TRY(gemm(Gemm(F16, (int)NT, HID, HID, 4).a(f16(B_att16), HID, NT * HID).b(e->W16(W_ca_wo16), HID).out32(f32(B_z), DEC, HID)
                .bias_col(e->F(W_ca_bo)).add_res(f32(B_xtok32), HID), stream));
 
   if (e->debug_stop == 1) return check_launch("engine_denoise_step(stop 1)");
-  TRY(dvd_layernorm_rows(f32(B_z), DEC, HID, f16(B_h16), HID, NT * HID, 4, NT, HID, nullptr, nullptr, sh_a, sc_a, 0, (int)NT,
-                         1e-6f, stream));
+  if (glue)
+    TRY(dvd_layernorm_rows(f32(B_z), DEC, HID, f16(B_h16), HID, NT * HID, 4, NT, HID, nullptr, nullptr, sh_a, sc_a, 0, (int)NT,
+                           1e-6f, stream));
+  else
+    TRY(layernorm_rows_form0(f32(B_z), DEC, HID, f16(B_h16), HID, NT * HID, 4, NT, HID, sh_a, sc_a, 0, (int)NT, 1e-6f, stream));
   TRY(gemm(Gemm(F16, (int)(4 * NT), 2 * HID, HID).a(f16(B_h16), HID).b(e->W16(W_sa_wqk16), HID).out16(f16(B_qk16), 2 * HID)
                .bias_col(e->F(W_sa_bqk)), stream));
   TRY(gemm(Gemm(F16S, HID, T, HID, 4 * N).a(e->W16(W_sa_wv16), HID).b(f16(B_h16), HID, TH).out16(f16(B_vt16), T, TH)
@@ -604,28 +656,38 @@
                .vt(f16(B_vt16), T, TH).out(f16(B_att16), HID, TH), stream));
   TRY(gemm(Gemm(F16, (int)NT, HID, HID, 4).a(f16(B_att16), HID, NT * HID).b(e->W16(W_sa_wp16), HID).out32(f32(B_z), DEC, HID)
                .bias_col(e->F(W_sa_bp)).mul_gate(g_a, (int)NT).add_res(f32(B_z), DEC, HID), stream));
-  TRY(dvd_layernorm_rows(f32(B_z), DEC, HID, f16(B_h16), HID, NT * HID, 4, NT, HID, nullptr, nullptr, sh_m, sc_m, 0, (int)NT,
-                         1e-6f, stream));
+  if (glue)
+    TRY(dvd_layernorm_rows(f32(B_z), DEC, HID, f16(B_h16), HID, NT * HID, 4, NT, HID, nullptr, nullptr, sh_m, sc_m, 0, (int)NT,
+                           1e-6f, stream));
+  else
+    TRY(layernorm_rows_form0(f32(B_z), DEC, HID, f16(B_h16), HID, NT * HID, 4, NT, HID, sh_m, sc_m, 0, (int)NT, 1e-6f, stream));
   TRY(gemm(Gemm(F16, (int)(4 * NT), 4 * HID, HID).a(f16(B_h16), HID).b(e->W16(W_fc1_w16), HID).out16(f16(B_mlp16), 4 * HID)
                .bias_col(e->F(W_fc1_b)).act_fn(GELU), stream));
   TRY(gemm(Gemm(F16, (int)NT, HID, 4 * HID, 4).a(f16(B_mlp16), 4 * HID, NT * 4 * HID).b(e->W16(W_fc2_w16), 4 * HID)
                .out32(f32(B_z), DEC, HID).bias_col(e->F(W_fc2_b)).mul_gate(g_m, (int)NT).add_res(f32(B_z), DEC, HID), stream));
 
   if (e->debug_stop == 2) return check_launch("engine_denoise_step(stop 2)");
-  TRY(dvd_colmean(f32(B_z), f32(B_part), f32(B_pooled), N, T, DEC, COLCHUNKS, stream));
+  if (glue) TRY(dvd_colmean(f32(B_z), f32(B_part), f32(B_pooled), N, T, DEC, COLCHUNKS, stream));
+  else TRY(colmean_form0(f32(B_z), f32(B_part), f32(B_pooled), N, T, DEC, COLCHUNKS, stream));
   TRY(dvd_small_linear(f32(B_pooled), DEC, e->F(W_pe_h0_w), e->F(W_pe_h0_b), f32(B_petmp), DEC, N, DEC, DEC, DEC, 0, 2, stream));
   TRY(dvd_small_linear(f32(B_petmp), DEC, e->F(W_pe_h2_w), e->F(W_pe_h2_b), f32(B_hs), DEC, N, DEC, DEC, DEC, 0, 3, stream));
   TRY(dvd_small_linear(f32(B_pooled), DEC, e->F(W_pe_w0_w), e->F(W_pe_w0_b), f32(B_petmp), DEC, N, DEC, DEC, DEC, 0, 2, stream));
   TRY(dvd_small_linear(f32(B_petmp), DEC, e->F(W_pe_w2_w), e->F(W_pe_w2_b), f32(B_wsc), DEC, N, DEC, DEC, DEC, 0, 3, stream));
-  TRY(dvd_posenc_add(f32(B_z), f32(B_hs), f32(B_wsc), e->F(W_pe_htab), e->F(W_pe_wtab), N, side, DEC, stream));
+  const bool fuse_pe = glue && e->debug_stop != 3;
+  if (fuse_pe)
+    TRY(posenc_add_ln(f32(B_z), f32(B_hs), f32(B_wsc), e->F(W_pe_htab), e->F(W_pe_wtab), f16(B_h16), e->F(W_dec(0, WD_n1w)),
+                          e->F(W_dec(0, WD_n1b)), 1e-5f, N, side, DEC, stream));
+  else
+    TRY(dvd_posenc_add(f32(B_z), f32(B_hs), f32(B_wsc), e->F(W_pe_htab), e->F(W_pe_wtab), N, side, DEC, stream));
 
   if (e->debug_stop == 3) return check_launch("engine_denoise_step(stop 3)");
   _Float16* f1 = f16(B_mlp16);
   _Float16* f2 = f1 + (size_t)NT * FFN;
   for (int j = 0; j < DEC_LAYERS; ++j) {
     auto w = [j](int k) { return W_dec(j, k); };
-    TRY(dvd_layernorm_rows(f32(B_z), DEC, 0, f16(B_h16), DEC, 0, 1, NT, DEC, e->F(w(WD_n1w)), e->F(w(WD_n1b)), nullptr, nullptr,
-                           0, 1, 1e-5f, stream));
+    if (j > 0 || !fuse_pe)
+      TRY(dvd_layernorm_rows(f32(B_z), DEC, 0, f16(B_h16), DEC, 0, 1, NT, DEC, e->F(w(WD_n1w)), e->F(w(WD_n1b)), nullptr, nullptr,
+                             0, 1, 1e-5f, stream));
     TRY(gemm(Gemm(F16, (int)NT, 2 * DEC, DEC).a(f16(B_h16), DEC).b(e->W16(w(WD_wqk16)), DEC).out16(f16(B_qk16), 2 * DEC),
              stream));
     TRY(gemm(Gemm(F16, DEC, T, DEC, N).a(e->W16(w(WD_wv16)), DEC).b(f16(B_h16), DEC, TD).out16(f16(B_vt16), T, TD), stream));
@@ -652,8 +714,12 @@
   }
 
   const float* finmod = f32(B_finmod);
-  TRY(dvd_final_tokens(f32(B_z), e->F(W_dec_nw), e->F(W_dec_nb), finmod, finmod + DEC, 0, (int)NT, e->F(W_fin_w),
-                       e->F(W_fin_b), init_flow, x0_out, nullptr, N, G, stream));
+  if (glue)
+    TRY(dvd_final_tokens(f32(B_z), e->F(W_dec_nw), e->F(W_dec_nb), finmod, finmod + DEC, 0, (int)NT, e->F(W_fin_w),
+                         e->F(W_fin_b), init_flow, x0_out, nullptr, N, G, stream));
+  else
+    TRY(final_tokens_form0(f32(B_z), e->F(W_dec_nw), e->F(W_dec_nb), finmod, finmod + DEC, 0, (int)NT, e->F(W_fin_w), e->F(W_fin_b),
+                           init_flow, x0_out, N, G, stream));
   return check_launch("engine_denoise_step");
 }
 
@@ -670,9 +736,26 @@
   set_scalar_kernel<<<1, 1, 0, st>>>(e->f32(B_tbuf), t_embed);
   if (e->dither && !e->small_tiles) {
     _Float16* dst = e->f16(B_w16dith);
-    for (int i : e->dith_list)
-      TRY(dvd_dither_f16(e->wptr[i], e->wptr[i + 1], dst + e->dith_off[i], e->specs[i].nelem, (unsigned)e->dith_off[i],
-                         e->dither_step, stream));
+    if (e->fused_glue && e->dith_list.size() <= 64) {
+      if (e->dith_dirty) {
+        e->dith_segs.clear();
+        for (int i : e->dith_list)
+          e->dith_segs.push_back({e->wptr[i], e->wptr[i + 1], dst + e->dith_off[i], e->specs[i].nelem, (unsigned)e->dith_off[i], 0u});
+        e->dith_blocks = dvd_dither_table_fill(e->dith_segs.data(), (int)e->dith_segs.size());
+        DVD_REQUIRE(e->dith_blocks > 0, "engine_denoise_step: bad dither table");
+        if (hipMemcpyAsync(e->B(B_dithtab), e->dith_segs.data(), e->dith_segs.size() * sizeof(dvd_dither_seg),
+                           hipMemcpyHostToDevice, st) != hipSuccess) {
+          set_error("engine_denoise_step: dither table upload failed");
+          return DVD_E_LAUNCH;
+        }
+        e->dith_dirty = false;
+      }
+      TRY(dither_table(e->B(B_dithtab), (int)e->dith_segs.size(), e->dith_blocks, e->dither_step, stream));
+    } else {
+      for (int i : e->dith_list)
+        TRY(dvd_dither_f16(e->wptr[i], e->wptr[i + 1], dst + e->dith_off[i], e->specs[i].nelem, (unsigned)e->dith_off[i],
+                           e->dither_step, stream));
+    }
   }
   if (!e->use_graphs || e->prof_on || e->debug_stop)
     return enqueue_step(e, x_t, feat_mode, init_flow, init_feat_nchw, x0_out, stream);
diff --git a/dvd_amd/csrc/tokens.hip b/dvd_amd/csrc/tokens.hip
--- a/dvd_amd/csrc/tokens.hip
+++ b/dvd_amd/csrc/tokens.hip
@@ -1,3 +1,5 @@
+#include <algorithm>
+
 #include "common.h"
 #include "mfma.h"
 
@@ -110,6 +112,66 @@
       o[e] = (_Float16)y;
     }
     *(hvec*)(op + c0) = o;
+  }
+}
+
+__global__ void __launch_bounds__(256) layernorm_rows4x384_kernel(const float* __restrict__ in, int ldin, long sIn,
+                                                                  _Float16* __restrict__ out, int ldout, long sOut,
+                                                                  const float* __restrict__ shift,
+                                                                  const float* __restrict__ scale, int ldmod, int mod_rows,
+                                                                  float eps, long rows) {
+  constexpr int C = 384, PER = 6, V = 2, NV = 3;
+  const long row = (long)blockIdx.x * 4 + (threadIdx.x >> 6);
+  if (row >= rows) return;
+  const int lane = threadIdx.x & 63;
+  typedef float fvec __attribute__((ext_vector_type(V)));
+  typedef _Float16 hvec __attribute__((ext_vector_type(V)));
+  fvec x[4][NV];
+#pragma unroll
+  for (int z = 0; z < 4; ++z)
+#pragma unroll
+    for (int k = 0; k < NV; ++k) x[z][k] = *(const fvec*)(in + z * sIn + row * ldin + (k * 64 + lane) * V);
+  const float* sh = shift + (row / mod_rows) * ldmod;
+  const float* sc = scale + (row / mod_rows) * ldmod;
+  fvec scv[NV], shv[NV];
+#pragma unroll
+  for (int k = 0; k < NV; ++k) {
+    const int c0 = (k * 64 + lane) * V;
+    scv[k] = *(const fvec*)(sc + c0);
+    shv[k] = *(const fvec*)(sh + c0);
+  }
+#pragma unroll
+  for (int z = 0; z < 4; ++z) {
+    float v[PER];
+    float s = 0.f;
+#pragma unroll
+    for (int k = 0; k < NV; ++k)
+#pragma unroll
+      for (int e = 0; e < V; ++e) {
+        v[k * V + e] = x[z][k][e];
+        s += x[z][k][e];
+      }
+    const float mean = wave_sum(s) * (1.f / C);
+    float q2 = 0.f;
+#pragma unroll
+    for (int k = 0; k < PER; ++k) {
+      const float d = v[k] - mean;
+      q2 += d * d;
+    }
+    const float rstd = rsqrtf(wave_sum(q2) * (1.f / C) + eps);
+    _Float16* op = out + z * sOut + row * ldout;
+#pragma unroll
+    for (int k = 0; k < NV; ++k) {
+      const int c0 = (k * 64 + lane) * V;
+      hvec o;
+#pragma unroll
+      for (int e = 0; e < V; ++e) {
+        float y = (v[k * V + e] - mean) * rstd;
+        y = y * (1.f + scv[k][e]) + shv[k][e];
+        o[e] = (_Float16)y;
+      }
+      *(hvec*)(op + c0) = o;
+    }
   }
 }
 
@@ -455,6 +517,33 @@
   part[((size_t)n * chunks + chunk) * c + col] = s;
 }
 
+__global__ void __launch_bounds__(128) colsum_partial4_kernel(const float* __restrict__ z, float* __restrict__ part,
+                                                              int T, int c, int chunks) {
+  const int n = blockIdx.z, chunk = blockIdx.y;
+  const int col = (blockIdx.x * 128 + threadIdx.x) * 4;
+  if (col >= c) return;
+  const int per = (T + chunks - 1) / chunks;
+  const int t0 = chunk * per, t1 = min(T, t0 + per);
+  const float* p = z + ((size_t)n * T + t0) * c + col;
+  floatx4 s = {0.f, 0.f, 0.f, 0.f};
+  int t = t0;
+  for (; t + 8 <= t1; t += 8, p += (size_t)8 * c) {
+    floatx4 x[8];
+#pragma unroll
+    for (int u = 0; u < 8; ++u) x[u] = *(const floatx4*)(p + (size_t)u * c);
+#pragma unroll
+    for (int u = 0; u < 8; ++u)
+#pragma unroll
+      for (int e = 0; e < 4; ++e) s[e] += x[u][e];
+  }
+  for (; t < t1; ++t, p += c) {
+    const floatx4 x = *(const floatx4*)p;
+#pragma unroll
+    for (int e = 0; e < 4; ++e) s[e] += x[e];
+  }
+  *(floatx4*)(part + ((size_t)n * chunks + chunk) * c + col) = s;
+}
+
 __global__ void __launch_bounds__(256) colmean_final_kernel(const float* __restrict__ part,
                                                             float* __restrict__ pooled, int T, int c, int chunks,
                                                             int total) {
@@ -485,6 +574,90 @@
 #pragma unroll
   for (int e = 0; e < 4; ++e) v[e] = (v[e] + a[e] * hb[e]) + b[e] * wb[e];
   *(floatx4*)(z + tok * c + ch) = v;
+}
+
+constexpr int PE_ROWS = 4;
+__global__ void __launch_bounds__(256, 2) posenc_add_ln_kernel(float* __restrict__ z, const float* __restrict__ hs,
+                                                               const float* __restrict__ ws, const float* __restrict__ htab,
+                                                               const float* __restrict__ wtab, int side,
+                                                               _Float16* __restrict__ out, const float* __restrict__ gamma,
+                                                               const float* __restrict__ beta, float eps, long rows) {
+  constexpr int C = 1536, PER = 24, V = 4, NV = 6;
+  const long row0 = ((long)blockIdx.x * 4 + __builtin_amdgcn_readfirstlane((int)(threadIdx.x >> 6))) * PE_ROWS;
+  if (row0 >= rows) return;
+  const int lane = threadIdx.x & 63;
+  const int T = side * side;
+  floatx4 x[PE_ROWS][NV];
+#pragma unroll
+  for (int u = 0; u < PE_ROWS; ++u) {
+    const float* zp = z + min(row0 + u, rows - 1) * C;
+#pragma unroll
+    for (int k = 0; k < NV; ++k) x[u][k] = *(const floatx4*)(zp + (k * 64 + lane) * V);
+  }
+  floatx4 a[NV], b[NV], hb[NV], wb[NV];
+  int n_have = -1, ty_have = -1;
+  typedef _Float16 hvec __attribute__((ext_vector_type(V)));
+#pragma unroll
+  for (int u = 0; u < PE_ROWS; ++u) {
+    const long row = row0 + u;
+    if (row < rows) {
+      const int n = (int)(row / T), t = (int)(row % T);
+      const int ty = t / side, tx = t % side;
+#pragma unroll
+      for (int k = 0; k < NV; ++k) wb[k] = *(const floatx4*)(wtab + (size_t)tx * C + (k * 64 + lane) * V);
+      if (n != n_have) {
+        n_have = n;
+#pragma unroll
+        for (int k = 0; k < NV; ++k) {
+          a[k] = *(const floatx4*)(hs + (size_t)n * C + (k * 64 + lane) * V);
+          b[k] = *(const floatx4*)(ws + (size_t)n * C + (k * 64 + lane) * V);
+        }
+      }
+      if (ty != ty_have) {
+        ty_have = ty;
+#pragma unroll
+        for (int k = 0; k < NV; ++k) hb[k] = *(const floatx4*)(htab + (size_t)ty * C + (k * 64 + lane) * V);
+      }
+      float* zp = z + row * C;
+      float v[PER];
+      float s = 0.f;
+#pragma unroll
+      for (int k = 0; k < NV; ++k) {
+        const int ch = (k * 64 + lane) * V;
+        floatx4 vv = x[u][k];
+#pragma unroll
+        for (int e = 0; e < 4; ++e) vv[e] = (vv[e] + a[k][e] * hb[k][e]) + b[k][e] * wb[k][e];
+        *(floatx4*)(zp + ch) = vv;
+#pragma unroll
+        for (int e = 0; e < V; ++e) {
+          v[k * V + e] = vv[e];
+          s += vv[e];
+        }
+      }
+      const float mean = wave_sum(s) * (1.f / C);
+      float q2 = 0.f;
+#pragma unroll
+      for (int k = 0; k < PER; ++k) {
+        const float d = v[k] - mean;
+        q2 += d * d;
+      }
+      const float rstd = rsqrtf(wave_sum(q2) * (1.f / C) + eps);
+      _Float16* op = out + row * C;
+#pragma unroll
+      for (int k = 0; k < NV; ++k) {
+        const int c0 = (k * 64 + lane) * V;
+        const floatx4 g = *(const floatx4*)(gamma + c0), bt = *(const floatx4*)(beta + c0);
+        hvec o;
+#pragma unroll
+        for (int e = 0; e < V; ++e) {
+          float y = (v[k * V + e] - mean) * rstd;
+          y = y * g[e] + bt[e];
+          o[e] = (_Float16)y;
+        }
+        *(hvec*)(op + c0) = o;
+      }
+    }
+  }
 }
 
 __global__ void __launch_bounds__(256) small_linear_kernel(const float* __restrict__ x, int ldx,
@@ -617,6 +790,121 @@
   }
 }
 
+__global__ void __launch_bounds__(256, 2) final_tokens_walk_kernel(const float* __restrict__ z,
+                                                                   const float* __restrict__ gamma,
+                                                                   const float* __restrict__ beta,
+                                                                   const float* __restrict__ shift,
+                                                                   const float* __restrict__ scale, int ldmod,
+                                                                   int mod_rows, const float* __restrict__ w,
+                                                                   const float* __restrict__ b,
+                                                                   const float* __restrict__ init_flow,
+                                                                   float* __restrict__ x0, float* __restrict__ tok8, int g,
+                                                                   int rpw, long rows) {
+  constexpr int C = 1536, PER = 24;
+  __shared__ __attribute__((aligned(16))) float sw[8 * C];
+  for (int i = threadIdx.x; i < 8 * C / 4; i += 256) ((floatx4*)sw)[i] = ((const floatx4*)w)[i];
+  __syncthreads();
+  const int lane = threadIdx.x & 63;
+  const long wid = (long)blockIdx.x * 4 + __builtin_amdgcn_readfirstlane((int)(threadIdx.x >> 6));
+  const long r0 = wid * rpw, r1 = min(rows, r0 + rpw);
+  if (r0 >= rows) return;
+  float gm[PER], bt[PER], osc[PER], shv[PER];
+#pragma unroll
+  for (int k = 0; k < 6; ++k) {
+    const floatx4 a = *(const floatx4*)(gamma + (k * 64 + lane) * 4), c = *(const floatx4*)(beta + (k * 64 + lane) * 4);
+#pragma unroll
+    for (int e = 0; e < 4; ++e) { gm[k * 4 + e] = a[e]; bt[k * 4 + e] = c[e]; }
+  }
+  const float bias = lane < 8 ? b[lane] : 0.f;
+  const int side = g >> 1, T = side * side;
+  long cur_mod = -1;
+  floatx4 nx[6];
+#pragma unroll
+  for (int k = 0; k < 6; ++k) nx[k] = *(const floatx4*)(z + r0 * C + (k * 64 + lane) * 4);
+  for (long row = r0; row < r1; ++row) {
+    float v[PER];
+    float s = 0.f;
+#pragma unroll
+    for (int k = 0; k < 6; ++k) {
+      const floatx4 f = nx[k];
+#pragma unroll
+      for (int e = 0; e < 4; ++e) {
+        v[k * 4 + e] = f[e];
+        s += f[e];
+      }
+    }
+    {
+      const float* np = z + min(row + 1, r1 - 1) * C;
+#pragma unroll
+      for (int k = 0; k < 6; ++k) nx[k] = *(const floatx4*)(np + (k * 64 + lane) * 4);
+    }
+    const long mr = row / mod_rows;
+    if (mr != cur_mod) {
+      cur_mod = mr;
+      const float* sh = shift + mr * ldmod;
+      const float* sc = scale + mr * ldmod;
+#pragma unroll
+      for (int k = 0; k < 6; ++k) {
+        const floatx4 a = *(const floatx4*)(sc + (k * 64 + lane) * 4), c = *(const floatx4*)(sh + (k * 64 + lane) * 4);
+#pragma unroll
+        for (int e = 0; e < 4; ++e) { osc[k * 4 + e] = 1.f + a[e]; shv[k * 4 + e] = c[e]; }
+      }
+    }
+    float mean = wave_sum(s) * (1.f / C);
+    float q2 = 0.f;
+#pragma unroll
+    for (int k = 0; k < PER; ++k) {
+      const float d = v[k] - mean;
+      q2 += d * d;
+    }
+    float rstd = rsqrtf(wave_sum(q2) * (1.f / C) + 1e-5f);
+    s = 0.f;
+#pragma unroll
+    for (int k = 0; k < PER; ++k) {
+      v[k] = (v[k] - mean) * rstd * gm[k] + bt[k];
+      s += v[k];
+    }
+    mean = wave_sum(s) * (1.f / C);
+    q2 = 0.f;
+#pragma unroll
+    for (int k = 0; k < PER; ++k) {
+      const float d = v[k] - mean;
+      q2 += d * d;
+    }
+    rstd = rsqrtf(wave_sum(q2) * (1.f / C) + 1e-6f);
+    float dot[8];
+#pragma unroll
+    for (int j = 0; j < 8; ++j) dot[j] = 0.f;
+#pragma unroll
+    for (int k = 0; k < 6; ++k) {
+      floatx4 wv[8];
+      asm volatile("" ::: "memory");
+#pragma unroll
+      for (int j = 0; j < 8; ++j) wv[j] = *(const floatx4*)(sw + j * C + (k * 64 + lane) * 4);
+#pragma unroll
+      for (int e = 0; e < 4; ++e) {
+        const float y = ((v[k * 4 + e] - mean) * rstd) * osc[k * 4 + e] + shv[k * 4 + e];
+#pragma unroll
+        for (int j = 0; j < 8; ++j) dot[j] += y * wv[j][e];
+      }
+    }
+#pragma unroll
+    for (int j = 0; j < 8; ++j) dot[j] = wave_sum(dot[j]);
+    if (lane < 8) {
+      float o = 0.f;
+#pragma unroll
+      for (int j = 0; j < 8; ++j)
+        if (lane == j) o = dot[j];
+      o += bias;
+      if (tok8) tok8[row * 8 + lane] = o;
+      const int n = (int)(row / T), t = (int)(row % T);
+      const int p = lane >> 2, q = (lane >> 1) & 1, c = lane & 1;
+      const size_t at = (((size_t)n * 2 + c) * g + 2 * (t / side) + p) * g + 2 * (t % side) + q;
+      x0[at] = o + (init_flow ? init_flow[at] : 0.f);
+    }
+  }
+}
+
 }
 
 using namespace dvd;
@@ -632,10 +920,10 @@
   return check_launch("embed_obs_ln");
 }
 
-extern "C" int dvd_layernorm_rows(const float* in, int ldin, long stride_in, void* out16, int ldout, long stride_out,
-                                  int batch, long rows, int c, const float* gamma, const float* beta,
-                                  const float* shift, const float* scale, int ldmod, int mod_rows, float eps,
-                                  void* stream) {
+extern "C" int dvd_layernorm_rows_form(const float* in, int ldin, long stride_in, void* out16, int ldout, long stride_out,
+                                       int batch, long rows, int c, const float* gamma, const float* beta,
+                                       const float* shift, const float* scale, int ldmod, int mod_rows, float eps, int form,
+                                       void* stream) {
   DVD_REQUIRE(in && out16, "layernorm_rows: null pointer");
   DVD_REQUIRE(c == 384 || c == 1536, "layernorm_rows: C=%d not in {384,1536}", c);
   DVD_REQUIRE((gamma == nullptr) == (beta == nullptr) && (shift == nullptr) == (scale == nullptr),
@@ -646,8 +934,12 @@
                   ((uintptr_t)in % 16) == 0 && ((uintptr_t)out16 % 8) == 0 && ((uintptr_t)gamma % 16) == 0 &&
                   ((uintptr_t)beta % 16) == 0 && ((uintptr_t)shift % 16) == 0 && ((uintptr_t)scale % 16) == 0,
               "layernorm_rows: rows must be 16-byte aligned (vector loads)");
+  DVD_REQUIRE(form == 0 || form == 1, "layernorm_rows: form %d not in {0,1}", form);
   dim3 grid(cdiv(rows, 4), batch);
-  if (c == 384)
+  if (form == 1 && c == 384 && batch == 4 && ldin == 1536 && stride_in == 384 && !gamma && shift)
+    layernorm_rows4x384_kernel<<<LAUNCH_ROWS(rows)>>>(in, ldin, stride_in, (_Float16*)out16, ldout, stride_out, shift, scale,
+                                                      ldmod, mod_rows, eps, rows);
+  else if (c == 384)
     layernorm_rows_kernel<384><<<grid, 256, 0, (hipStream_t)stream>>>(in, ldin, stride_in, (_Float16*)out16, ldout,
                                                                        stride_out, gamma, beta, shift, scale, ldmod,
                                                                        mod_rows > 0 ? mod_rows : 1, eps, rows);
@@ -656,6 +948,14 @@
                                                                         stride_out, gamma, beta, shift, scale, ldmod,
                                                                         mod_rows > 0 ? mod_rows : 1, eps, rows);
   return check_launch("layernorm_rows");
+}
+
+extern "C" int dvd_layernorm_rows(const float* in, int ldin, long stride_in, void* out16, int ldout, long stride_out,
+                                  int batch, long rows, int c, const float* gamma, const float* beta,
+                                  const float* shift, const float* scale, int ldmod, int mod_rows, float eps,
+                                  void* stream) {
+  return dvd_layernorm_rows_form(in, ldin, stride_in, out16, ldout, stride_out, batch, rows, c, gamma, beta, shift, scale,
+                                 ldmod, mod_rows, eps, 1, stream);
 }
 
 extern "C" int dvd_build_r_rows(const float* feat_nhwc, const float* init_feat_nchw, const float* flow, void* out16,
@@ -739,14 +1039,25 @@
   return check_launch("dwconv3x3");
 }
 
+extern "C" int dvd_colmean_form(const float* z, float* partial, float* pooled, int n, int t, int c, int chunks, int form,
+                                void* stream) {
+  DVD_REQUIRE(z && partial && pooled, "colmean: null pointer");
+  DVD_REQUIRE(n > 0 && n < 65536 && t > 0 && c > 0 && chunks > 0 && chunks < 65536, "colmean: bad shape");
+  DVD_REQUIRE(form == 0 || form == 1, "colmean: form %d not in {0,1}", form);
+  if (form == 1 && c % 4 == 0 && ((uintptr_t)z % 16) == 0 && ((uintptr_t)partial % 16) == 0) {
+    dim3 grid(cdiv(c / 4, 128), chunks, n);
+    colsum_partial4_kernel<<<grid, 128, 0, (hipStream_t)stream>>>(z, partial, t, c, chunks);
+  } else {
+    dim3 grid(cdiv(c, 256), chunks, n);
+    colsum_partial_kernel<<<grid, 256, 0, (hipStream_t)stream>>>(z, partial, t, c, chunks);
+  }
+  colmean_final_kernel<<<cdiv((long)n * c, 256), 256, 0, (hipStream_t)stream>>>(partial, pooled, t, c, chunks, n * c);
+  return check_launch("colmean");
+}
+
 extern "C" int dvd_colmean(const float* z, float* partial, float* pooled, int n, int t, int c, int chunks,
                            void* stream) {
-  DVD_REQUIRE(z && partial && pooled, "colmean: null pointer");
-  DVD_REQUIRE(n > 0 && n < 65536 && t > 0 && c > 0 && chunks > 0 && chunks < 65536, "colmean: bad shape");
-  dim3 grid(cdiv(c, 256), chunks, n);
-  colsum_partial_kernel<<<grid, 256, 0, (hipStream_t)stream>>>(z, partial, t, c, chunks);
-  colmean_final_kernel<<<cdiv((long)n * c, 256), 256, 0, (hipStream_t)stream>>>(partial, pooled, t, c, chunks, n * c);
-  return check_launch("colmean");
+  return dvd_colmean_form(z, partial, pooled, n, t, c, chunks, 1, stream);
 }
 
 extern "C" int dvd_posenc_add(float* z, const float* hs, const float* ws, const float* htab, const float* wtab,
@@ -756,6 +1067,20 @@
   const long total4 = (long)n * side * side * (c / 4);
   posenc_add_kernel<<<cdiv(total4, 256), 256, 0, (hipStream_t)stream>>>(z, hs, ws, htab, wtab, side, c, total4);
   return check_launch("posenc_add");
+}
+
+extern "C" int dvd_posenc_add_ln(float* z, const float* hs, const float* ws, const float* htab, const float* wtab,
+                                 void* out16, const float* gamma, const float* beta, float eps, int n, int side, int c,
+                                 void* stream) {
+  DVD_REQUIRE(z && hs && ws && htab && wtab && out16 && gamma && beta, "posenc_add_ln: null pointer");
+  DVD_REQUIRE(n > 0 && side > 0 && c == 1536, "posenc_add_ln: bad shape (C must be 1536)");
+  DVD_REQUIRE(((uintptr_t)z % 16) == 0 && ((uintptr_t)hs % 16) == 0 && ((uintptr_t)ws % 16) == 0 &&
+                  ((uintptr_t)htab % 16) == 0 && ((uintptr_t)wtab % 16) == 0 && ((uintptr_t)out16 % 8) == 0 &&
+                  ((uintptr_t)gamma % 16) == 0 && ((uintptr_t)beta % 16) == 0,
+              "posenc_add_ln: pointers must be 16-byte aligned (vector loads)");
+  const long rows = (long)n * side * side;
+  posenc_add_ln_kernel<<<LAUNCH_ROWS(cdiv(rows, PE_ROWS))>>>(z, hs, ws, htab, wtab, side, (_Float16*)out16, gamma, beta, eps, rows);
+  return check_launch("posenc_add_ln");
 }
 
 extern "C" int dvd_small_linear(const float* x, int ldx, const float* w, const float* b, float* y, int ldy, int m,
@@ -768,13 +1093,33 @@
   return check_launch("small_linear");
 }
 
+constexpr long FINAL_WALK_MIN_ROWS = 8192;
+constexpr int FINAL_WALK_MIN_RPW = 8, FINAL_WALK_WAVES = 2048;
+extern "C" int dvd_final_tokens_form(const float* z, const float* gamma, const float* beta, const float* shift,
+                                     const float* scale, int ldmod, int mod_rows, const float* w8, const float* b8,
+                                     const float* init_flow, float* x0, float* tok8, int n, int g, int form, void* stream) {
+  DVD_REQUIRE(z && gamma && beta && shift && scale && w8 && b8 && x0, "final_tokens: null pointer");
+  DVD_REQUIRE(n > 0 && g >= 2 && g % 2 == 0 && mod_rows > 0, "final_tokens: bad shape");
+  DVD_REQUIRE(form >= -1 && form <= 1, "final_tokens: form %d not in {-1,0,1}", form);
+  const long rows = (long)n * (g / 2) * (g / 2);
+  const bool aligned = ldmod % 4 == 0 && ((uintptr_t)z % 16) == 0 && ((uintptr_t)gamma % 16) == 0 &&
+                       ((uintptr_t)beta % 16) == 0 && ((uintptr_t)shift % 16) == 0 && ((uintptr_t)scale % 16) == 0 &&
+                       ((uintptr_t)w8 % 16) == 0;
+  DVD_REQUIRE(form != 1 || aligned, "final_tokens: the walk form needs 16-byte aligned vectors");
+  if (form == 1 || (form == -1 && aligned && rows >= FINAL_WALK_MIN_ROWS)) {
+    const int rpw = (int)std::max<long>(FINAL_WALK_MIN_RPW, cdiv(rows, (long)FINAL_WALK_WAVES));
+    const long waves = cdiv(rows, (long)rpw);
+    final_tokens_walk_kernel<<<(unsigned)cdiv(waves, 4L), 256, 0, (hipStream_t)stream>>>(
+        z, gamma, beta, shift, scale, ldmod, mod_rows, w8, b8, init_flow, x0, tok8, g, rpw, rows);
+    return check_launch("final_tokens(walk)");
+  }
+  final_tokens_kernel<<<LAUNCH_ROWS(rows)>>>(z, gamma, beta, shift, scale, ldmod, mod_rows, w8, b8, init_flow, x0,
+                                             tok8, g, rows);
+  return check_launch("final_tokens");
+}
+
 extern "C" int dvd_final_tokens(const float* z, const float* gamma, const float* beta, const float* shift,
                                 const float* scale, int ldmod, int mod_rows, const float* w8, const float* b8,
                                 const float* init_flow, float* x0, float* tok8, int n, int g, void* stream) {
-  DVD_REQUIRE(z && gamma && beta && shift && scale && w8 && b8 && x0, "final_tokens: null pointer");
-  DVD_REQUIRE(n > 0 && g >= 2 && g % 2 == 0 && mod_rows > 0, "final_tokens: bad shape");
-  const long rows = (long)n * (g / 2) * (g / 2);
-  final_tokens_kernel<<<LAUNCH_ROWS(rows)>>>(z, gamma, beta, shift, scale, ldmod, mod_rows, w8, b8, init_flow, x0,
-                                             tok8, g, rows);
-  return check_launch("final_tokens");
-}
+  return dvd_final_tokens_form(z, gamma, beta, shift, scale, ldmod, mod_rows, w8, b8, init_flow, x0, tok8, n, g, -1, stream);
+}
diff --git a/dvd_amd/lib.py b/dvd_amd/lib.py
--- a/dvd_amd/lib.py
+++ b/dvd_amd/lib.py
@@ -57,6 +57,16 @@
                 ("scale", C.c_float)]
 
 
+class AttnGroup(C.Structure):
+    _fields_ = [("K", C.c_void_p), ("strideK", C.c_long), ("Vt", C.c_void_p), ("strideVt", C.c_long),
+                ("O", C.c_void_p), ("strideO", C.c_long), ("kv_batch_div", C.c_int)]
+
+
+class DitherSeg(C.Structure):
+    _fields_ = [("hi", C.c_void_p), ("lo", C.c_void_p), ("out", C.c_void_p), ("nelem", C.c_long), ("elem0", C.c_uint),
+                ("block0", C.c_uint)]
+
+
 class CnOp(C.Structure):
     _fields_ = [("op", C.c_int), ("a", C.c_int), ("b", C.c_int), ("dst", C.c_int), ("ks", C.c_int), ("dil", C.c_int),
                 ("cout", C.c_int), ("act", C.c_int), ("w_off", C.c_long), ("h", C.c_int), ("w", C.c_int),
@@ -100,7 +110,8 @@
               "dvd_flash_attn_kernel_name", "dvd_gemm_kernel_name", "dvd_convnet_workspace_bytes", "dvd_convnet_weight_floats",
               "dvd_ingest_scratch_bytes", "dvd_ingest_ragged_scratch_bytes", "dvd_resize_gray_scratch_bytes",
               "dvd_msssim_workspace_bytes", "dvd_png_bound", "dvd_png_scratch_bytes", "dvd_png_scratch_bytes_huff", "dvd_jpeg_bound",
-              "dvd_jpeg_scratch_bytes", "dvd_sflow_level_workspace_bytes", "dvd_sflow_workspace_bytes"}
+              "dvd_jpeg_scratch_bytes", "dvd_sflow_level_workspace_bytes", "dvd_sflow_workspace_bytes",
+              "dvd_dither_table_fill"}
 
 SIGNATURES = {
     "dvd_grid_sample_bilinear_zeros_ac": [c_void, c_void, c_void, C.c_int, C.c_int, C.c_int, C.c_int, C.c_int,
@@ -122,19 +133,27 @@
     "dvd_gemm_nt": [C.POINTER(GemmDesc), c_void],
     "dvd_gemm_kernel_name": [C.POINTER(GemmDesc)],
     "dvd_flash_attn": [C.POINTER(AttnDesc), c_void],
+    "dvd_flash_attn_multi": [C.POINTER(AttnDesc), C.POINTER(AttnGroup), C.c_int, c_void],
     "dvd_embed_obs_ln": [c_void, c_void, c_void, c_void, c_void, c_void, C.c_int, C.c_int, c_void],
     "dvd_layernorm_rows": [c_void, C.c_int, C.c_long, c_void, C.c_int, C.c_long, C.c_int, C.c_long, C.c_int, c_void,
                            c_void, c_void, c_void, C.c_int, C.c_int, C.c_float, c_void],
+    "dvd_layernorm_rows_form": [c_void, C.c_int, C.c_long, c_void, C.c_int, C.c_long, C.c_int, C.c_long, C.c_int, c_void,
+                                c_void, c_void, c_void, C.c_int, C.c_int, C.c_float, C.c_int, c_void],
     "dvd_build_r_rows": [c_void, c_void, c_void, c_void, C.c_int, C.c_int, C.c_int, C.c_int, C.c_int, c_void],
     "dvd_patch_rows": [c_void, C.c_long, C.c_long, C.c_long, C.c_long, c_void, C.c_int, C.c_int, C.c_int, C.c_int,
                        c_void],
     "dvd_dwconv3x3": [c_void, c_void, c_void, c_void, C.c_int, C.c_int, C.c_int, c_void],
     "dvd_colmean": [c_void, c_void, c_void, C.c_int, C.c_int, C.c_int, C.c_int, c_void],
     "dvd_posenc_add": [c_void, c_void, c_void, c_void, c_void, C.c_int, C.c_int, C.c_int, c_void],
+    "dvd_colmean_form": [c_void, c_void, c_void, C.c_int, C.c_int, C.c_int, C.c_int, C.c_int, c_void],
+    "dvd_posenc_add_ln": [c_void, c_void, c_void, c_void, c_void, c_void, c_void, c_void, C.c_float, C.c_int, C.c_int,
+                          C.c_int, c_void],
     "dvd_small_linear": [c_void, C.c_int, c_void, c_void, c_void, C.c_int, C.c_int, C.c_int, C.c_int, C.c_int, C.c_int,
                          C.c_int, c_void],
     "dvd_final_tokens": [c_void, c_void, c_void, c_void, c_void, C.c_int, C.c_int, c_void, c_void, c_void, c_void,
                          c_void, C.c_int, C.c_int, c_void],
+    "dvd_final_tokens_form": [c_void, c_void, c_void, c_void, c_void, C.c_int, C.c_int, c_void, c_void, c_void, c_void,
+                              c_void, C.c_int, C.c_int, C.c_int, c_void],
     "dvd_im2col3x3": [c_void, C.c_long, C.c_long, C.c_long, c_void, C.c_int, C.c_int, C.c_int, C.c_int, c_void],
     "dvd_conv3x3_nhwc": [c_void, C.c_int, c_void, C.c_int, c_void, c_void, C.c_int, C.c_int, C.c_int, C.c_int, c_void],
     "dvd_maxpool2_nhwc": [c_void, c_void, C.c_int, C.c_int, C.c_int, c_void],
@@ -182,6 +201,8 @@
     "dvd_jpegdec_probe": [c_void, C.c_long, C.POINTER(JpegDecInfo)],
     "dvd_jpeg_decode_rgb8": [c_void, c_void, C.c_long, c_void, C.c_long, C.c_int, C.POINTER(C.c_int), c_void, c_void],
     "dvd_dither_f16": [c_void, c_void, c_void, C.c_long, C.c_uint, C.c_uint, c_void],
+    "dvd_dither_table_fill": [C.POINTER(DitherSeg), C.c_int],
+    "dvd_dither_f16_table": [c_void, C.c_int, C.c_long, C.c_uint, c_void],
     "dvd_engine_create": [C.c_int, C.c_int, C.c_int, C.POINTER(c_void)],
     "dvd_engine_destroy": [c_void],
     "dvd_engine_bind_workspace": [c_void, c_void, C.c_long],
@@ -203,7 +224,7 @@
             "dvd_resize_gray_scratch_bytes": C.c_long, "dvd_msssim_workspace_bytes": C.c_long,
             "dvd_sflow_level_workspace_bytes": C.c_long, "dvd_sflow_workspace_bytes": C.c_long,
             "dvd_png_bound": C.c_long, "dvd_png_scratch_bytes": C.c_long, "dvd_png_scratch_bytes_huff": C.c_long,
-            "dvd_jpeg_bound": C.c_long, "dvd_jpeg_scratch_bytes": C.c_long}
+            "dvd_jpeg_bound": C.c_long, "dvd_jpeg_scratch_bytes": C.c_long, "dvd_dither_table_fill": C.c_long}
 
 LAB_SIGNATURES = {"dvd_gemm_debug_stamps": [c_void], "dvd_attn_debug_stamps": [c_void]}
 
diff --git a/dvd_amd/ops.py b/dvd_amd/ops.py
--- a/dvd_amd/ops.py
+++ b/dvd_amd/ops.py
@@ -250,6 +250,25 @@
     return out
 
 
+def flash_attn_multi(q, groups, heads, head_dim, scale):
+    k0, vt0, out0, _ = groups[0]
+    d = lib.AttnDesc()
+    d.head_dim, d.heads, d.batch, d.tq, d.tk = head_dim, heads, q.shape[0], q.shape[1], k0.shape[1]
+    d.kv_batch_div = 1
+    d.Q, d.ldq, d.strideQ = q.data_ptr(), q.stride(1), q.stride(0)
+    d.ldk, d.ldvt, d.ldo = k0.stride(1), vt0.stride(1), out0.stride(1)
+    d.scale = scale
+    arr = (lib.AttnGroup * len(groups))()
+    for g, (k, vt, out, div) in zip(arr, groups):
+        assert (k.stride(1), vt.stride(1), out.stride(1)) == (d.ldk, d.ldvt, d.ldo) and k.shape[1] == d.tk
+        g.K, g.strideK = k.data_ptr(), k.stride(0)
+        g.Vt, g.strideVt = vt.data_ptr(), vt.stride(0)
+        g.O, g.strideO = out.data_ptr(), out.stride(0)
+        g.kv_batch_div = div
+    lib.call("dvd_flash_attn_multi", C.byref(d), arr, len(groups), stream_ptr())
+    return [g[2] for g in groups]
+
+
 def layernorm_rows(x, c, gamma=None, beta=None, shift=None, scale=None, mod_rows=1, eps=1e-6):
     rows = x.shape[0]
     out = torch.empty(rows, c, dtype=torch.float16, device=x.device)
diff --git a/include/dvd_hip.h b/include/dvd_hip.h
--- a/include/dvd_hip.h
+++ b/include/dvd_hip.h
@@ -95,6 +95,14 @@
 int dvd_flash_attn(const dvd_attn_desc* desc, void* stream);
 const char* dvd_flash_attn_kernel_name(int head_dim, int tq, int tk);
 
+typedef struct {
+  const void* K; long strideK;
+  const void* Vt; long strideVt;
+  void* O; long strideO;
+  int kv_batch_div;
+} dvd_attn_group;
+int dvd_flash_attn_multi(const dvd_attn_desc* desc, const dvd_attn_group* groups, int ngroups, void* stream);
+
 
 int dvd_embed_obs_ln(const float* x, const float* w, const float* bias, const float* pos, float* tok32,
                      void* ln16, int n, int g, void* stream);
@@ -102,6 +110,9 @@
 int dvd_layernorm_rows(const float* in, int ldin, long stride_in, void* out16, int ldout, long stride_out,
                        int batch, long rows, int c, const float* gamma, const float* beta, const float* shift,
                        const float* scale, int ldmod, int mod_rows, float eps, void* stream);
+int dvd_layernorm_rows_form(const float* in, int ldin, long stride_in, void* out16, int ldout, long stride_out,
+                            int batch, long rows, int c, const float* gamma, const float* beta, const float* shift,
+                            const float* scale, int ldmod, int mod_rows, float eps, int form, void* stream);
 
 int dvd_build_r_rows(const float* feat_nhwc, const float* init_feat_nchw, const float* flow, void* out16, int ldo,
                      int n, int g, int n_hyp, int mode, void* stream);
@@ -115,6 +126,10 @@
 int dvd_colmean(const float* z, float* partial, float* pooled, int n, int t, int c, int chunks, void* stream);
 int dvd_posenc_add(float* z, const float* hs, const float* ws, const float* htab, const float* wtab, int n, int side,
                    int c, void* stream);
+int dvd_colmean_form(const float* z, float* partial, float* pooled, int n, int t, int c, int chunks, int form,
+                     void* stream);
+int dvd_posenc_add_ln(float* z, const float* hs, const float* ws, const float* htab, const float* wtab, void* out16,
+                      const float* gamma, const float* beta, float eps, int n, int side, int c, void* stream);
 
 int dvd_small_linear(const float* x, int ldx, const float* w, const float* b, float* y, int ldy, int m, int k, int n,
                      int kmod, int act_in, int act_out, void* stream);
@@ -122,6 +137,9 @@
 int dvd_final_tokens(const float* z, const float* gamma, const float* beta, const float* shift, const float* scale,
                      int ldmod, int mod_rows, const float* w8, const float* b8, const float* init_flow, float* x0,
                      float* tok8, int n, int g, void* stream);
+int dvd_final_tokens_form(const float* z, const float* gamma, const float* beta, const float* shift, const float* scale,
+                          int ldmod, int mod_rows, const float* w8, const float* b8, const float* init_flow, float* x0,
+                          float* tok8, int n, int g, int form, void* stream);
 
 int dvd_im2col3x3(const float* in, long sc, long sy, long sx, float* out, int ldo, int c, int h, int w, void* stream);
 int dvd_conv3x3_nhwc(const float* in, int c, const float* wgt, int kp, const float* bias, float* out, int cout, int h, int w,
@@ -176,6 +194,13 @@
                          void* stream);
 
 int dvd_dither_f16(const void* hi, const void* lo, void* out, long nelem, unsigned elem0, unsigned step, void* stream);
+typedef struct {
+  const void* hi; const void* lo; void* out;
+  long nelem;
+  unsigned elem0, block0;
+} dvd_dither_seg;
+long dvd_dither_table_fill(dvd_dither_seg* segs, int nseg);
+int dvd_dither_f16_table(const dvd_dither_seg* segs_dev, int nseg, long blocks, unsigned step, void* stream);
 
 int dvd_engine_create(int grid, int docs, int n_hyp, void** handle);
 int dvd_engine_destroy(void* handle);
```

New measurement: 0.4906, median of 6. About the same (+0.7%).
